# GAP-LAB-CUHK-SZ/GaussReg

Measured on AMD Instinct MI355X. Metric: GS views/sec @1M pts 640x480 (+ radius_neighbors Mpts/sec, see radius_neighbors), higher is better.
Workload: dtype f32; 1 GPU; diff_gaussian_rasterization forward: 1000000 synthetic Gaussians (SH deg 3), 640x480, 32 views per step per GPU (configs[1]); gaussians=1000000, width=640, height=480, parallelism=per-view sharding x1

## Files before the change

### gaussreg_amd/_lib.py

```python
import ctypes
import os
import re

_HERE = os.path.dirname(os.path.abspath(__file__))
LIB_PATH = os.path.join(_HERE, "lib", "libgaussreg_hip.so")
HEADER_PATH = os.path.join(_HERE, "..", "include", "gaussreg_hip.h")
TRAIN_HEADER_PATH = os.path.join(_HERE, "..", "include", "gaussreg_hip_train.h")
MATCH_TRAIN_HEADER_PATH = os.path.join(_HERE, "..", "include", "gaussreg_hip_train_matching.h")
BACKBONE_TRAIN_HEADER_PATH = os.path.join(_HERE, "..", "include", "gaussreg_hip_train_backbone.h")

_lib = None

c_void = ctypes.c_void_p
c_f32 = ctypes.c_float


class RasterView(ctypes.Structure):
    _fields_ = [("image_height", ctypes.c_int32), ("image_width", ctypes.c_int32),
                ("tanfovx", c_f32), ("tanfovy", c_f32), ("bg", c_f32 * 3), ("scale_modifier", c_f32),
                ("viewmatrix", c_f32 * 16), ("projmatrix", c_f32 * 16), ("campos", c_f32 * 3),
                ("sh_degree", ctypes.c_int32), ("prefiltered", ctypes.c_int32), ("debug", ctypes.c_int32)]


class GsAdamGroup(ctypes.Structure):
    _fields_ = [("param", c_void), ("grad", c_void), ("exp_avg", c_void), ("exp_avg_sq", c_void),
                ("lr", ctypes.c_double), ("K", ctypes.c_int32)]


class GsDensifyGroup(ctypes.Structure):
    _fields_ = [("src_param", c_void), ("dst_param", c_void), ("src_exp_avg", c_void), ("dst_exp_avg", c_void),
                ("src_exp_avg_sq", c_void), ("dst_exp_avg_sq", c_void), ("K", ctypes.c_int32), ("role", ctypes.c_int32)]


_SCALARS = {"int": ctypes.c_int, "int32_t": ctypes.c_int32, "uint32_t": ctypes.c_uint32, "int64_t": ctypes.c_int64,
            "size_t": ctypes.c_size_t, "float": ctypes.c_float, "double": ctypes.c_double}
_POINTEES = set(_SCALARS) | {"void", "uint8_t", "uint64_t"}
_STRUCTS = {"gr_raster_view": RasterView, "gr_gs_adam_group": GsAdamGroup, "gr_gs_densify_group": GsDensifyGroup}
_TYPE = r"(?:const\s+)?(\w+)"


def _ctype(base, star, where):
    if star:
        if base == "char":
            return ctypes.c_char_p
        if base in _STRUCTS:
            return ctypes.POINTER(_STRUCTS[base])
        if base in _POINTEES:
            return ctypes.c_void_p
    elif base in _SCALARS:
        return _SCALARS[base]
    raise ValueError(f"gaussreg_hip.h: type '{base}{star}' in {where} is outside the binding's vocabulary")


def parse_header(text):
    text = re.sub(r"/\*.*?\*/", " ", text, flags=re.S)
    defines = {m.group(1): int(m.group(2)) for m in re.finditer(r"^[ \t]*#[ \t]*define[ \t]+(GR_\w+)[ \t]+(-?\d+)[ \t]*$",
                                                                  text, flags=re.M)}
    text = re.sub(r"^[ \t]*#.*$", "", text, flags=re.M)
    text = re.sub(r"\b(?:typedef\s+struct|enum)\b[^{};]*\{[^{}]*\}[^;]*;", "", text)
    text = re.sub(r'extern\s+"C"\s*\{(.*)\}', r"\1", text, flags=re.S)
    signatures = {}
    for decl in filter(None, (" ".join(d.split()) for d in text.split(";"))):
        m = re.fullmatch(r"(.+?)\b(gr_\w+) ?\((.*)\)", decl)
        if m is None:
            raise ValueError(f"gaussreg_hip.h: cannot parse the declaration '{decl}'")
        ret, name, args = m.group(1).strip(), m.group(2), m.group(3).strip()
        r = re.fullmatch(_TYPE + r"\s*(\*?)", ret)
        if r is None:
            raise ValueError(f"gaussreg_hip.h: cannot parse the return type '{ret}' of {name}")
        restype = None if r.groups() == ("void", "") else _ctype(r.group(1), r.group(2), f"the return type of {name}")
        argtypes = []
        for arg in ([] if args in ("", "void") else args.split(",")):
            a = re.fullmatch(_TYPE + r"(?:\s*(\*)\s*|\s+)\w+", arg.strip())
            if a is None:
                raise ValueError(f"gaussreg_hip.h: cannot parse the argument '{arg.strip()}' of {name}")
            argtypes.append(_ctype(a.group(1), a.group(2) or "", f"argument '{arg.strip()}' of {name}"))
        if name in signatures:
            raise ValueError(f"gaussreg_hip.h: {name} is declared twice")
        signatures[name] = (restype, argtypes)
    return signatures, defines


with open(HEADER_PATH) as _f:
    SIGNATURES, DEFINES = parse_header(_f.read())
with open(TRAIN_HEADER_PATH) as _f:
    TRAIN_SIGNATURES, TRAIN_DEFINES = parse_header(_f.read())
with open(MATCH_TRAIN_HEADER_PATH) as _f:
    MATCH_TRAIN_SIGNATURES, MATCH_TRAIN_DEFINES = parse_header(_f.read())
with open(BACKBONE_TRAIN_HEADER_PATH) as _f:
    BACKBONE_TRAIN_SIGNATURES, BACKBONE_TRAIN_DEFINES = parse_header(_f.read())

GR_PENDING = DEFINES["GR_PENDING"]
GR_RETRY_FULL = DEFINES["GR_RETRY_FULL"]
GR_RETRY_BIN = DEFINES["GR_RETRY_BIN"]
GS_ADAM_MAX_GROUPS = DEFINES["GR_GS_ADAM_MAX_GROUPS"]
GS_KNN_MAX_K = DEFINES["GR_GS_KNN_MAX_K"]
GS_DENSIFY_CARRIED, GS_DENSIFY_XYZ, GS_DENSIFY_SCALING = (DEFINES["GR_GS_DENSIFY_" + r] for r in ("CARRIED", "XYZ", "SCALING"))


class HipLibraryError(RuntimeError):
    pass


def lib():
    global _lib
    if _lib is None:
        import torch
        if not os.path.exists(LIB_PATH):
            raise HipLibraryError(
                f"{LIB_PATH} is missing: build it with `python -m gaussreg_amd.build` "
                "(there is no CPU fallback for the gaussreg_amd ops)")
        L = ctypes.CDLL(LIB_PATH)
        for name, (res, args) in (list(SIGNATURES.items()) + list(TRAIN_SIGNATURES.items())
                                   + list(MATCH_TRAIN_SIGNATURES.items()) + list(BACKBONE_TRAIN_SIGNATURES.items())):
            fn = getattr(L, name)
            fn.restype = res
            fn.argtypes = args
        _lib = L
    return _lib


def check(rc, allow=()):
    if rc != 0 and rc not in allow:
        msg = lib().gr_last_error()
        raise RuntimeError("gaussreg_hip: " + (msg.decode() if msg else f"error {rc}"))
    return rc


def tensor_stamp(tensors):
    out = []
    for t in tensors:
        if t.is_inference():
            return None
        out.append((t.data_ptr(), t._version))
    return tuple(out)


def require_gpu():
    import torch
    if not torch.cuda.is_available():
        raise HipLibraryError("gaussreg_amd ops need an MI355X (torch.cuda.is_available() is False); "
                              "there is no CPU fallback")
    return torch.device("cuda", torch.cuda.current_device())


_ws_cache = {}


def workspace(device, nbytes):
    import threading

    import torch
    key = (device.type, device.index, torch.cuda.current_stream(device).cuda_stream, threading.get_ident())
    buf = _ws_cache.get(key)
    if buf is None or buf.numel() < nbytes:
        buf = torch.empty(int(nbytes * 1.25) + 4096, dtype=torch.uint8, device=device)
        _ws_cache[key] = buf
    return buf


def stream_ptr(device):
    import torch
    return ctypes.c_void_p(torch.cuda.current_stream(device).cuda_stream)


def ptr(t):
    return ctypes.c_void_p(t.data_ptr()) if t is not None else ctypes.c_void_p(0)


def device_ptr(t, dev, what, pos=None):
    if t is None:
        return None
    if t.is_cuda and t.device == dev and t.is_contiguous():
        return t.data_ptr()
    where = what if pos is None else f"{what}: argument {pos}"
    if not t.is_contiguous():
        raise HipLibraryError(f"{where}: the tensor is not contiguous")
    raise HipLibraryError(f"{where}: the tensor is on {t.device}, the call runs on {dev}")


def call(dev, name, *args, ws=None, allow=()):
    import torch
    Tensor = torch.Tensor
    argv = [device_ptr(a, dev, name, i) if isinstance(a, Tensor) else a for i, a in enumerate(args)]
    if ws is not None:
        if not isinstance(ws, Tensor):
            ws = workspace(dev, ws)
        argv += (device_ptr(ws, dev, name + ": workspace"), ws.numel())
    fn = getattr(lib(), name)
    with torch.cuda.device(dev):
        return check(fn(*argv, torch.cuda.current_stream(dev).cuda_stream), allow)


def to_device(t, dev, dtype=None, name=None, cast=True):
    if dtype is not None and not cast and t.dtype != dtype:
        raise RuntimeError(f"{name} must be a float tensor" if name else "expected a float tensor")
    if dev is None:
        dev = require_gpu()
    t = t if t.is_cuda else t.to(dev)
    return (t if dtype is None else t.to(dtype)).contiguous()


def to_device_bool(t, dev):
    import torch
    return to_device(t if t.dtype == torch.bool else t != 0, dev)


def like_input(outs, out_device):
    if out_device.type == "cuda":
        return outs
    return tuple(o.to(out_device) for o in outs) if isinstance(outs, (tuple, list)) else outs.to(out_device)


def offsets(lengths):
    off = [0]
    for n in lengths:
        off.append(off[-1] + int(n))
    return off


def host_i64(values):
    arr = (ctypes.c_int64 * max(len(values), 1))(*[int(v) for v in values])
    return arr
```

### gaussreg_amd/build.py

```python
import concurrent.futures
import os
import subprocess
import sys

HERE = os.path.dirname(os.path.abspath(__file__))
CSRC = os.path.join(HERE, "csrc")
LIBDIR = os.path.join(HERE, "lib")
OBJDIR = os.path.join(LIBDIR, "obj")
LIB = os.path.join(LIBDIR, "libgaussreg_hip.so")

HIPCC = os.environ.get("HIPCC", "/opt/rocm/bin/hipcc")
FLAGS = ["--offload-arch=gfx950", "-O3", "-std=c++17", "-fPIC", "-ffp-contract=off", "-Wall",
         "-Wno-unused-function", "-Wno-unused-result"]


def sources():
    return sorted(f for f in os.listdir(CSRC) if f.endswith(".hip"))


def _stale(out, deps):
    if not os.path.exists(out):
        return True
    t = os.path.getmtime(out)
    return any(os.path.getmtime(d) > t for d in deps)


def build(force=False, verbose=False):
    os.makedirs(OBJDIR, exist_ok=True)
    headers = [os.path.join(CSRC, f) for f in os.listdir(CSRC) if f.endswith((".hpp", ".h"))]
    headers += [os.path.join(HERE, "..", "include", h) for h in ("gaussreg_hip.h", "gaussreg_hip_train.h",
                                                                 "gaussreg_hip_train_matching.h",
                                                                 "gaussreg_hip_train_backbone.h")]
    jobs = []
    objs = []
    for src in sources():
        s = os.path.join(CSRC, src)
        o = os.path.join(OBJDIR, src[:-4] + ".o")
        objs.append(o)
        if force or _stale(o, [s] + headers):
            jobs.append([HIPCC] + FLAGS + ["-c", s, "-o", o])

    def run(cmd):
        if verbose:
            print(" ".join(cmd), flush=True)
        r = subprocess.run(cmd, stdout=subprocess.PIPE, stderr=subprocess.STDOUT, text=True)
        return cmd, r.returncode, r.stdout

    if jobs:
        with concurrent.futures.ThreadPoolExecutor(max_workers=min(8, len(jobs))) as ex:
            for cmd, rc, out in ex.map(run, jobs):
                if rc != 0:
                    raise RuntimeError("hipcc failed: %s\n%s" % (" ".join(cmd), out))
                if verbose and out.strip():
                    print(out)
    if force or jobs or _stale(LIB, objs):
        cmd = [HIPCC, "--offload-arch=gfx950", "-shared", "-fPIC", "-o", LIB] + objs
        _, rc, out = run(cmd)
        if rc != 0:
            raise RuntimeError("link failed:\n" + out)
    return LIB


if __name__ == "__main__":
    print(build(force="--force" in sys.argv, verbose=True))
```

### gaussreg_amd/csrc/common.hpp

```cpp
#pragma once
#include <hip/hip_runtime.h>

#include <cstdarg>
#include <cstdint>
#include <cstdio>
#include <cstring>

#include "../../include/gaussreg_hip.h"

namespace gr {

constexpr int WAVE = 64;
#if defined(__HIP_DEVICE_COMPILE__) && !defined(__gfx950__)
#error "libgaussreg_hip is written for gfx950 (MI355X, 160 KB of LDS per CU): build with --offload-arch=gfx950"
#endif

void set_error(const char* fmt, ...);

#define GR_HIP(call)                                                                       \
  do {                                                                                     \
    hipError_t _e = (call);                                                                \
    if (_e != hipSuccess) {                                                                \
      gr::set_error("%s failed: %s (%s:%d)", #call, hipGetErrorString(_e), __FILE__, __LINE__); \
      return GR_ERR_HIP;                                                                   \
    }                                                                                      \
  } while (0)

#define GR_REQUIRE(cond, ...)       \
  do {                              \
    if (!(cond)) {                  \
      gr::set_error(__VA_ARGS__);   \
      return GR_ERR_INVALID;        \
    }                               \
  } while (0)

#define GR_LAUNCH_CHECK() GR_HIP(hipGetLastError())

inline size_t align_up(size_t x, size_t a) { return (x + a - 1) / a * a; }

struct Carver {
  char* base;
  size_t off = 0;
  explicit Carver(void* p) : base(static_cast<char*>(p)) {}
  template <typename T>
  T* take(size_t count) {
    off = align_up(off, 256);
    T* r = reinterpret_cast<T*>(base ? base + off : nullptr);
    off += sizeof(T) * count;
    return r;
  }
  size_t used() const { return align_up(off, 256); }
};

__host__ __device__ inline uint32_t f2ord(float f) {
  uint32_t u;
#ifdef __HIP_DEVICE_COMPILE__
  u = __float_as_uint(f);
#else
  memcpy(&u, &f, 4);
#endif
  return (u & 0x80000000u) ? ~u : (u | 0x80000000u);
}
__host__ __device__ inline float ord2f(uint32_t o) {
  uint32_t u = (o & 0x80000000u) ? (o & 0x7fffffffu) : ~o;
  float f;
#ifdef __HIP_DEVICE_COMPILE__
  f = __uint_as_float(u);
#else
  memcpy(&f, &u, 4);
#endif
  return f;
}

size_t scan_ws_ints(int64_t n);
constexpr int SCAN_SINGLE_ROW = 2048;
int exclusive_scan_i32(const int32_t* in, int32_t* out, int64_t n, int rows, int64_t row_stride,
                       int32_t* scan_ws, int32_t* total, hipStream_t stream, const int32_t* last_dev = nullptr,
                       int32_t* row_max = nullptr);

void* pinned_scratch(int slot, size_t bytes);

constexpr int MAIL_WORDS = 1024;
constexpr int MAIL_GRID_BOXES = 0;
constexpr int MAIL_GRID_COUNTS = 512;
constexpr int MAIL_RADIUS = 1008;
volatile int32_t* mailbox();
inline void mailbox_arm(volatile int32_t* stamp_word) { __atomic_store_n(stamp_word, 0, __ATOMIC_RELEASE); }
int mailbox_next_stamp();
int mailbox_wait(const volatile int32_t* stamp_word, int stamp, hipStream_t stream, const char* what);
__device__ __forceinline__ void mail_post(int32_t* stamp_word, int stamp) {
  __hip_atomic_store(stamp_word, stamp, __ATOMIC_RELEASE, __HIP_MEMORY_SCOPE_SYSTEM);
}

void bbox_block_offsets(const int32_t* h_off, int32_t* h_blk, int nb);
int compute_bbox(const float* pts, const int32_t* h_off, int32_t* h_blk, const int32_t* off_dev, int nb,
                 uint32_t* bbox_dev, int32_t* blk_off_dev, hipStream_t stream, bool blk_off_on_device = false,
                 bool init_bbox = true,
                 int32_t* zeroed_ticket = nullptr, int32_t* mail = nullptr, int stamp = 0);

size_t sort_pairs_temp_bytes(int64_t n);
int sort_pairs_u64_i32(void* temp, size_t temp_bytes, const uint64_t* keys_in, uint64_t* keys_out,
                       const int32_t* vals_in, int32_t* vals_out, int64_t n, int begin_bit,
                       int end_bit, hipStream_t stream);
int sort_pairs_u64_iota(void* temp, size_t temp_bytes, const uint64_t* keys_in, uint64_t* keys_out, int64_t period,
                        int32_t* vals_out, int64_t n, int begin_bit, int end_bit, hipStream_t stream);

int lds_atomics_lane_ordered(hipStream_t stream, bool* ordered);
int lds_atomics_lane_ordered_state();
int lds_ballot_ranking_force(int on);
void lds_order_demote();

constexpr int RASTER_TILE = 16;
constexpr uint32_t RECT_MARKER26 = 127u | (127u << 7);
#ifdef __HIPCC__
__device__ __forceinline__ void get_rect(float px, float py, int radius, int gx, int gy, int* rmin, int* rmax) {
  const float r = (float)radius;
  rmin[0] = min(gx, max(0, (int)((px - r) / (float)RASTER_TILE)));
  rmin[1] = min(gy, max(0, (int)((py - r) / (float)RASTER_TILE)));
  rmax[0] = min(gx, max(0, (int)((px + r + (float)(RASTER_TILE - 1)) / (float)RASTER_TILE)));
  rmax[1] = min(gy, max(0, (int)((py + r + (float)(RASTER_TILE - 1)) / (float)RASTER_TILE)));
}
__device__ __forceinline__ bool rect_decode(uint32_t r, int id, int64_t vbase, const float4* __restrict__ rec, int gx,
                                            int gy, int& x0, int& y0, int& w, int& h) {
  x0 = (int)(r & 127u);
  y0 = (int)((r >> 7) & 127u);
  w = (int)((r >> 14) & 63u);
  h = (int)((r >> 20) & 63u);
  if (r == RECT_MARKER26) {
    const float4 r0 = rec[4 * (vbase + id)];
    int rmin[2], rmax[2];
    get_rect(r0.x, r0.y, __float_as_int(rec[4 * (vbase + id) + 3].x), gx, gy, rmin, rmax);
    x0 = rmin[0];
    y0 = rmin[1];
    w = rmax[0] - rmin[0];
    h = rmax[1] - rmin[1];
  }
  return w * h != 0;
}
#endif

struct DepthSortTotals {
  int32_t* chunk_total;
  int chunk, nchunk;
  const float4* rec;
  int gx, gy;
};
struct DepthSortSegments {
  const int32_t* seg_off;
  const uint32_t* range_in;
  uint64_t* key64_out;
  int key64_shift;
  int32_t* big_cnt;
  int32_t* big_list;
  const uint64_t* gather64;
  int bins_used = 0;
  int xcd_segments = 0;
};
size_t depth_sort_table_bytes(int64_t P, int V);
int depth_sort_views(const uint32_t* field, const uint32_t* rect_raw, uint64_t* keys_a, uint64_t* keys_b, int32_t* ids_out,
                     uint32_t* rect_out, int32_t* nvalid_out, int64_t P, int V, int key_bits, void* table, size_t table_bytes,
                     hipStream_t stream, const int2* key_mm = nullptr, int nb_mm = 0, int32_t* overflow_flag = nullptr,
                     int overflow_value = 0, const DepthSortTotals* chunk_totals = nullptr,
                     const DepthSortSegments* segments = nullptr);
bool depth_sort_msd_possible(int64_t P, int V, int key_bits);

void kpconv_rowflag_launch(const float* s_feats, int64_t n, int64_t cin, uint8_t* flag, hipStream_t stream);
void kpconv_gather_launch(int plan, const float* s_feats, const float* q_points, const float* s_points,
                          const int64_t* neighbor_indices, int64_t n, int64_t m, int64_t h, int64_t cin, int64_t k,
                          const float* kernel_points, float sigma, float inf, const uint8_t* flag, float* WF, float* num,
                          hipStream_t stream);

struct KernelTimer {
  KernelTimer(const char* name, hipStream_t stream);
  ~KernelTimer();
  KernelTimer(const KernelTimer&) = delete;
  int slot_;
  hipStream_t stream_;
};

void unordered_map_order(const uint64_t* keys, int64_t n, int32_t base, int32_t* perm_out);
size_t hash_order_device_bytes(int64_t n, int64_t batch);
int hash_order_device(const uint64_t* keys, const int64_t* h_begins, int64_t batch, int32_t* perm_out, void* ws,
                      size_t ws_bytes, hipStream_t stream, const float* rows_in = nullptr, const int32_t* row_of = nullptr,
                      float* rows_out = nullptr);

__device__ __forceinline__ int wave_incl_scan_add_dpp(int v) {
  v += __builtin_amdgcn_update_dpp(0, v, 0x111, 0xf, 0xf, false);
  v += __builtin_amdgcn_update_dpp(0, v, 0x112, 0xf, 0xf, false);
  v += __builtin_amdgcn_update_dpp(0, v, 0x114, 0xf, 0xf, false);
  v += __builtin_amdgcn_update_dpp(0, v, 0x118, 0xf, 0xf, false);
  v += __builtin_amdgcn_update_dpp(0, v, 0x142, 0xa, 0xf, false);
  v += __builtin_amdgcn_update_dpp(0, v, 0x143, 0xc, 0xf, false);
  return v;
}

__device__ __forceinline__ double wave_sum_f64_dpp(double x) {
#define GR_F64_STEP(CTRL, ROWMASK)                                                                         \
  {                                                                                                        \
    const int lo = __builtin_amdgcn_update_dpp(0, __double2loint(x), CTRL, ROWMASK, 0xf, false);           \
    const int hi = __builtin_amdgcn_update_dpp(0, __double2hiint(x), CTRL, ROWMASK, 0xf, false);           \
    x += __hiloint2double(hi, lo);                                                                         \
  }
  GR_F64_STEP(0x111, 0xf) GR_F64_STEP(0x112, 0xf) GR_F64_STEP(0x114, 0xf) GR_F64_STEP(0x118, 0xf)
  GR_F64_STEP(0x142, 0xa) GR_F64_STEP(0x143, 0xc)
#undef GR_F64_STEP
  return __hiloint2double(__builtin_amdgcn_readlane(__double2hiint(x), 63), __builtin_amdgcn_readlane(__double2loint(x), 63));
}

#define GR_DPP_REDUCE(NAME, OP, IDENT)                                                         \
  __device__ __forceinline__ int NAME(int v) {                                                 \
    v = OP(v, __builtin_amdgcn_update_dpp(IDENT, v, 0x111, 0xf, 0xf, false));                  \
    v = OP(v, __builtin_amdgcn_update_dpp(IDENT, v, 0x112, 0xf, 0xf, false));                  \
    v = OP(v, __builtin_amdgcn_update_dpp(IDENT, v, 0x114, 0xf, 0xf, false));                  \
    v = OP(v, __builtin_amdgcn_update_dpp(IDENT, v, 0x118, 0xf, 0xf, false));                  \
    v = OP(v, __builtin_amdgcn_update_dpp(IDENT, v, 0x142, 0xa, 0xf, false));                  \
    v = OP(v, __builtin_amdgcn_update_dpp(IDENT, v, 0x143, 0xc, 0xf, false));                  \
    return __builtin_amdgcn_readlane(v, 63);                                                   \
  }
#define GR_OP_MIN(a, b) min(a, b)
#define GR_OP_MAX(a, b) max(a, b)
#define GR_OP_ADD(a, b) ((a) + (b))
GR_DPP_REDUCE(wave_min_i32_dpp, GR_OP_MIN, 0x7fffffff)
GR_DPP_REDUCE(wave_max_i32_dpp, GR_OP_MAX, (int)0x80000000)
GR_DPP_REDUCE(wave_sum_i32_dpp, GR_OP_ADD, 0)
#undef GR_DPP_REDUCE

__device__ inline int find_batch(const int32_t* __restrict__ off, int nb, int32_t i) {
  int lo = 0, hi = nb;
  while (hi - lo > 1) {
    int mid = (lo + hi) >> 1;
    if (off[mid] <= i) lo = mid; else hi = mid;
  }
  return lo;
}

}
```

### gaussreg_amd/csrc/preprocess_body.hpp

```cpp
#ifndef GR_PREPROCESS_BODY_OK
#error "preprocess_body.hpp is the body of the two preprocess kernels of rasterizer.hip"
#endif
static_assert(std::is_same<decltype(WAVE_MM), const bool>::value, "the including kernel defines `constexpr bool WAVE_MM`");
  if (LATE && blockIdx.x == 0 && threadIdx.x < (int)(sizeof(DevView) / 4))
    reinterpret_cast<float*>(const_cast<DevView*>(views))[threadIdx.x] = reinterpret_cast<const float*>(&cam1)[threadIdx.x];
  __shared__ float4 s_sh[(SH16 && !LATE) ? WAVE * SH_ROW : 1];
  __shared__ float4 s_rec[256 / WAVE][4 * REC_PLANE];
  __shared__ int s_mm[WAVE_MM ? 1 : 2][2][256 / WAVE];
  int i = blockIdx.x * blockDim.x + threadIdx.x;
  float shr[SH16 ? 48 : 1];
  if (SH16 && !LATE) {
    const int g0 = blockIdx.x * 256;
    const int n_here = min(256, P - g0);
    const float4* src = reinterpret_cast<const float4*>(shs + (int64_t)g0 * 48);
#pragma unroll 1
    for (int w = 0; w < 256 / WAVE; ++w) {
      const int lim = min(WAVE, n_here - w * WAVE) * 12;
#pragma unroll
      for (int u = 0; u < 3; ++u) {
        const int f = threadIdx.x + u * 256;
        if (f < lim) {
          const int g = f / 12, j = f - g * 12;
          s_sh[g * SH_ROW + j] = src[w * WAVE * 12 + f];
        }
      }
      __syncthreads();
      if ((int)threadIdx.x / WAVE == w && i < P) {
#pragma unroll
        for (int j = 0; j < 12; ++j) {
          const float4 t = s_sh[(threadIdx.x & (WAVE - 1)) * SH_ROW + j];
          shr[4 * j] = t.x;
          shr[4 * j + 1] = t.y;
          shr[4 * j + 2] = t.z;
          shr[4 * j + 3] = t.w;
        }
      }
      __syncthreads();
    }
  }
  const bool valid = i < P;
  const int lane = threadIdx.x & (WAVE - 1);
  const int wave_first = i - lane;
  i = min(i, P - 1);
  const float p[3] = {means3D[3 * (int64_t)i], means3D[3 * (int64_t)i + 1], means3D[3 * (int64_t)i + 2]};
  const float opacity = opacities[i];
  float c6[6];
  if (HAS_COV) {
#pragma unroll
    for (int k = 0; k < 6; ++k) c6[k] = cov3D_precomp[6 * (int64_t)i + k];
  }
  const int gx = (W + TILE - 1) / TILE, gy = (H + TILE - 1) / TILE;
  const float* sh = HAS_SH ? shs + (int64_t)i * M * 3 : nullptr;
  float cpre[3] = {0.f, 0.f, 0.f};
  if (!HAS_SH) {
#pragma unroll
    for (int k = 0; k < 3; ++k) cpre[k] = colors_precomp[3 * (int64_t)i + k];
  }
  float4* wrec = s_rec[threadIdx.x / WAVE];
  float mod_prev = 0.f;
  bool have_cov = HAS_COV;
  for (int v = 0; v < V; ++v) {
    const DevView& cam = LATE ? cam1 : views[v];
    const int64_t o = (int64_t)v * P + i;
    int out_radius = 0;
    uint32_t out_field = 0u, out_rect = 0u;
    float out_depth = 0.f, out_sxx = INFINITY, out_syy = INFINITY, out_kc = 0.f;
    float2 out_xy = make_float2(0.f, 0.f);
    float4 out_co = make_float4(0.f, 0.f, 0.f, 0.f);
    bool shade = false;
    float rgb[3] = {0.f, 0.f, 0.f};
    float pv[3];
    xform4x3(cam.view, p, pv);
    if (pv[2] > 0.2f) {
      float ph[4];
      xform4x4(cam.proj, p, ph);
      const float pw = 1.0f / (ph[3] + 0.0000001f);
      const float pprojx = ph[0] * pw, pprojy = ph[1] * pw;
      if (!HAS_COV && (!have_cov || cam.scale_mod != mod_prev)) {
        float sc[3], rot[4];
#pragma unroll
        for (int k = 0; k < 3; ++k) sc[k] = scales[3 * (int64_t)i + k];
#pragma unroll
        for (int k = 0; k < 4; ++k) rot[k] = rotations[4 * (int64_t)i + k];
        cov3d_from_scale_rot(sc, cam.scale_mod, rot, c6);
        have_cov = true;
        mod_prev = cam.scale_mod;
      }
      float cv[3];
      cov2d(pv, cam.fx, cam.fy, cam.tanx, cam.tany, c6, cam.view, cv);
      const float det = cv[0] * cv[2] - cv[1] * cv[1];
      if (det != 0.0f) {
        const float det_inv = 1.f / det;
        const float mid = 0.5f * (cv[0] + cv[2]);
        const float sq = sqrtf(fmaxf(0.1f, mid * mid - det));
        const float l1 = mid + sq, l2 = mid - sq;
        const float my_radius = ceilf(3.f * sqrtf(fmaxf(l1, l2)));
        const float px = ((pprojx + 1.0f) * (float)W - 1.0f) * 0.5f;
        const float py = ((pprojy + 1.0f) * (float)H - 1.0f) * 0.5f;
        int rmin[2], rmax[2];
        get_rect(px, py, (int)my_radius, gx, gy, rmin, rmax);
        const int ntile = (rmax[0] - rmin[0]) * (rmax[1] - rmin[1]);
        if (ntile != 0) {
          shade = true;
          if (HAS_SH && SH16 && LATE) {
            const float4* s4 = reinterpret_cast<const float4*>(shs + (int64_t)i * 48);
#pragma unroll
            for (int jj = 0; jj < 12; ++jj) {
              const float4 t4 = s4[jj];
              shr[4 * jj] = t4.x;
              shr[4 * jj + 1] = t4.y;
              shr[4 * jj + 2] = t4.z;
              shr[4 * jj + 3] = t4.w;
            }
            sh_to_rgb(D, p, cam.campos, [&](int k, int c) { return shr[k * 3 + c]; }, rgb);
          }
          out_depth = pv[2];
          out_radius = (int)my_radius;
          out_xy = make_float2(px, py);
          out_co = make_float4(cv[2] * det_inv, -cv[1] * det_inv, cv[0] * det_inv, opacity);
          const bool cullable = det > 0.0f && l2 >= 0.29f && l1 < 1.0e4f;
          const float kc = cullable ? 1.001f / (0.5f / l1 - 2.0e-6f) : INFINITY;
          out_kc = kc;
          if (cullable) {
            out_sxx = 2.0f * cv[0] * 1.004f;
            out_syy = 2.0f * cv[2] * 1.004f;
            const float pcm = __logf(255.0f * opacity) + 2.0e-3f;
            if (pcm > 0.0f) {
              const float cp = pcm + 2.0e-6f * (pcm * kc);
              const float hx = sqrtf(2.0f * cp * cv[0]) * 1.001f + 1.0e-2f;
              const float hy = sqrtf(2.0f * cp * cv[2]) * 1.001f + 1.0e-2f;
              const float xlo = ceilf(px - hx), xhi = floorf(px + hx), ylo = ceilf(py - hy), yhi = floorf(py + hy);
              if (xlo > -1.0e6f && xhi < 1.0e6f && ylo > -1.0e6f && yhi < 1.0e6f) {
                rmin[0] = max(rmin[0], (int)floorf(xlo / (float)TILE));
                rmin[1] = max(rmin[1], (int)floorf(ylo / (float)TILE));
                rmax[0] = min(rmax[0], (int)floorf(xhi / (float)TILE) + 1);
                rmax[1] = min(rmax[1], (int)floorf(yhi / (float)TILE) + 1);
                if (rmax[0] < rmin[0]) rmax[0] = rmin[0];
                if (rmax[1] < rmin[1]) rmax[1] = rmin[1];
              }
            }
          }
          uint32_t dk = __float_as_uint(out_depth) - KEY_DEPTH_BASE;
          if (dk >= (1u << KEY_DEPTH_BITS)) {
            dk = (1u << KEY_DEPTH_BITS) - 1;
            if (LATE) *far_flag = far_seq; else atomicOr(far_flag, 1);
          }
          out_field = dk;
          out_rect = pack_rect(rmin, rmax);
        }
      }
    }
    if (valid) {
      __builtin_nontemporal_store(out_radius, radii + o);
      dfield[o] = out_field;
      rect_raw[o] = out_rect;
    }
    wrec[0 * REC_PLANE + lane] = make_float4(out_xy.x, out_xy.y, out_sxx, out_syy);
    wrec[1 * REC_PLANE + lane] = out_co;
    wrec[3 * REC_PLANE + lane] = make_float4(__int_as_float(out_radius), out_depth, 0.f, 0.f);
    if (WAVE_MM) {
      const uint32_t fld = valid ? out_field : 0u;
      const int mn = wave_min_i32_dpp(fld != 0u ? (int)fld : 0x7fffffff), mx = wave_max_i32_dpp((int)fld);
      const int wave_id = __builtin_amdgcn_readfirstlane((int)(blockIdx.x * (256 / WAVE) + threadIdx.x / WAVE));
      if (lane == 0) key_mm[(int64_t)v * (gridDim.x * (256 / WAVE)) + wave_id] = make_int2(mn, mx);
      __builtin_amdgcn_fence(__ATOMIC_RELEASE, "wavefront");
      __builtin_amdgcn_wave_barrier();
      __builtin_amdgcn_fence(__ATOMIC_ACQUIRE, "wavefront");
    } else if (key_mm != nullptr) {
      const uint32_t fld = valid ? out_field : 0u;
      const int mn = wave_min_i32_dpp(fld != 0u ? (int)fld : 0x7fffffff), mx = wave_max_i32_dpp((int)fld);
      if (lane == 0) s_mm[v & 1][0][threadIdx.x / WAVE] = mn, s_mm[v & 1][1][threadIdx.x / WAVE] = mx;
      __syncthreads();
      if (threadIdx.x == 0) {
        int bmn = 0x7fffffff, bmx = 0;
#pragma unroll
        for (int w = 0; w < 256 / WAVE; ++w) bmn = min(bmn, s_mm[v & 1][0][w]), bmx = max(bmx, s_mm[v & 1][1][w]);
        key_mm[(int64_t)v * gridDim.x + blockIdx.x] = make_int2(bmn, bmx);
      }
    }
    if (shade && !(HAS_SH && SH16 && LATE)) {
      if (HAS_SH) {
        if (SH16) sh_to_rgb(D, p, cam.campos, [&](int k, int c) { return shr[k * 3 + c]; }, rgb);
        else sh_to_rgb(D, p, cam.campos, [&](int k, int c) { return sh[k * 3 + c]; }, rgb);
      } else {
        rgb[0] = cpre[0]; rgb[1] = cpre[1]; rgb[2] = cpre[2];
      }
    }
    wrec[2 * REC_PLANE + lane] = make_float4(rgb[0], rgb[1], rgb[2], out_kc);
    const unsigned long long vis = __ballot(valid && out_radius > 0);
    __builtin_amdgcn_fence(__ATOMIC_RELEASE, "wavefront");
    __builtin_amdgcn_wave_barrier();
    __builtin_amdgcn_fence(__ATOMIC_ACQUIRE, "wavefront");
    float4* wout = rec + 4 * ((int64_t)v * P + wave_first);
#pragma unroll
    for (int k = 0; k < 4; ++k) {
      const int rl = 16 * k + lane / 4;
      const float4 piece = wrec[(lane & 3) * REC_PLANE + rl];
      if ((vis >> rl) & 1ull) {
        typedef float pre_f4 __attribute__((ext_vector_type(4)));
        __builtin_nontemporal_store(pre_f4{piece.x, piece.y, piece.z, piece.w}, reinterpret_cast<pre_f4*>(wout + 4 * rl + (lane & 3)));
      }
    }
    __builtin_amdgcn_fence(__ATOMIC_RELEASE, "wavefront");
    __builtin_amdgcn_wave_barrier();
    __builtin_amdgcn_fence(__ATOMIC_ACQUIRE, "wavefront");
  }
```

### gaussreg_amd/csrc/raster_shared.hpp

```cpp
#pragma once

#include "common.hpp"

namespace gr {
namespace {

constexpr int TILE = 16;
constexpr int BLOCK = TILE * TILE;
constexpr int MAX_VIEWS = 64;

struct DevView {
  float view[16];
  float proj[16];
  float campos[3];
  float tanx, tany;
  float fx, fy;
  float scale_mod;
  float bg[3];
};

__device__ __constant__ float SH_C0 = 0.28209479177387814f;
__device__ __constant__ float SH_C1 = 0.4886025119029199f;
__device__ __constant__ float SH_C2[5] = {1.0925484305920792f, -1.0925484305920792f,
                                          0.31539156525252005f, -1.0925484305920792f,
                                          0.5462742152960396f};
__device__ __constant__ float SH_C3[7] = {-0.5900435899266435f, 2.890611442640554f,
                                          -0.4570457994644658f, 0.3731763325901154f,
                                          -0.4570457994644658f, 1.445305721320277f,
                                          -0.5900435899266435f};

__device__ __forceinline__ float exp_det(float x) {
  x = fmaxf(x, -86.0f);
  const float L2E = 1.44269504088896341f, MAGIC = 12582912.0f;
  const float t = x * L2E;
  const float tm = t + MAGIC;
  const float nf = tm - MAGIC;
  const float f = fmaf(x, L2E, -nf);
  float p = 1.3264815788716078e-3f;
  p = fmaf(p, f, 9.671512059867382e-3f);
  p = fmaf(p, f, 5.550733581185341e-2f);
  p = fmaf(p, f, 2.4022242426872253e-1f);
  p = fmaf(p, f, 6.931470036506653e-1f);
  p = fmaf(p, f, 1.0f);
  return __uint_as_float(__float_as_uint(p) + (__float_as_uint(tm) << 23));
}

__device__ __forceinline__ void xform4x3(const float* M, const float* p, float* o) {
  o[0] = fmaf(M[0], p[0], fmaf(M[4], p[1], fmaf(M[8], p[2], M[12])));
  o[1] = fmaf(M[1], p[0], fmaf(M[5], p[1], fmaf(M[9], p[2], M[13])));
  o[2] = fmaf(M[2], p[0], fmaf(M[6], p[1], fmaf(M[10], p[2], M[14])));
}
__device__ __forceinline__ void xform4x4(const float* M, const float* p, float* o) {
  o[0] = fmaf(M[0], p[0], fmaf(M[4], p[1], fmaf(M[8], p[2], M[12])));
  o[1] = fmaf(M[1], p[0], fmaf(M[5], p[1], fmaf(M[9], p[2], M[13])));
  o[2] = fmaf(M[2], p[0], fmaf(M[6], p[1], fmaf(M[10], p[2], M[14])));
  o[3] = fmaf(M[3], p[0], fmaf(M[7], p[1], fmaf(M[11], p[2], M[15])));
}

__device__ __forceinline__ void cov3d_from_scale_rot(const float* sc, float mod, const float* q,
                                                     float* c6) {
  const float s0 = mod * sc[0], s1 = mod * sc[1], s2 = mod * sc[2];
  const float r = q[0], x = q[1], y = q[2], z = q[3];
  float R[3][3];
  R[0][0] = 1.f - 2.f * (y * y + z * z);
  R[0][1] = 2.f * (x * y - r * z);
  R[0][2] = 2.f * (x * z + r * y);
  R[1][0] = 2.f * (x * y + r * z);
  R[1][1] = 1.f - 2.f * (x * x + z * z);
  R[1][2] = 2.f * (y * z - r * x);
  R[2][0] = 2.f * (x * z - r * y);
  R[2][1] = 2.f * (y * z + r * x);
  R[2][2] = 1.f - 2.f * (x * x + y * y);
  float M[3][3];
#pragma unroll
  for (int i = 0; i < 3; ++i) {
    M[0][i] = s0 * R[i][0];
    M[1][i] = s1 * R[i][1];
    M[2][i] = s2 * R[i][2];
  }
#define GR_SIG(i, j) fmaf(M[0][i], M[0][j], fmaf(M[1][i], M[1][j], M[2][i] * M[2][j]))
  c6[0] = GR_SIG(0, 0);
  c6[1] = GR_SIG(0, 1);
  c6[2] = GR_SIG(0, 2);
  c6[3] = GR_SIG(1, 1);
  c6[4] = GR_SIG(1, 2);
  c6[5] = GR_SIG(2, 2);
#undef GR_SIG
}

__device__ __forceinline__ void cov2d(const float* t_in, float fx, float fy, float tanx, float tany,
                                      const float* c6, const float* V, float* out3) {
  float t[3] = {t_in[0], t_in[1], t_in[2]};
  const float limx = 1.3f * tanx, limy = 1.3f * tany;
  const float txtz = t[0] / t[2], tytz = t[1] / t[2];
  t[0] = fminf(limx, fmaxf(-limx, txtz)) * t[2];
  t[1] = fminf(limy, fmaxf(-limy, tytz)) * t[2];
  const float J00 = fx / t[2];
  const float J02 = -(fx * t[0]) / (t[2] * t[2]);
  const float J11 = fy / t[2];
  const float J12 = -(fy * t[1]) / (t[2] * t[2]);
  float A0[3], A1[3];
#pragma unroll
  for (int j = 0; j < 3; ++j) {
    A0[j] = fmaf(J00, V[j * 4 + 0], J02 * V[j * 4 + 2]);
    A1[j] = fmaf(J11, V[j * 4 + 1], J12 * V[j * 4 + 2]);
  }
  const float S[3][3] = {{c6[0], c6[1], c6[2]}, {c6[1], c6[3], c6[4]}, {c6[2], c6[4], c6[5]}};
  float B0[3], B1[3];
#pragma unroll
  for (int k = 0; k < 3; ++k) {
    B0[k] = fmaf(S[k][0], A0[0], fmaf(S[k][1], A0[1], S[k][2] * A0[2]));
    B1[k] = fmaf(S[k][0], A1[0], fmaf(S[k][1], A1[1], S[k][2] * A1[2]));
  }
  out3[0] = fmaf(A0[0], B0[0], fmaf(A0[1], B0[1], A0[2] * B0[2])) + 0.3f;
  out3[1] = fmaf(A1[0], B0[0], fmaf(A1[1], B0[1], A1[2] * B0[2]));
  out3[2] = fmaf(A1[0], B1[0], fmaf(A1[1], B1[1], A1[2] * B1[2])) + 0.3f;
}

template <typename ShLoad>
__device__ __forceinline__ void sh_to_rgb(int deg, const float* pos, const float* campos,
                                          ShLoad S, float* rgb) {
  const float dx = pos[0] - campos[0], dy = pos[1] - campos[1], dz = pos[2] - campos[2];
  const float len = sqrtf(dx * dx + dy * dy + dz * dz);
  const float x = dx / len, y = dy / len, z = dz / len;
#pragma unroll
  for (int c = 0; c < 3; ++c) {
    float res = SH_C0 * S(0, c);
    if (deg > 0) {
      res = res - SH_C1 * y * S(1, c) + SH_C1 * z * S(2, c) - SH_C1 * x * S(3, c);
      if (deg > 1) {
        const float xx = x * x, yy = y * y, zz = z * z, xy = x * y, yz = y * z, xz = x * z;
        res = res + SH_C2[0] * xy * S(4, c) + SH_C2[1] * yz * S(5, c) +
              SH_C2[2] * (2.0f * zz - xx - yy) * S(6, c) + SH_C2[3] * xz * S(7, c) +
              SH_C2[4] * (xx - yy) * S(8, c);
        if (deg > 2) {
          res = res + SH_C3[0] * y * (3.0f * xx - yy) * S(9, c) + SH_C3[1] * xy * z * S(10, c) +
                SH_C3[2] * y * (4.0f * zz - xx - yy) * S(11, c) +
                SH_C3[3] * z * (2.0f * zz - 3.0f * xx - 3.0f * yy) * S(12, c) +
                SH_C3[4] * x * (4.0f * zz - xx - yy) * S(13, c) +
                SH_C3[5] * z * (xx - yy) * S(14, c) + SH_C3[6] * x * (xx - 3.0f * yy) * S(15, c);
        }
      }
    }
    res += 0.5f;
    rgb[c] = fmaxf(res, 0.0f);
  }
}

struct Geom {
  float4* rec;
  uint32_t* dfield;
  uint32_t* rect_raw;
  uint64_t* keys_a;
  uint64_t* keys_b;
  int32_t* order_a;
  int32_t* order_b;
  uint32_t* rects;
  uint16_t* chunk_cnt;
  uint32_t* seg_off;
  int32_t* chunk_total;
  int32_t* chunk_max;
  void* ds_table;
  size_t ds_table_bytes;
  int2* key_mm;
  int32_t* nvis;
  int32_t* totals;
  DevView* views;
  int32_t* scan_ws;
  size_t bytes;
};

constexpr int BIN_T = 256;
constexpr int BIN_CHUNK = 2048;

Geom carve_geom(void* p, int64_t P, int V, int64_t tiles) {
  Geom g;
  Carver c(p);
  const int64_t nchunk = (P + BIN_CHUNK - 1) / BIN_CHUNK;
  g.rec = c.take<float4>(P * V * 4);
  g.dfield = c.take<uint32_t>(P * V);
  g.rect_raw = c.take<uint32_t>(P * V);
  g.keys_a = c.take<uint64_t>(P * V);
  g.keys_b = c.take<uint64_t>(P * V);
  g.order_a = nullptr;
  g.order_b = c.take<int32_t>(P * V);
  g.rects = c.take<uint32_t>(P * V);
  g.chunk_cnt = c.take<uint16_t>(V * nchunk * tiles);
  g.seg_off = c.take<uint32_t>(V * nchunk * (tiles + 1));
  g.chunk_total = c.take<int32_t>(2 * V * nchunk);
  g.chunk_max = c.take<int32_t>(1);
  g.ds_table_bytes = depth_sort_table_bytes(P, V);
  g.ds_table = c.take<char>(g.ds_table_bytes);
  g.key_mm = c.take<int2>(V <= 4 ? V * ((P + 255) / 256) : P <= (1ll << 20) ? V * ((P + 255) / 256) * (256 / WAVE) : 0);
  g.nvis = c.take<int32_t>(V);
  g.totals = c.take<int32_t>(2 * V + 4 + MAX_VIEWS * (sizeof(DevView) / sizeof(int32_t)));
  g.views = reinterpret_cast<DevView*>(g.totals ? g.totals + 2 * V + 4 : nullptr);
  static_assert(sizeof(DevView) % sizeof(int32_t) == 0, "camera table follows an int array");
  g.scan_ws = c.take<int32_t>(V * scan_ws_ints(nchunk));
  g.bytes = c.used();
  return g;
}

struct Bin {
  int32_t* point_list;
  size_t bytes;
};

Bin carve_bin(void* p, int64_t R, int64_t vtiles) {
  Bin b;
  Carver c(p);
  (void)vtiles;
  b.point_list = c.take<int32_t>(R + 64);
  b.bytes = c.used();
  return b;
}

}
}
```

### gaussreg_amd/csrc/rasterizer.hip

```cpp
#include <algorithm>
#include <type_traits>
#include <vector>

#include <atomic>

#include "raster_shared.hpp"

namespace gr {
namespace {

static_assert(TILE == RASTER_TILE, "get_rect / rect_decode (common.hpp) are written for this tile size");


constexpr int KEY_DEPTH_BITS = 27;
constexpr uint32_t KEY_DEPTH_BASE = 0x3E000000u;

__device__ __forceinline__ uint32_t pack_rect(const int* rmin, const int* rmax) {
  const int w = rmax[0] - rmin[0], h = rmax[1] - rmin[1];
  if (w > 63 || h > 63 || rmin[0] > 126 || rmin[1] > 126) return RECT_MARKER26;
  return (uint32_t)rmin[0] | ((uint32_t)rmin[1] << 7) | ((uint32_t)w << 14) | ((uint32_t)h << 20);
}

constexpr int REC_PLANE = 66;
constexpr int SH_ROW = 13;

template <bool HAS_SH, bool HAS_COV, bool SH16, bool LATE>
__global__ __launch_bounds__(256) void preprocess_kernel(
    int P, int D, int M, int V, const DevView* __restrict__ views, const float* __restrict__ means3D,
    const float* __restrict__ shs, const float* __restrict__ colors_precomp,
    const float* __restrict__ opacities, const float* __restrict__ scales,
    const float* __restrict__ rotations, const float* __restrict__ cov3D_precomp, int W, int H,
    int32_t* __restrict__ radii, float4* __restrict__ rec, uint32_t* __restrict__ dfield,
    uint32_t* __restrict__ rect_raw, int32_t* __restrict__ far_flag, DevView cam1, int far_seq,
    int2* __restrict__ key_mm) {
  constexpr bool WAVE_MM = false;
#define GR_PREPROCESS_BODY_OK
#include "preprocess_body.hpp"
#undef GR_PREPROCESS_BODY_OK
}

template <bool HAS_SH, bool HAS_COV, bool SH16>
__global__ __launch_bounds__(256) void preprocess_many_kernel(
    int P, int D, int M, int V, const DevView* __restrict__ views, const float* __restrict__ means3D,
    const float* __restrict__ shs, const float* __restrict__ colors_precomp,
    const float* __restrict__ opacities, const float* __restrict__ scales,
    const float* __restrict__ rotations, const float* __restrict__ cov3D_precomp, int W, int H,
    int32_t* __restrict__ radii, float4* __restrict__ rec, uint32_t* __restrict__ dfield,
    uint32_t* __restrict__ rect_raw, int32_t* __restrict__ far_flag, DevView cam1, int far_seq,
    int2* __restrict__ key_mm) {
  constexpr bool WAVE_MM = true;
  constexpr bool LATE = false;
#define GR_PREPROCESS_BODY_OK
#include "preprocess_body.hpp"
#undef GR_PREPROCESS_BODY_OK
}

__global__ __launch_bounds__(256) void full_keys_kernel(int64_t n, const float4* __restrict__ rec,
                                                        const int32_t* __restrict__ radii, uint32_t* __restrict__ dfield) {
  const int64_t o = (int64_t)blockIdx.x * blockDim.x + threadIdx.x;
  if (o >= n) return;
  dfield[o] = radii[o] > 0 ? __float_as_uint(rec[4 * o + 3].y) : 0u;
}


__device__ __forceinline__ bool bin_block(int V, int nchunk, int& v, int& c) {
  const int b = blockIdx.x;
  if (V >= 8) {
    const int k = b >> 3;
    v = (b & 7) + 8 * (k / nchunk);
    c = k % nchunk;
    return v < V;
  }
  v = b / nchunk;
  c = b % nchunk;
  return true;
}
inline int bin_grid(int V, int nchunk) { return V >= 8 ? 8 * ((V + 7) / 8) * nchunk : V * nchunk; }
inline bool bin_scans_self(int nchunk, int V) { return !(nchunk <= SCAN_SINGLE_ROW && V <= 4); }
constexpr int SCATTER_WGS = 6;
constexpr int WIDE_T = 1024;

__device__ __forceinline__ constexpr int mod_small(int n, int d) {
  const unsigned long long tab = d <= 4 ? 0x2001'2aab'4001'8001ull : 0x1001'124a'1556'199aull;
  const unsigned int m = (unsigned int)(tab >> (((d - 1) & 3) * 16)) & 0xffffu;
  return n - (int)(((unsigned int)n * m) >> 15) * d;
}
static_assert(mod_small(255, 7) == 255 % 7 && mod_small(254, 3) == 254 % 3 && mod_small(250, 5) == 0 &&
              mod_small(251, 6) == 251 % 6 && mod_small(255, 8) == 7 && mod_small(200, 1) == 0, "mod_small multipliers");
template <typename F>
__device__ __forceinline__ void by_modulus(int mx, F&& f) {
  switch (mx) {
    case 1: f(std::integral_constant<int, 1>{}); break;
    case 2: f(std::integral_constant<int, 2>{}); break;
    case 3: f(std::integral_constant<int, 3>{}); break;
    case 4: f(std::integral_constant<int, 4>{}); break;
    case 5: f(std::integral_constant<int, 5>{}); break;
    case 6: f(std::integral_constant<int, 6>{}); break;
    case 7: f(std::integral_constant<int, 7>{}); break;
    default: f(std::integral_constant<int, 8>{}); break;
  }
}

__global__ __launch_bounds__(BIN_T) void tile_count_kernel(int P, int V, int gx, int gy, int nchunk,
                                                           const int32_t* __restrict__ nvis,
                                                           const uint32_t* __restrict__ rects,
                                                           const int32_t* __restrict__ ids,
                                                           const float4* __restrict__ rec,
                                                           uint16_t* __restrict__ chunk_cnt,
                                                           int32_t* __restrict__ chunk_total) {
  extern __shared__ unsigned int s_hist[];
  __shared__ int s_wsum[BIN_T / WAVE];
  int v, c;
  if (!bin_block(V, nchunk, v, c)) return;
  const int tiles = gx * gy;
  for (int T = threadIdx.x; T < tiles; T += BIN_T) s_hist[T] = 0u;
  __syncthreads();
  const int64_t vbase = (int64_t)v * P;
  const int nv = nvis[v];
  int mine = 0;
  uint32_t rr[BIN_CHUNK / BIN_T];
#pragma unroll
  for (int it = 0; it < BIN_CHUNK / BIN_T; ++it) {
    const int t = c * BIN_CHUNK + it * BIN_T + threadIdx.x;
    rr[it] = t < nv ? rects[vbase + t] : 0u;
  }
#pragma unroll
  for (int it = 0; it < BIN_CHUNK / BIN_T; ++it) {
    const int t = c * BIN_CHUNK + it * BIN_T + threadIdx.x;
    const uint32_t r = rr[it];
    if (r == 0u) continue;
    int x0, y0, w, h;
    if (!rect_decode(r, r == RECT_MARKER26 ? ids[vbase + t] : 0, vbase, rec, gx, gy, x0, y0, w, h)) continue;
    mine += w * h;
    for (int y = y0; y < y0 + h; ++y)
      for (int x = x0; x < x0 + w; ++x) atomicAdd(&s_hist[y * gx + x], 1u);
  }
  const int wsum = wave_sum_i32_dpp(mine);
  if ((threadIdx.x & (WAVE - 1)) == 0) s_wsum[threadIdx.x / WAVE] = wsum;
  __syncthreads();
  uint16_t* dst = chunk_cnt + ((int64_t)v * nchunk + c) * tiles;
  for (int T = threadIdx.x; T < tiles; T += BIN_T) dst[T] = (uint16_t)s_hist[T];
  if (threadIdx.x == 0) {
    int tot = 0;
    for (int i = 0; i < BIN_T / WAVE; ++i) tot += s_wsum[i];
    chunk_total[v * nchunk + c] = tot;
  }
}

__global__ __launch_bounds__(BIN_T) void chunk_total_kernel(int P, int V, int gx, int gy, int nchunk,
                                                            const int32_t* __restrict__ nvis,
                                                            const uint32_t* __restrict__ rects,
                                                            const int32_t* __restrict__ ids,
                                                            const float4* __restrict__ rec,
                                                            int32_t* __restrict__ chunk_total) {
  __shared__ int s_wsum[BIN_T / WAVE];
  int v, c;
  if (!bin_block(V, nchunk, v, c)) return;
  const int64_t vbase = (int64_t)v * P;
  const int nv = nvis[v];
  int mine = 0;
  uint32_t rr[BIN_CHUNK / BIN_T];
#pragma unroll
  for (int it = 0; it < BIN_CHUNK / BIN_T; ++it) {
    const int t = c * BIN_CHUNK + it * BIN_T + threadIdx.x;
    rr[it] = t < nv ? rects[vbase + t] : 0u;
  }
#pragma unroll
  for (int it = 0; it < BIN_CHUNK / BIN_T; ++it) {
    const int t = c * BIN_CHUNK + it * BIN_T + threadIdx.x;
    const uint32_t r = rr[it];
    int x0, y0, w, h;
    if (r != 0u && rect_decode(r, r == RECT_MARKER26 ? ids[vbase + t] : 0, vbase, rec, gx, gy, x0, y0, w, h)) mine += w * h;
  }
  const int wsum = wave_sum_i32_dpp(mine);
  if ((threadIdx.x & (WAVE - 1)) == 0) s_wsum[threadIdx.x / WAVE] = wsum;
  __syncthreads();
  if (threadIdx.x == 0) {
    int tot = 0;
    for (int i = 0; i < BIN_T / WAVE; ++i) tot += s_wsum[i];
    chunk_total[v * nchunk + c] = tot;
  }
}

__global__ __launch_bounds__(1024) void chunk_max_kernel(int n, const int32_t* __restrict__ chunk_total,
                                                         int32_t* __restrict__ chunk_max) {
  __shared__ int s_m[1024 / WAVE];
  int m = 0;
  for (int i = threadIdx.x; i < n; i += 1024) m = max(m, chunk_total[i]);
  m = wave_max_i32_dpp(m);
  if ((threadIdx.x & (WAVE - 1)) == 0) s_m[threadIdx.x / WAVE] = m;
  __syncthreads();
  if (threadIdx.x == 0) {
    for (int i = 0; i < 1024 / WAVE; ++i) m = max(m, s_m[i]);
    *chunk_max = m;
  }
}

template <bool SELF>
__global__ __launch_bounds__(256) void seg_scan_kernel(int V, int tiles, int nchunk, const uint16_t* __restrict__ chunk_cnt,
                                                       const int32_t* __restrict__ chunk_base ,
                                                       int32_t* __restrict__ totals, uint32_t* __restrict__ seg_off,
                                                       int32_t* __restrict__ mail, int mail_seq) {
  __shared__ int s_w[256 / WAVE];
  __shared__ int s_carry;
  const int v = blockIdx.x / nchunk, c = blockIdx.x % nchunk;
  const int lane = threadIdx.x & (WAVE - 1), wv = threadIdx.x / WAVE;
  int vb = 0;
  if (SELF) {
    const int me = (int)blockIdx.x;
    int part = 0;
    for (int i = threadIdx.x; i < me; i += 256) part += chunk_base[i];
    part = wave_sum_i32_dpp(part);
    if (lane == 0) s_w[wv] = part;
    __syncthreads();
    vb = s_w[0] + s_w[1] + s_w[2] + s_w[3];
    __syncthreads();
    if (c == 0) {
      int sum = 0, mx = 0;
      for (int i = threadIdx.x; i < nchunk; i += 256) {
        const int t = chunk_base[v * nchunk + i];
        sum += t;
        mx = max(mx, t);
      }
      sum = wave_sum_i32_dpp(sum);
      mx = wave_max_i32_dpp(mx);
      if (lane == 0) {
        s_w[wv] = sum;
      }
      __shared__ int s_m[256 / WAVE];
      if (lane == 0) s_m[wv] = mx;
      __syncthreads();
      if (threadIdx.x == 0) {
        const int tv = s_w[0] + s_w[1] + s_w[2] + s_w[3], mv = max(max(s_m[0], s_m[1]), max(s_m[2], s_m[3]));
        totals[v] = tv;
        totals[V + v] = mv;
        if (mail != nullptr) {
          __hip_atomic_store(&mail[v], tv, __ATOMIC_RELAXED, __HIP_MEMORY_SCOPE_SYSTEM);
          __hip_atomic_store(&mail[V + v], mv, __ATOMIC_RELAXED, __HIP_MEMORY_SCOPE_SYSTEM);
          if (v == 0) __hip_atomic_store(&mail[2 * V], totals[2 * V], __ATOMIC_RELAXED, __HIP_MEMORY_SCOPE_SYSTEM);
          __hip_atomic_store(&mail[2 * V + 1 + v], mail_seq, __ATOMIC_RELEASE, __HIP_MEMORY_SCOPE_SYSTEM);
        }
      }
      __syncthreads();
    }
  } else {
    for (int u = 0; u < v; ++u) vb += totals[u];
  }
  const uint16_t* src = chunk_cnt + ((int64_t)v * nchunk + c) * tiles;
  uint32_t* dst = seg_off + ((int64_t)v * nchunk + c) * (tiles + 1);
  if (threadIdx.x == 0) s_carry = SELF ? vb : vb + chunk_base[v * nchunk + c];
  __syncthreads();
  for (int T0 = 0; T0 < tiles; T0 += 256) {
    const int T = T0 + threadIdx.x;
    const int n = T < tiles ? (int)src[T] : 0;
    const int incl = wave_incl_scan_add_dpp(n);
    if (lane == WAVE - 1) s_w[wv] = incl;
    __syncthreads();
    int base = s_carry;
    for (int i = 0; i < wv; ++i) base += s_w[i];
    if (T < tiles) dst[T] = (uint32_t)(base + incl - n);
    __syncthreads();
    if (threadIdx.x == 255) s_carry = base + incl;
    __syncthreads();
  }
  if (threadIdx.x == 0) dst[tiles] = (uint32_t)s_carry;
}

constexpr int SEG_READ = 0, SEG_SELF_RAW = 1, SEG_SELF_SCAN = 2;
struct SelfSeg {
  const int32_t* chunk_total;
  int32_t* totals;
  int32_t* mail;
  int mail_seq;
};
template <bool LANE_ORDERED, int TT, int SEG = SEG_READ>
__global__ __launch_bounds__(TT) void tile_scatter_kernel(int P, int V, int gx, int gy, int nchunk, int tile_bits,
                                                             int stage_cap, const int32_t* __restrict__ nvis,
                                                             const uint32_t* __restrict__ rects,
                                                             const int32_t* __restrict__ ids,
                                                             const float4* __restrict__ rec,
                                                             uint32_t* __restrict__ seg_off,
                                                             int32_t* __restrict__ point_list, unsigned int list_cap, int elist_cap,
                                                             SelfSeg self) {
  extern __shared__ unsigned int s_cur[];
  constexpr int NW = TT / WAVE, CW = BIN_CHUNK / NW;
  constexpr bool SELF = SEG != SEG_READ;
  int v, c;
  if (!bin_block(V, nchunk, v, c)) return;
  const int tiles = gx * gy;
  const int row = (tiles + 1) & ~1;
  uint32_t* seg = seg_off + ((int64_t)v * nchunk + c) * (tiles + 1);
  const int lane = threadIdx.x & (WAVE - 1), wv = threadIdx.x / WAVE;
  const int64_t vbase = (int64_t)v * P;
  const int w_begin = c * BIN_CHUNK + wv * (BIN_CHUNK / (TT / WAVE));
  uint32_t rr[BIN_CHUNK / TT];
  int32_t ii[BIN_CHUNK / TT];
#pragma unroll
  for (int j = 0; j < BIN_CHUNK / TT; ++j) {
    const int64_t o = vbase + min(w_begin + j * WAVE + lane, P - 1);
    rr[j] = rects[o];
    ii[j] = ids[o];
  }
  const int nv = nvis[v];
  __shared__ int s_red[2][TT / WAVE];
  __shared__ unsigned int s_carry;
  unsigned int chunk_begin;
  int total;
  if (SEG == SEG_SELF_RAW) {
    const int me = v * nchunk + c;
    int part = 0;
    for (int i = threadIdx.x; i < me; i += TT) part += self.chunk_total[i];
    part = wave_sum_i32_dpp(part);
    if (lane == 0) s_red[0][wv] = part;
    __syncthreads();
    int front = 0;
#pragma unroll
    for (int w2 = 0; w2 < TT / WAVE; ++w2) front += s_red[0][w2];
    chunk_begin = (unsigned int)front;
    total = self.chunk_total[me];
    if (c == 0) {
      __syncthreads();
      int sum = 0, mx = 0;
      for (int i = threadIdx.x; i < nchunk; i += TT) {
        const int t = self.chunk_total[v * nchunk + i];
        sum += t;
        mx = max(mx, t);
      }
      sum = wave_sum_i32_dpp(sum);
      mx = wave_max_i32_dpp(mx);
      if (lane == 0) s_red[0][wv] = sum, s_red[1][wv] = mx;
      __syncthreads();
      if (threadIdx.x == 0) {
        int tv = 0, mv = 0;
        for (int w2 = 0; w2 < TT / WAVE; ++w2) tv += s_red[0][w2], mv = max(mv, s_red[1][w2]);
        self.totals[v] = tv;
        self.totals[V + v] = mv;
        if (self.mail != nullptr) {
          __hip_atomic_store(&self.mail[v], tv, __ATOMIC_RELAXED, __HIP_MEMORY_SCOPE_SYSTEM);
          __hip_atomic_store(&self.mail[V + v], mv, __ATOMIC_RELAXED, __HIP_MEMORY_SCOPE_SYSTEM);
          if (v == 0) __hip_atomic_store(&self.mail[2 * V], self.totals[2 * V], __ATOMIC_RELAXED, __HIP_MEMORY_SCOPE_SYSTEM);
          __hip_atomic_store(&self.mail[2 * V + 1 + v], self.mail_seq, __ATOMIC_RELEASE, __HIP_MEMORY_SCOPE_SYSTEM);
        }
      }
    }
  } else if (SEG == SEG_SELF_SCAN) {
    unsigned int front = (unsigned int)self.chunk_total[(int64_t)V * nchunk + v * nchunk + c];
    for (int u = 0; u < v; ++u) front += (unsigned int)self.totals[u];
    chunk_begin = front;
    total = self.chunk_total[v * nchunk + c];
  } else {
    chunk_begin = seg[0];
    total = (int)(seg[tiles] - chunk_begin);
    if (total == 0 || seg[tiles] > list_cap) return;
  }
  if (SELF && total == 0) {
    for (int T = threadIdx.x; T <= tiles; T += TT) seg[T] = chunk_begin;
    return;
  }
  const bool big = total > 0xffff;
  const bool staged = !big && total <= stage_cap;
  unsigned int* myw = s_cur + wv * (row / 2);
  unsigned short* const cur16 = reinterpret_cast<unsigned short*>(s_cur);
  unsigned short* my16 = cur16 + wv * row;
  unsigned short* stage = reinterpret_cast<unsigned short*>(s_cur + NW * (row / 2));
  unsigned int* elist = s_cur + NW * (row / 2) + (stage_cap + 1) / 2 + wv * elist_cap;
  for (int T = threadIdx.x; T < NW * (row / 2); T += TT) s_cur[T] = 0u;
  __syncthreads();
  const int w_end = min(nv, w_begin + CW);
#pragma unroll
  for (int j = 0; j < CW / WAVE; ++j) {
    const int t = w_begin + j * WAVE + lane;
    rr[j] = t < w_end ? rr[j] : 0u;
    ii[j] = t < w_end ? ii[j] : 0;
  }
  auto count = [&](int tile) { atomicAdd(&myw[tile >> 1], 1u << ((tile & 1) * 16)); };
#pragma unroll
  for (int j = 0; j < CW / WAVE; ++j) {
    const uint32_t r = rr[j];
    int x0 = 0, y0 = 0, w = 0, h = 0;
    if (r != 0u && !rect_decode(r, ii[j], vbase, rec, gx, gy, x0, y0, w, h)) w = h = 0;
    const int Mx = wave_max_i32_dpp(w), My = wave_max_i32_dpp(h);
    auto cwalk = [&](auto mtag) {
      constexpr int MX = decltype(mtag)::value;
      const int x0m = mod_small(x0, MX), y0m = mod_small(y0, My);
#pragma unroll 1
      for (int ry = 0; ry < My; ++ry) {
        int dy = ry - y0m;
        dy += dy < 0 ? My : 0;
        const int rowbase = (y0 + dy) * gx + x0;
#pragma unroll
        for (int rx = 0; rx < MX; ++rx) {
          int dx = rx - x0m;
          dx += dx < 0 ? MX : 0;
          if (dy < h && dx < w) count(rowbase + dx);
        }
      }
    };
    if (Mx == 0) continue;
    if (TT == WIDE_T || max(Mx, My) > 8) {
      for (int y = y0; y < y0 + h; ++y)
        for (int x = x0; x < x0 + w; ++x) count(y * gx + x);
    } else
      by_modulus(Mx, cwalk);
  }
  __syncthreads();
  if (SELF) {
    if (threadIdx.x == 0) s_carry = 0u;
    __syncthreads();
    for (int T0 = 0; T0 < tiles; T0 += TT) {
      const int T = T0 + (int)threadIdx.x;
      unsigned int cw[NW];
      int n_all = 0;
#pragma unroll
      for (int w2 = 0; w2 < NW; ++w2) {
        cw[w2] = T < tiles ? cur16[w2 * row + T] : 0u;
        n_all += (int)cw[w2];
      }
      const int incl = wave_incl_scan_add_dpp(n_all);
      if (lane == WAVE - 1) s_red[0][wv] = incl;
      __syncthreads();
      unsigned int before = s_carry + (unsigned int)(incl - n_all);
      for (int w2 = 0; w2 < wv; ++w2) before += (unsigned int)s_red[0][w2];
      if (T < tiles) {
        seg[T] = chunk_begin + before;
        unsigned int run = big ? 0u : before;
#pragma unroll
        for (int w2 = 0; w2 < NW; ++w2) {
          cur16[w2 * row + T] = (unsigned short)run;
          run += cw[w2];
        }
      }
      __syncthreads();
      if (threadIdx.x == TT - 1) s_carry = before + (unsigned int)n_all;
      __syncthreads();
    }
    if (threadIdx.x == 0) seg[tiles] = chunk_begin + (unsigned int)total;
    if (chunk_begin + (unsigned int)total > list_cap) return;
  } else {
    for (int T = threadIdx.x; T < tiles; T += TT) {
      unsigned int run = big ? 0u : seg[T] - chunk_begin;
#pragma unroll
      for (int w2 = 0; w2 < NW; ++w2) {
        const unsigned int n = cur16[w2 * row + T];
        cur16[w2 * row + T] = (unsigned short)run;
        run += n;
      }
    }
  }
  __syncthreads();
  auto put = [&](unsigned int tile, unsigned int pos, int local, int val) {
    if (staged) stage[pos] = (unsigned short)local;
    else if (!big) point_list[chunk_begin + pos] = val;
    else point_list[seg[tile] + pos] = val;
  };
  auto bump_raw = [&](unsigned int tile) -> unsigned int {
    return atomicAdd(&myw[tile >> 1], 1u << ((tile & 1u) * 16u));
  };
  auto bump = [&](unsigned int tile) -> unsigned int { return (bump_raw(tile) >> ((tile & 1u) * 16u)) & 0xffffu; };
  const unsigned long long lt = (1ull << lane) - 1ull;
#pragma unroll 1
  for (int t0 = w_begin; t0 < w_end; t0 += WAVE) {
    const int t = t0 + lane;
    int x0 = 0, y0 = 0, w = 0, h = 0;
    const int id = ii[0];
    const uint32_t r_now = rr[0];
#pragma unroll
    for (int k = 0; k + 1 < CW / WAVE; ++k) {
      rr[k] = rr[k + 1];
      ii[k] = ii[k + 1];
    }
    if (r_now != 0u && !rect_decode(r_now, id, vbase, rec, gx, gy, x0, y0, w, h)) w = h = 0;
    unsigned long long live = __ballot(w * h != 0);
    if (live == 0ull) continue;
    const int Mx = wave_max_i32_dpp(w), My = wave_max_i32_dpp(h);
    const int maxd = max(Mx, My);
    if (maxd <= 8) {
      auto walk = [&](auto mtag) {
        constexpr int MX = decltype(mtag)::value;
        const int x0m = mod_small(x0, MX), y0m = mod_small(y0, My);
        auto dx_of = [&](int rx) {
          const int d = rx - x0m;
          return d + (d < 0 ? MX : 0);
        };
#pragma unroll 1
        for (int ry = 0; ry < My; ++ry) {
          int dy = ry - y0m;
          dy += dy < 0 ? My : 0;
          const int rowbase = (y0 + dy) * gx + x0;
          const bool vy = dy < h;
          if (LANE_ORDERED) {
            unsigned int raw[MX];
            bool act[MX];
            const int wrow = vy ? w : 0;
#pragma unroll
            for (int rx = 0; rx < MX; ++rx) {
              const int dx = dx_of(rx);
              act[rx] = dx < wrow;
              raw[rx] = 0u;
              if (act[rx]) raw[rx] = bump_raw((unsigned int)(rowbase + dx));
            }
#pragma unroll
            for (int rx = 0; rx < MX; ++rx)
              if (act[rx]) {
                const unsigned int tile = (unsigned int)(rowbase + dx_of(rx));
                put(tile, (raw[rx] >> ((tile & 1u) * 16u)) & 0xffffu, t - c * BIN_CHUNK, id);
              }
          } else {
            for (int rx = 0; rx < MX; ++rx) {
              const int dx = dx_of(rx);
              const bool act = vy && dx < w;
              const unsigned int tile = (unsigned int)(rowbase + dx);
              unsigned long long peers = __ballot(act);
              if (peers == 0ull) continue;
              for (int bit = 0; bit < tile_bits; ++bit) {
                const bool one = (tile >> bit) & 1u;
                const unsigned long long bal = __ballot(one);
                peers &= one ? bal : ~bal;
              }
              if (act) {
                const unsigned int base = my16[tile];
                put(tile, base + (unsigned int)__popcll(peers & lt), t - c * BIN_CHUNK, id);
                if ((peers >> lane) == 1ull) my16[tile] = (unsigned short)(base + (unsigned int)__popcll(peers));
              }
              __builtin_amdgcn_fence(__ATOMIC_RELEASE, "wavefront");
              __builtin_amdgcn_wave_barrier();
              __builtin_amdgcn_fence(__ATOMIC_ACQUIRE, "wavefront");
            }
          }
        }
      };
      int n_inst = 0, inc_inst = 0, t_inst = 0x7fffffff;
      if (maxd > 4 && elist_cap > 0) {
        n_inst = w * h;
        inc_inst = wave_incl_scan_add_dpp(n_inst);
        t_inst = __builtin_amdgcn_readlane(inc_inst, WAVE - 1);
      }
      if (t_inst > elist_cap) by_modulus(Mx, walk);
      else {
        {
          unsigned int* dst = elist + (inc_inst - n_inst);
          const unsigned int tag = (unsigned int)lane << 16;
          for (int dy = 0; dy < h; ++dy)
            for (int dx = 0; dx < w; ++dx) *dst++ = tag | (unsigned int)((y0 + dy) * gx + x0 + dx);
        }
        __builtin_amdgcn_fence(__ATOMIC_RELEASE, "wavefront");
        __builtin_amdgcn_wave_barrier();
        __builtin_amdgcn_fence(__ATOMIC_ACQUIRE, "wavefront");
        for (int i0 = 0; i0 < t_inst; i0 += WAVE) {
          const int i = i0 + lane;
          const bool act = i < t_inst;
          const unsigned int e = act ? elist[i] : 0u;
          const int owner = (int)(e >> 16);
          const unsigned int tile = e & 0xffffu;
          const int oid = __shfl(id, owner, WAVE);
          const int olocal = t0 + owner - c * BIN_CHUNK;
          if (LANE_ORDERED) {
            if (act) put(tile, bump(tile), olocal, oid);
          } else {
            unsigned long long peers = __ballot(act);
            for (int bit = 0; bit < tile_bits; ++bit) {
              const bool one = (tile >> bit) & 1u;
              const unsigned long long bal = __ballot(one);
              peers &= one ? bal : ~bal;
            }
            if (act) {
              const unsigned int base = my16[tile];
              put(tile, base + (unsigned int)__popcll(peers & lt), olocal, oid);
              if ((peers >> lane) == 1ull) my16[tile] = (unsigned short)(base + (unsigned int)__popcll(peers));
            }
          }
          __builtin_amdgcn_fence(__ATOMIC_RELEASE, "wavefront");
          __builtin_amdgcn_wave_barrier();
          __builtin_amdgcn_fence(__ATOMIC_ACQUIRE, "wavefront");
        }
      }
    } else {
      const uint32_t pr = (uint32_t)x0 | ((uint32_t)y0 << 8) | ((uint32_t)w << 16) | ((uint32_t)h << 24);
      while (live) {
        const int j = __ffsll((long long)live) - 1;
        live &= live - 1ull;
        const uint32_t sr = (uint32_t)__builtin_amdgcn_readlane((int)pr, j);
        const int sid = __builtin_amdgcn_readlane(id, j);
        const int sx = (int)(sr & 255u), sy = (int)((sr >> 8) & 255u), sw = (int)((sr >> 16) & 255u), sh = (int)(sr >> 24);
        for (int y = 0; y < sh; ++y)
          for (int xb = 0; xb < sw; xb += WAVE)
            if (xb + lane < sw) {
              const unsigned int tile = (unsigned int)((sy + y) * gx + sx + xb + lane);
              if (LANE_ORDERED) {
                put(tile, bump(tile), t0 + j - c * BIN_CHUNK, sid);
              } else {
                const unsigned int pos = my16[tile];
                my16[tile] = (unsigned short)(pos + 1u);
                put(tile, pos, t0 + j - c * BIN_CHUNK, sid);
              }
            }
        __builtin_amdgcn_fence(__ATOMIC_RELEASE, "wavefront");
        __builtin_amdgcn_wave_barrier();
        __builtin_amdgcn_fence(__ATOMIC_ACQUIRE, "wavefront");
      }
    }
  }
  if (!staged) return;
  __syncthreads();
  const int32_t* cid = ids + vbase + (int64_t)c * BIN_CHUNK;
  int i = threadIdx.x;
  for (; i + 3 * TT < total; i += 4 * TT) {
    const int a0 = cid[stage[i]], a1 = cid[stage[i + TT]], a2 = cid[stage[i + 2 * TT]], a3 = cid[stage[i + 3 * TT]];
    point_list[chunk_begin + i] = a0;
    point_list[chunk_begin + i + TT] = a1;
    point_list[chunk_begin + i + 2 * TT] = a2;
    point_list[chunk_begin + i + 3 * TT] = a3;
  }
  for (; i < total; i += TT) point_list[chunk_begin + i] = cid[stage[i]];
}

typedef float f32x2 __attribute__((ext_vector_type(2)));
constexpr int CELL = 4;
constexpr int NCELL = (TILE / CELL) * (TILE / CELL);

template <typename T>
__device__ __forceinline__ T lds_at(const T* base, unsigned int byte_off) {
  return *reinterpret_cast<const T*>(reinterpret_cast<const char*>(base) + byte_off);
}
__device__ __forceinline__ float max_f32_raw(float a, float b) {
  float r;
  asm("v_max_f32 %0, %1, %2" : "=v"(r) : "v"(a), "v"(b));
  return r;
}

__device__ __forceinline__ float min_f32_raw(float a, float b) {
  float r;
  asm("v_min_f32 %0, %1, %2" : "=v"(r) : "v"(a), "v"(b));
  return r;
}

template <bool FAST_EXP>
__device__ __forceinline__ float entry_alpha(float4 a, float cy, float op, f32x2 pf, float& power) {
  const f32x2 d = f32x2{a.x, a.y} - pf;
  const f32x2 m = f32x2{a.z, a.w} * d;
  float q, t;
  asm("v_mul_f32 %0, %1, %2" : "=v"(q) : "v"(m.y), "v"(d.y));
  asm("v_fma_f32 %0, %1, %2, %0" : "+v"(q) : "v"(m.x), "v"(d.x));
  asm("v_mul_f32 %0, %1, %2" : "=v"(t) : "v"(cy), "v"(d.x));
  asm("v_mul_f32 %0, %0, %1" : "+v"(t) : "v"(d.y));
  asm("v_fma_f32 %0, -0.5, %1, -%2" : "=v"(power) : "v"(q), "v"(t));
  float e;
  if (FAST_EXP) {
    e = __builtin_amdgcn_exp2f(power * 1.44269504088896341f);
  } else {
    const float x = max_f32_raw(power, -86.0f);
    const float tm = x * 1.44269504088896341f + 12582912.0f;
    const float f = fmaf(x, 1.44269504088896341f, -(tm - 12582912.0f));
    float pl = fmaf(1.3264815788716078e-3f, f, 9.671512059867382e-3f);
    pl = fmaf(pl, f, 5.550733581185341e-2f);
    pl = fmaf(pl, f, 2.4022242426872253e-1f);
    pl = fmaf(pl, f, 6.931470036506653e-1f);
    pl = fmaf(pl, f, 1.0f);
    e = __uint_as_float(__float_as_uint(pl) + (__float_as_uint(tm) << 23));
  }
  return min_f32_raw(op * e, 0.99f);
}

template <bool AUX>
struct BlendAux {};
template <>
struct BlendAux<true> {
  float* depth;
  float* alpha;
  float* state;
};

template <bool FAST_EXP, bool KEEP = false, bool AUX = false>
__global__ __launch_bounds__(BLOCK) __attribute__((amdgpu_waves_per_eu(8, 8))) void blend_kernel(
    int P, int W, int H, int nchunk, const DevView* __restrict__ views, const uint32_t* __restrict__ seg_off,
    const int32_t* __restrict__ point_list, const float4* __restrict__ rec, float* __restrict__ out_color,
    unsigned int list_cap, BlendAux<AUX> aux) {
  __shared__ float4 s_ga[BLOCK + 1], s_gb[BLOCK + 1];
  __shared__ f32x2 s_gc[BLOCK + 1];
  __shared__ float s_z[AUX ? BLOCK + 1 : 1];
  __shared__ unsigned short s_list[NCELL][BLOCK + 2];
  __shared__ int s_cnt[NCELL][BLOCK / WAVE];
  __shared__ int s_alldone[BLOCK / WAVE];
  __shared__ int s_wpre[WAVE];
  __shared__ unsigned int s_woff[WAVE];
  const int gx = (W + TILE - 1) / TILE, gy = (H + TILE - 1) / TILE;
  if (list_cap != 0xffffffffu && nchunk > 0 &&
      seg_off[(int64_t)gridDim.z * nchunk * (gx * gy + 1) - 1] > list_cap) return;
  const int v = blockIdx.z;
  const int tile = blockIdx.y * gx + blockIdx.x;
  const int tid = threadIdx.x;
  const int lane = tid & (WAVE - 1), lw = tid / WAVE;
  const int cell = tid / (CELL * CELL), pin = tid % (CELL * CELL);
  const int lx = (cell % (TILE / CELL)) * CELL + pin % CELL;
  const int ly = (cell / (TILE / CELL)) * CELL + pin / CELL;
  const int pxi = blockIdx.x * TILE + lx, pyi = blockIdx.y * TILE + ly;
  const bool inside = pxi < W && pyi < H;
  const f32x2 pf = {(float)pxi, (float)pyi};
  const float tx0 = (float)(blockIdx.x * TILE), ty0 = (float)(blockIdx.y * TILE);
  const int tiles = gx * gy;
  const int64_t goff = (int64_t)v * P;
  bool done = !inside;
  if (tid == 0) {
    s_ga[BLOCK] = make_float4(0.0f, 0.0f, 0.0f, 0.0f);
    s_gb[BLOCK] = make_float4(0.0f, 0.0f, INFINITY, 0.0f);
    s_gc[BLOCK] = f32x2{0.0f, 0.0f};
    if (AUX) s_z[BLOCK] = 0.0f;
  }
  float T = 1.0f, C0 = 0.f, Dz = 0.f;
  f32x2 C12 = {0.f, 0.f};
  int c_next = 0, w_pos = 0, w_total = 0;
  int list_base = 0, batch_base = 0, last = 0;
  const uint32_t* seg_col = seg_off + (int64_t)v * nchunk * (tiles + 1) + tile;
  while (true) {
    const unsigned long long live = __ballot(!done);
    if (lane == 0) s_alldone[lw] = live == 0ull ? 1 : 0;
    __syncthreads();
    if (s_alldone[0] & s_alldone[1] & s_alldone[2] & s_alldone[3]) break;
    bool exhausted = false;
    while (w_pos >= w_total) {
      if (c_next >= nchunk) {
        exhausted = true;
        break;
      }
      if (tid < WAVE) {
        const int c = c_next + tid;
        unsigned int a = 0u, b = 0u;
        if (c < nchunk) {
          a = seg_col[(int64_t)c * (tiles + 1)];
          b = seg_col[(int64_t)c * (tiles + 1) + 1];
        }
        s_woff[tid] = a;
        s_wpre[tid] = wave_incl_scan_add_dpp((int)(b - a));
      }
      __syncthreads();
      if (KEEP) list_base += w_total;
      w_total = s_wpre[WAVE - 1];
      w_pos = 0;
      c_next += WAVE;
      __syncthreads();
    }
    if (exhausted) break;
    const int e = w_pos + tid;
    if (KEEP) batch_base = list_base + w_pos;
    w_pos += BLOCK;
    float ctr_x = 0.0f, ctr_y = 0.0f, rc2 = -1.0f, hx2 = 0.0f, hy2 = 0.0f;
    if (e < w_total) {
      int lo = 0;
#pragma unroll
      for (int st = WAVE / 2; st > 0; st >>= 1)
        if (s_wpre[lo + st - 1] <= e) lo += st;
      const int before = lo ? s_wpre[lo - 1] : 0;
      const float4* r = rec + 4 * (goff + point_list[s_woff[lo] + (unsigned int)(e - before)]);
      const float4 r0 = r[0];
      const float4 co = r[1];
      const float4 col = r[2];
      const float pc = -__logf(255.0f * co.w) - 1.0e-3f;
      rc2 = -pc * col.w;
      const float cpr = -pc + 1.0e-3f + 2.0e-6f * rc2;
      hx2 = cpr * r0.z;
      hy2 = cpr * r0.w;
      ctr_x = r0.x;
      ctr_y = r0.y;
      s_ga[tid] = make_float4(r0.x, r0.y, co.x, co.z);
      s_gb[tid] = make_float4(co.y, co.w, pc, col.x);
      s_gc[tid] = f32x2{col.y, col.z};
      if (AUX) s_z[tid] = r[3].y;
    }
    float ex2[TILE / CELL], ey2[TILE / CELL];
    bool xin[TILE / CELL], yin[TILE / CELL];
#pragma unroll
    for (int c = 0; c < TILE / CELL; ++c) {
      const float xlo = tx0 + (float)(c * CELL), ylo = ty0 + (float)(c * CELL);
      const float ex = fmaxf(fmaxf(xlo - ctr_x, ctr_x - (xlo + (float)(CELL - 1))), 0.0f);
      const float ey = fmaxf(fmaxf(ylo - ctr_y, ctr_y - (ylo + (float)(CELL - 1))), 0.0f);
      ex2[c] = ex * ex;
      ey2[c] = ey * ey;
      xin[c] = !(ex2[c] > hx2);
      yin[c] = !(ey2[c] > hy2);
    }
    unsigned long long reach[NCELL];
    int cnt_lane = 0;
#pragma unroll
    for (int c = 0; c < NCELL; ++c) {
      reach[c] = __ballot(!(ex2[c % (TILE / CELL)] + ey2[c / (TILE / CELL)] > rc2) && xin[c % (TILE / CELL)] &&
                          yin[c / (TILE / CELL)]);
      asm("v_writelane_b32 %0, %1, %2" : "+v"(cnt_lane) : "s"((int)__popcll(reach[c])), "n"(c));
    }
    if (lane < NCELL) s_cnt[lane][lw] = cnt_lane;
    __syncthreads();
    int base_lane = 0, tot_lane = 0;
    if (lane < NCELL) {
#pragma unroll
      for (int w = 0; w < BLOCK / WAVE; ++w) {
        const int n = s_cnt[lane][w];
        base_lane += w < lw ? n : 0;
        tot_lane += n;
      }
      if (lw == 0 && (tot_lane & 1)) s_list[lane][tot_lane] = (unsigned short)(16 * BLOCK);
    }
#pragma unroll
    for (int c = 0; c < NCELL; ++c) {
      const int base = __builtin_amdgcn_readlane(base_lane, c);
      const unsigned int rank = __builtin_amdgcn_mbcnt_hi((unsigned int)(reach[c] >> 32),
                                                          __builtin_amdgcn_mbcnt_lo((unsigned int)reach[c], 0u));
      if (__builtin_amdgcn_inverse_ballot_w64(reach[c])) s_list[c][base + rank] = (unsigned short)(16 * tid);
    }
    __syncthreads();
    const int len_cell = __shfl(tot_lane, (BLOCK / WAVE) * lw + lane / (CELL * CELL));
    const int n_cell = done ? 0 : len_cell;
    const unsigned int* lp = reinterpret_cast<const unsigned int*>(&s_list[cell][0]);
    unsigned int pair = lp[0];
    for (int i = 0; i < n_cell && !done; i += 2) {
      const unsigned int o0 = pair & 0xffffu, o1 = pair >> 16;
      pair = lp[i / 2 + 1];
      const float4 a0 = lds_at(s_ga, o0), b0 = lds_at(s_gb, o0);
      const float4 a1 = lds_at(s_ga, o1), b1 = lds_at(s_gb, o1);
      const f32x2 c0 = lds_at(s_gc, o0 / 2), c1 = lds_at(s_gc, o1 / 2);
      asm volatile("" ::"v"(b0.w), "v"(b1.w), "v"(b0.z), "v"(b1.z));
      float power0, power1;
      const float alpha0 = entry_alpha<FAST_EXP>(a0, b0.x, b0.y, pf, power0);
      const float alpha1 = entry_alpha<FAST_EXP>(a1, b1.x, b1.y, pf, power1);
      asm volatile("" ::"v"(c0.x), "v"(c0.y), "v"(c1.x), "v"(c1.y), "v"(alpha0), "v"(alpha1));
      const bool ok0 = !(power0 > 0.0f) && !(alpha0 < 1.0f / 255.0f);
      const bool ok1 = !(power1 > 0.0f) && !(alpha1 < 1.0f / 255.0f);
      if (ok0) {
        const float test_T = T * (1.0f - alpha0);
        if (test_T < 0.0001f) {
          done = true;
        } else {
          const float w = alpha0 * T;
          C0 = fmaf(b0.w, w, C0);
          C12 = __builtin_elementwise_fma(c0, f32x2{w, w}, C12);
          if (AUX) Dz = fmaf(lds_at(s_z, o0 / 4), w, Dz);
          T = test_T;
          if (KEEP) last = batch_base + (int)(o0 / 16) + 1;
        }
      }
      if (ok1 && !done) {
        const float test_T = T * (1.0f - alpha1);
        if (test_T < 0.0001f) {
          done = true;
        } else {
          const float w = alpha1 * T;
          C0 = fmaf(b1.w, w, C0);
          C12 = __builtin_elementwise_fma(c1, f32x2{w, w}, C12);
          if (AUX) Dz = fmaf(lds_at(s_z, o1 / 4), w, Dz);
          T = test_T;
          if (KEEP) last = batch_base + (int)(o1 / 16) + 1;
        }
      }
    }
  }
  if (inside) {
    const DevView& cam = views[v];
    float* o = out_color + (int64_t)v * 3 * H * W + (int64_t)pyi * W + pxi;
    o[0] = fmaf(T, cam.bg[0], C0);
    o[(int64_t)H * W] = fmaf(T, cam.bg[1], C12.x);
    o[2 * (int64_t)H * W] = fmaf(T, cam.bg[2], C12.y);
    if constexpr (AUX) {
      const int64_t q = ((int64_t)v * H + pyi) * W + pxi;
      aux.depth[q] = Dz;
      aux.alpha[q] = 1.0f - T;
    }
    if (KEEP) {
      const int64_t q = ((int64_t)v * H + pyi) * W + pxi, hw = (int64_t)gridDim.z * H * W;
      if constexpr (AUX) {
        aux.state[q] = T;
        reinterpret_cast<int32_t*>(aux.state)[hw + q] = last;
      } else {
        out_color[3 * hw + q] = T;
        reinterpret_cast<int32_t*>(out_color)[4 * hw + q] = last;
      }
    }
  }
}

__global__ __launch_bounds__(256) void mark_visible_kernel(int P, const float* __restrict__ means3D,
                                                           float v2, float v6, float v10, float v14,
                                                           uint8_t* __restrict__ present) {
  const int i = blockIdx.x * blockDim.x + threadIdx.x;
  if (i >= P) return;
  const float z = fmaf(v2, means3D[3 * (int64_t)i],
                       fmaf(v6, means3D[3 * (int64_t)i + 1], fmaf(v10, means3D[3 * (int64_t)i + 2], v14)));
  present[i] = z > 0.2f ? 1 : 0;
}

int check_views(const gr_raster_view* h_views, int num_views) {
  GR_REQUIRE(h_views != nullptr && num_views >= 1, "need at least one view");
  GR_REQUIRE(num_views <= MAX_VIEWS, "at most %d views per call (got %d)", MAX_VIEWS, num_views);
  for (int v = 0; v < num_views; ++v) {
    GR_REQUIRE(h_views[v].image_width == h_views[0].image_width &&
                   h_views[v].image_height == h_views[0].image_height &&
                   h_views[v].sh_degree == h_views[0].sh_degree,
               "all views of one call must share image size and sh_degree");
    GR_REQUIRE(h_views[v].image_width > 0 && h_views[v].image_height > 0, "bad image size");
    GR_REQUIRE(h_views[v].sh_degree >= 0 && h_views[v].sh_degree <= 3, "sh_degree must be 0..3");
  }
  return GR_OK;
}

__global__ __launch_bounds__(256) void verify_depth_order_kernel(int P, int V, const int32_t* __restrict__ nvis,
                                                                 const uint32_t* __restrict__ dfield,
                                                                 const int32_t* __restrict__ ids, int32_t* __restrict__ rank,
                                                                 int* __restrict__ bad) {
  const int v = blockIdx.y;
  const int n = nvis[v];
  const int64_t o = (int64_t)v * P;
  for (int i = blockIdx.x * 256 + threadIdx.x; i < n; i += gridDim.x * 256) {
    const int a = ids[o + i];
    rank[o + a] = i;
    if (i + 1 < n) {
      const int b = ids[o + i + 1];
      const uint32_t fa = dfield[o + a], fb = dfield[o + b];
      if (fa > fb || (fa == fb && a >= b)) atomicOr(bad, 1);
    }
  }
}

__global__ __launch_bounds__(256) void verify_tile_lists_kernel(int P, int V, int nchunk, int tiles,
                                                                const uint32_t* __restrict__ seg_off,
                                                                const int32_t* __restrict__ point_list,
                                                                const int32_t* __restrict__ rank, int* __restrict__ bad) {
  const int v = blockIdx.x / nchunk;
  const uint32_t* seg = seg_off + (int64_t)blockIdx.x * (tiles + 1);
  const int32_t* rk = rank + (int64_t)v * P;
  for (int t = threadIdx.x; t < tiles; t += 256) {
    int prev = -1;
    for (uint32_t e = seg[t]; e < seg[t + 1]; ++e) {
      const int r = rk[point_list[e]];
      if (r <= prev) atomicOr(bad, 2);
      prev = r;
    }
  }
}

}
}

namespace gr {
namespace {
std::atomic<int> g_frames[64];

bool verify_this_frame() {
  static const bool always = getenv("GR_RASTER_VERIFY") && getenv("GR_RASTER_VERIFY")[0] == '1';
  if (lds_atomics_lane_ordered_state() != 1) return always;
  int dev = 0;
  if (hipGetDevice(&dev) != hipSuccess || dev < 0 || dev >= 64) dev = 63;
  const int f = g_frames[dev].load();
  return always || f < 3 || (f & 255) == 0;
}

thread_local int g_bucket_cooldown = 0;
constexpr int BUCKET_COOLDOWN_FRAMES = 256;
bool bucket_sort_allowed(bool possible) {
  if (!possible) return false;
  if (g_bucket_cooldown == 0) return true;
  --g_bucket_cooldown;
  return false;
}
void bucket_sort_overflowed() { g_bucket_cooldown = BUCKET_COOLDOWN_FRAMES; }

void frame_done() {
  int dev = 0;
  if (hipGetDevice(&dev) != hipSuccess || dev < 0 || dev >= 64) dev = 63;
  g_frames[dev].fetch_add(1);
}

template <typename F>
int device_check(hipStream_t stream, F&& launch_check, int* h_flag) {
  int* d_bad = nullptr;
  GR_HIP(hipMallocAsync(reinterpret_cast<void**>(&d_bad), sizeof(int), stream));
  GR_HIP(hipMemsetAsync(d_bad, 0, sizeof(int), stream));
  launch_check(d_bad);
  GR_HIP(hipMemcpyAsync(h_flag, d_bad, sizeof(int), hipMemcpyDeviceToHost, stream));
  GR_HIP(hipStreamSynchronize(stream));
  GR_HIP(hipFreeAsync(d_bad, stream));
  return GR_OK;
}

constexpr int VIEW_PACK = 4;
struct ViewPack {
  DevView v[VIEW_PACK];
};
__global__ void upload_views_kernel(ViewPack pack, int num_views, int32_t* __restrict__ d_flag) {
  const int t = threadIdx.x;
  if (t < 4) d_flag[t] = 0;
  constexpr int WORDS = sizeof(DevView) / 4;
  float* dst = reinterpret_cast<float*>(d_flag + 4);
  const float* src = reinterpret_cast<const float*>(&pack);
  for (int i = t; i < num_views * WORDS; i += blockDim.x) dst[i] = src[i];
}

static void fill_view(DevView& d, const gr_raster_view& s) {
  memcpy(d.view, s.viewmatrix, sizeof(d.view));
  memcpy(d.proj, s.projmatrix, sizeof(d.proj));
  memcpy(d.campos, s.campos, sizeof(d.campos));
  memcpy(d.bg, s.bg, sizeof(d.bg));
  d.tanx = s.tanfovx;
  d.tany = s.tanfovy;
  d.fx = (float)s.image_width / (2.0f * s.tanfovx);
  d.fy = (float)s.image_height / (2.0f * s.tanfovy);
  d.scale_mod = s.scale_modifier;
}

int upload_views(const gr_raster_view* h_views, int num_views, int32_t* d_flag, hipStream_t stream) {
  static_assert(sizeof(DevView) % 4 == 0, "DevView is copied word by word");
  if (num_views <= VIEW_PACK) {
    ViewPack pack;
    memset(&pack, 0, sizeof(pack));
    for (int v = 0; v < num_views; ++v) fill_view(pack.v[v], h_views[v]);
    hipLaunchKernelGGL(upload_views_kernel, dim3(1), dim3(WAVE), 0, stream, pack, num_views, d_flag);
    GR_LAUNCH_CHECK();
    return GR_OK;
  }
  char* raw = static_cast<char*>(pinned_scratch(0, 16 + sizeof(DevView) * num_views));
  GR_REQUIRE(raw != nullptr, "pinned staging buffer for %d views could not be allocated", num_views);
  memset(raw, 0, 16);
  DevView* stage = reinterpret_cast<DevView*>(raw + 16);
  for (int v = 0; v < num_views; ++v) fill_view(stage[v], h_views[v]);
  GR_HIP(hipMemcpyAsync(d_flag, raw, 16 + sizeof(DevView) * num_views, hipMemcpyHostToDevice, stream));
  return GR_OK;
}

}
}

using namespace gr;

static int64_t tiles_of(int width, int height) {
  return (int64_t)((width + TILE - 1) / TILE) * ((height + TILE - 1) / TILE);
}

extern "C" int gr_raster_lds_atomics_lane_ordered(void) { return lds_atomics_lane_ordered_state(); }
extern "C" int gr_raster_ballot_ranking(int on) { return lds_ballot_ranking_force(on); }

extern "C" size_t gr_raster_geom_bytes(int64_t P, int num_views, int width, int height) {
  if (P < 0 || num_views < 1 || width <= 0 || height <= 0) return 0;
  return carve_geom(nullptr, P, num_views, tiles_of(width, height)).bytes;
}

extern "C" int gr_raster_debug_geom_layout(int64_t P, int num_views, int width, int height, int64_t* h_offsets) {
  GR_REQUIRE(P >= 0 && num_views >= 1 && width > 0 && height > 0 && h_offsets != nullptr, "bad argument");
  char* const origin = reinterpret_cast<char*>(uintptr_t(1) << 32);
  const Geom g = carve_geom(origin, P, num_views, tiles_of(width, height));
  h_offsets[0] = reinterpret_cast<char*>(g.dfield) - origin;
  h_offsets[1] = reinterpret_cast<char*>(g.order_b) - origin;
  h_offsets[2] = reinterpret_cast<char*>(g.rects) - origin;
  h_offsets[3] = reinterpret_cast<char*>(g.nvis) - origin;
  return 4;
}

extern "C" size_t gr_raster_bin_bytes(int64_t total_rendered, int width, int height, int num_views) {
  if (total_rendered < 0 || width <= 0 || height <= 0 || num_views < 1) return 0;
  return carve_bin(nullptr, total_rendered, tiles_of(width, height) * num_views).bytes;
}

struct Deferred {
  hipEvent_t ev;
  volatile int32_t* mail;
  int seq;
  int far_seq;
  bool by_mail;
  bool bucket_sort;
  bool self_seg;
};

static int preprocess_impl(int64_t P, int M, const float* means3D, const float* shs,
                           const float* colors_precomp, const float* opacities,
                           const float* scales, const float* rotations,
                           const float* cov3D_precomp, const gr_raster_view* h_views,
                           int num_views, int32_t* radii, void* geom, size_t geom_bytes,
                           int64_t* h_num_rendered, hipStream_t stream, Deferred* defer_ev) {
  int rc = check_views(h_views, num_views);
  if (rc != GR_OK) return rc;
  GR_REQUIRE(h_num_rendered != nullptr, "h_num_rendered is null");
  for (int v = 0; v <= num_views; ++v) h_num_rendered[v] = 0;
  GR_REQUIRE(P >= 0 && P < (1ll << 31) - 1, "P out of range");
  if (P == 0) {
    Geom g0 = carve_geom(geom, 0, num_views, tiles_of(h_views[0].image_width, h_views[0].image_height));
    if (!geom || geom_bytes < g0.bytes) {
      set_error("raster geometry buffer too small: need %zu bytes, got %zu", g0.bytes, geom_bytes);
      return GR_ERR_WORKSPACE;
    }
    rc = upload_views(h_views, num_views, g0.totals + 2 * num_views, stream);
    if (rc != GR_OK) return rc;
    GR_HIP(hipStreamSynchronize(stream));
    return GR_OK;
  }
  GR_REQUIRE(means3D && opacities && radii, "means3D / opacities / radii must be non-null");
  GR_REQUIRE((shs != nullptr) != (colors_precomp != nullptr),
             "Please provide excatly one of either SHs or precomputed colors!");
  GR_REQUIRE(((scales != nullptr && rotations != nullptr) != (cov3D_precomp != nullptr)) &&
                 ((scales != nullptr) == (rotations != nullptr)),
             "Please provide exactly one of either scale/rotation pair or precomputed 3D covariance!");
  const int D = h_views[0].sh_degree;
  if (shs) GR_REQUIRE(M >= (D + 1) * (D + 1), "shs has %d coefficients, sh_degree %d needs %d", M, D, (D + 1) * (D + 1));
  const int W = h_views[0].image_width, H = h_views[0].image_height;
  const int gx = (W + TILE - 1) / TILE, gy = (H + TILE - 1) / TILE;
  const int tiles = gx * gy;
  GR_REQUIRE(gx <= 255 && gy <= 255, "image too large: at most 255 x 255 tiles of 16 px (got %d x %d)", gx, gy);
  const size_t bin_lds = (size_t)(BIN_T / WAVE) * tiles * sizeof(unsigned int);
  GR_REQUIRE(bin_lds <= 156 * 1024, "image too large: the per-wave tile cursors (%zu bytes) do not fit in LDS", bin_lds);
  Geom g = carve_geom(geom, P, num_views, tiles);
  if (!geom || geom_bytes < g.bytes) {
    set_error("raster geometry buffer too small: need %zu bytes, got %zu", g.bytes, geom_bytes);
    return GR_ERR_WORKSPACE;
  }
  const dim3 blk(256), grd((unsigned)((P + 255) / 256));
  const bool sh16 = shs != nullptr && M == 16 && (reinterpret_cast<uintptr_t>(shs) % 16 == 0);
  const bool cam_in_args = sh16 && num_views == 1 && defer_ev != nullptr && defer_ev->mail != nullptr &&
                           (P + BIN_CHUNK - 1) / BIN_CHUNK <= SCAN_SINGLE_ROW;
  DevView cam1;
  memset(&cam1, 0, sizeof(cam1));
  int far_seq = 1;
  if (sh16 && num_views == 1) fill_view(cam1, h_views[0]);
  if (cam_in_args) {
    far_seq = defer_ev->seq;
  } else {
    rc = upload_views(h_views, num_views, g.totals + 2 * num_views, stream);
    if (rc != GR_OK) return rc;
  }
  if (defer_ev != nullptr) defer_ev->far_seq = far_seq;
  const bool msd_possible = depth_sort_msd_possible(P, num_views, KEY_DEPTH_BITS);
  const bool msd = msd_possible && (defer_ev != nullptr ? defer_ev->bucket_sort : bucket_sort_allowed(true));
  int2* const mm_out = msd ? g.key_mm : nullptr;
#define GR_PRE(SH, COV, S16)                                                                       \
  if (S16 && num_views == 1)                                                                       \
    hipLaunchKernelGGL((preprocess_kernel<SH, COV, S16, S16>), grd, blk, 0, stream, (int)P, D, M, num_views, \
                       g.views, means3D, shs, colors_precomp, opacities, scales, rotations,        \
                       cov3D_precomp, W, H, radii, g.rec, g.dfield, g.rect_raw, g.totals + 2 * num_views, cam1, far_seq, \
                       mm_out);                                                                    \
  else if (msd && num_views > 4)                                                                   \
    hipLaunchKernelGGL((preprocess_many_kernel<SH, COV, S16>), grd, blk, 0, stream, (int)P, D, M, num_views, \
                       g.views, means3D, shs, colors_precomp, opacities, scales, rotations,        \
                       cov3D_precomp, W, H, radii, g.rec, g.dfield, g.rect_raw, g.totals + 2 * num_views, cam1, far_seq, \
                       mm_out);                                                                    \
  else                                                                                             \
  hipLaunchKernelGGL((preprocess_kernel<SH, COV, S16, false>), grd, blk, 0, stream, (int)P, D, M, num_views, \
                     g.views, means3D, shs, colors_precomp, opacities, scales, rotations,          \
                     cov3D_precomp, W, H, radii, g.rec, g.dfield, g.rect_raw, g.totals + 2 * num_views, cam1, far_seq, \
                     mm_out)
  auto run_preprocess = [&]() {
    KernelTimer timer("raster_preprocess", stream);
    if (shs && cov3D_precomp) { if (sh16) GR_PRE(true, true, true); else GR_PRE(true, true, false); }
    else if (shs) { if (sh16) GR_PRE(true, false, true); else GR_PRE(true, false, false); }
    else if (cov3D_precomp) GR_PRE(false, true, false);
    else GR_PRE(false, false, false);
  };
  run_preprocess();
  GR_LAUNCH_CHECK();
  int32_t* tot = static_cast<int32_t*>(pinned_scratch(1, sizeof(int32_t) * (2 * num_views + 2)));
  GR_REQUIRE(tot != nullptr, "pinned read-back buffer could not be allocated");
  const int nchunk = (int)((P + BIN_CHUNK - 1) / BIN_CHUNK);
  int32_t h_chunk_max = 0;
  auto sort_and_count = [&](int key_bits, bool buckets = true) -> int {
    bool totals_sorted = false;
    {
      KernelTimer timer("raster_depth_sort", stream);
      const bool msd_now = msd && buckets && key_bits == KEY_DEPTH_BITS;
      const bool self_seg = msd_now && defer_ev != nullptr && defer_ev->mail != nullptr && nchunk <= SCAN_SINGLE_ROW &&
                            num_views <= 4;
      totals_sorted = msd_now && num_views > 4;
      const DepthSortTotals ct{g.chunk_total, BIN_CHUNK, nchunk, g.rec, gx, gy};
      int rcs = depth_sort_views(g.dfield, g.rect_raw, g.keys_a, g.keys_b, g.order_b, g.rects, g.nvis, P, num_views, key_bits,
                                 g.ds_table, g.ds_table_bytes, stream, msd_now ? g.key_mm : nullptr,
                                 num_views > 4 ? (int)((P + 255) / 256) * (256 / WAVE) : (int)((P + 255) / 256),
                                 g.totals + 2 * num_views, defer_ev != nullptr ? -far_seq : 2,
                                 self_seg || totals_sorted ? &ct : nullptr);
      if (rcs != GR_OK) return rcs;
      if (self_seg) {
        defer_ev->by_mail = true;
        defer_ev->self_seg = true;
        return GR_OK;
      }
    }
    {
      KernelTimer timer("raster_bin", stream);
      const bool short_rows = nchunk <= SCAN_SINGLE_ROW;
      if (!bin_scans_self(nchunk, num_views)) {
        if (tiles * sizeof(unsigned int) > 64 * 1024)
          GR_HIP(hipFuncSetAttribute(reinterpret_cast<const void*>(tile_count_kernel),
                                     hipFuncAttributeMaxDynamicSharedMemorySize, 160 * 1024));
        hipLaunchKernelGGL(tile_count_kernel, dim3((unsigned)bin_grid(num_views, nchunk)), dim3(BIN_T),
                           tiles * sizeof(unsigned int), stream, (int)P, num_views, gx, gy, nchunk, g.nvis, g.rects, g.order_b,
                           g.rec, g.chunk_cnt, g.chunk_total);
        const bool by_mail = defer_ev != nullptr && defer_ev->mail != nullptr;
        hipLaunchKernelGGL(seg_scan_kernel<true>, dim3((unsigned)(num_views * nchunk)), blk, 0, stream, num_views, tiles, nchunk,
                           g.chunk_cnt, g.chunk_total, g.totals, g.seg_off, by_mail ? const_cast<int32_t*>(defer_ev->mail) : nullptr,
                           by_mail ? defer_ev->seq : 0);
        if (by_mail) defer_ev->by_mail = true;
        GR_LAUNCH_CHECK();
      } else {
        if (!totals_sorted)
          hipLaunchKernelGGL(chunk_total_kernel, dim3((unsigned)bin_grid(num_views, nchunk)), dim3(BIN_T), 0, stream, (int)P,
                             num_views, gx, gy, nchunk, g.nvis, g.rects, g.order_b, g.rec, g.chunk_total);
        if (!short_rows)
          hipLaunchKernelGGL(chunk_max_kernel, dim3(1), dim3(1024), 0, stream, num_views * nchunk, g.chunk_total, g.chunk_max);
        GR_LAUNCH_CHECK();
        int rcs = exclusive_scan_i32(g.chunk_total, g.chunk_total + (int64_t)num_views * nchunk, nchunk, num_views, nchunk,
                                     g.scan_ws, g.totals, stream, nullptr, short_rows ? g.totals + num_views : nullptr);
        if (rcs != GR_OK) return rcs;
      }
    }
    const bool short_rows = nchunk <= SCAN_SINGLE_ROW;
    if (defer_ev != nullptr) {
      if (defer_ev->by_mail) return GR_OK;
      static thread_local hipStream_t side = nullptr;
      static thread_local hipEvent_t counted = nullptr;
      if (side == nullptr) GR_HIP(hipStreamCreateWithFlags(&side, hipStreamNonBlocking));
      if (counted == nullptr) GR_HIP(hipEventCreateWithFlags(&counted, hipEventDisableTiming));
      GR_HIP(hipEventRecord(counted, stream));
      GR_HIP(hipStreamWaitEvent(side, counted, 0));
      GR_HIP(hipMemcpyAsync(tot, g.totals, sizeof(int32_t) * (2 * num_views + 1), hipMemcpyDeviceToHost, side));
      if (!short_rows)
        GR_HIP(hipMemcpyAsync(tot + 2 * num_views + 1, g.chunk_max, sizeof(int32_t), hipMemcpyDeviceToHost, side));
      GR_HIP(hipEventRecord(defer_ev->ev, side));
      return GR_OK;
    }
    GR_HIP(hipMemcpyAsync(tot, g.totals, sizeof(int32_t) * (2 * num_views + 1), hipMemcpyDeviceToHost, stream));
    if (!short_rows)
      GR_HIP(hipMemcpyAsync(tot + 2 * num_views + 1, g.chunk_max, sizeof(int32_t), hipMemcpyDeviceToHost, stream));
    GR_HIP(hipStreamSynchronize(stream));
    h_chunk_max = short_rows ? tot[num_views] : tot[2 * num_views + 1];
    if (short_rows)
      for (int v = 1; v < num_views; ++v) h_chunk_max = std::max(h_chunk_max, tot[num_views + v]);
    return GR_OK;
  };
  rc = sort_and_count(KEY_DEPTH_BITS);
  if (rc != GR_OK) return rc;
  if (defer_ev != nullptr) return GR_OK;
  auto check_depth_order = [&]() -> int {
    if (!verify_this_frame()) return GR_OK;
    int h_bad = 0;
    int rcv = device_check(stream, [&](int* d_bad) {
      hipLaunchKernelGGL(verify_depth_order_kernel, dim3((unsigned)std::min<int64_t>((P + 255) / 256, 4096), num_views), blk, 0,
                         stream, (int)P, num_views, g.nvis, g.dfield, g.order_b, reinterpret_cast<int32_t*>(g.keys_a), d_bad);
    }, &h_bad);
    if (rcv != GR_OK) return rcv;
    if (h_bad != 0 && lds_atomics_lane_ordered_state() == 1) {
      lds_order_demote();
      return 1;
    }
    GR_REQUIRE(h_bad == 0, "depth sort produced an unsorted order (internal error)");
    return GR_OK;
  };
  if (tot[2 * num_views] & 2) {
    bucket_sort_overflowed();
    GR_HIP(hipMemsetD32Async(reinterpret_cast<hipDeviceptr_t>(g.totals + 2 * num_views), tot[2 * num_views] & 1, 1, stream));
    rc = sort_and_count(KEY_DEPTH_BITS, false);
    if (rc != GR_OK) return rc;
  }
  if (tot[2 * num_views] != 0) {
    hipLaunchKernelGGL(full_keys_kernel, dim3((unsigned)((P * num_views + 255) / 256)), blk, 0, stream, P * num_views,
                       g.rec, radii, g.dfield);
    GR_LAUNCH_CHECK();
    rc = sort_and_count(32);
    if (rc != GR_OK) return rc;
  }
  rc = check_depth_order();
  if (rc == 1) {
    rc = sort_and_count(tot[2 * num_views] != 0 ? 32 : KEY_DEPTH_BITS, false);
    if (rc != GR_OK) return rc;
    rc = check_depth_order();
    if (rc == 1) rc = GR_OK;
  }
  if (rc != GR_OK) return rc;
#undef GR_PRE
  for (int v = 0; v < num_views; ++v) h_num_rendered[v] = tot[v];
  h_num_rendered[num_views] = h_chunk_max;
  return GR_OK;
}

extern "C" int gr_raster_render(int64_t P, const gr_raster_view* h_views, int num_views,
                                const int64_t* h_num_rendered, const void* geom, size_t geom_bytes,
                                void* bin, size_t bin_bytes, float* out_color, void* stream_) {
  static const int env_flags = (getenv("GR_RASTER_FAST_EXP") && getenv("GR_RASTER_FAST_EXP")[0] == '1') ? GR_RASTER_FAST_EXP : 0;
  return gr_raster_render_ex(P, h_views, num_views, h_num_rendered, geom, geom_bytes, bin, bin_bytes, out_color, env_flags,
                             stream_);
}

extern "C" int gr_raster_preprocess(int64_t P, int M, const float* means3D, const float* shs,
                                    const float* colors_precomp, const float* opacities,
                                    const float* scales, const float* rotations,
                                    const float* cov3D_precomp, const gr_raster_view* h_views,
                                    int num_views, int32_t* radii, void* geom, size_t geom_bytes,
                                    int64_t* h_num_rendered, void* stream_) {
  return preprocess_impl(P, M, means3D, shs, colors_precomp, opacities, scales, rotations, cov3D_precomp, h_views, num_views,
                         radii, geom, geom_bytes, h_num_rendered, static_cast<hipStream_t>(stream_), nullptr);
}

static int preprocess_collect(int64_t P, int num_views, int64_t* h_num_rendered, bool* far_depth, Deferred& d, hipStream_t stream,
                              bool* bucket_overflow = nullptr) {
  const int nchunk = (int)((P + BIN_CHUNK - 1) / BIN_CHUNK);
  if (d.by_mail) {
    const volatile int32_t* m = d.mail;
    bool ready = false;
    for (unsigned long spin = 1; !ready; ++spin) {
      ready = true;
      for (int v = 0; v < num_views; ++v) ready = ready && __atomic_load_n(&m[2 * num_views + 1 + v], __ATOMIC_ACQUIRE) == d.seq;
      if (!ready && (spin & 0xffff) == 0 && hipStreamQuery(stream) != hipErrorNotReady) {
        ready = true;
        for (int v = 0; v < num_views; ++v) ready = ready && __atomic_load_n(&m[2 * num_views + 1 + v], __ATOMIC_ACQUIRE) == d.seq;
        GR_HIP(hipStreamSynchronize(stream));
        GR_REQUIRE(ready, "rasterizer: the counting kernel did not report its totals");
      }
    }
    int32_t cm = m[num_views];
    for (int v = 1; v < num_views; ++v) {
      const int32_t mv = m[num_views + v];
      cm = std::max(cm, mv);
    }
    for (int v = 0; v < num_views; ++v) h_num_rendered[v] = m[v];
    h_num_rendered[num_views] = cm;
    *far_depth = m[2 * num_views] == d.far_seq || m[2 * num_views] == -d.far_seq;
    if (bucket_overflow) *bucket_overflow = m[2 * num_views] == -d.far_seq;
    return GR_OK;
  }
  GR_HIP(hipEventSynchronize(d.ev));
  const int32_t* tot = static_cast<const int32_t*>(pinned_scratch(1, sizeof(int32_t) * (2 * num_views + 2)));
  GR_REQUIRE(tot != nullptr, "pinned read-back buffer missing");
  const bool short_rows = nchunk <= SCAN_SINGLE_ROW;
  int32_t cm = short_rows ? tot[num_views] : tot[2 * num_views + 1];
  if (short_rows)
    for (int v = 1; v < num_views; ++v) cm = std::max(cm, tot[num_views + v]);
  for (int v = 0; v < num_views; ++v) h_num_rendered[v] = tot[v];
  h_num_rendered[num_views] = cm;
  *far_depth = tot[2 * num_views] != 0;
  if (bucket_overflow) *bucket_overflow = tot[2 * num_views] < 0;
  return GR_OK;
}

static int render_impl(int64_t P, const gr_raster_view* h_views, int num_views, const int64_t* h_num_rendered,
                       const void* geom, size_t geom_bytes, void* bin, size_t bin_bytes, float* out_color, int flags,
                       int64_t spec_entries, hipStream_t stream, const Deferred* defer = nullptr, bool keep = false,
                       float* out_depth = nullptr, float* out_alpha = nullptr, float* aux_state = nullptr) {
  int rc = check_views(h_views, num_views);
  if (rc != GR_OK) return rc;
  GR_REQUIRE(out_color != nullptr && h_num_rendered != nullptr, "null argument");
  const bool spec = spec_entries >= 0;
  const int W = h_views[0].image_width, H = h_views[0].image_height;
  const int gx = (W + TILE - 1) / TILE, gy = (H + TILE - 1) / TILE;
  const int64_t vtiles = (int64_t)gx * gy * num_views;
  GR_REQUIRE(vtiles < (1ll << 31), "too many tiles");
  int64_t R = 0;
  if (spec) R = spec_entries;
  else
    for (int v = 0; v < num_views; ++v) R += h_num_rendered[v];
  GR_REQUIRE(R < (1ll << 31) - 1, "too many rendered instances (%lld)", (long long)R);
  const int tiles = gx * gy;
  Geom g = carve_geom(const_cast<void*>(geom), P, num_views, tiles);
  GR_REQUIRE(P == 0 || (geom && geom_bytes >= g.bytes), "geometry buffer missing or too small");
  Bin b = carve_bin(bin, R, vtiles);
  if (!bin || bin_bytes < b.bytes) {
    set_error("raster binning buffer too small: need %zu bytes, got %zu", b.bytes, bin_bytes);
    return GR_ERR_WORKSPACE;
  }
  const int32_t* point_list = b.point_list;
  const int nchunk = (int)((P + BIN_CHUNK - 1) / BIN_CHUNK);
  const unsigned int list_cap = spec ? (unsigned int)R : 0xffffffffu;
  if (R > 0 || (spec && P > 0)) {
    const bool wide = num_views <= 4 && (size_t)(WIDE_T / WAVE) * tiles * sizeof(unsigned int) <= 100 * 1024;
    const int scatter_threads = wide ? WIDE_T : BIN_T;
    const size_t cur_bytes = (size_t)(scatter_threads / WAVE) * ((tiles + 1) & ~1) * sizeof(unsigned short);
    int64_t lds_budget = wide ? 156 * 1024 : 160 * 1024 / SCATTER_WGS - 512;
    if (lds_budget < (int64_t)cur_bytes + 8 * 1024) lds_budget = 78 * 1024;
    const int64_t cap_max = (lds_budget - (int64_t)cur_bytes) / 2;
    int64_t want = std::max<int64_t>(h_num_rendered[num_views], 0);
    if (spec) want = want > 0 ? want + 64 : cap_max;
    int stage_cap = (int)std::min<int64_t>(std::max<int64_t>(cap_max, 0), (want + 63) / 64 * 64);
    constexpr int ELIST = 1024;
    const size_t base_lds = cur_bytes + ((size_t)stage_cap * sizeof(unsigned short) + 3) / 4 * 4;
    const int elist_cap = tiles >= 4096 && base_lds + (size_t)(scatter_threads / WAVE) * ELIST * 4 <= 156 * 1024 ? ELIST : 0;
    const size_t lds = base_lds + (size_t)(scatter_threads / WAVE) * elist_cap * 4;
    bool ordered = false;
    rc = lds_atomics_lane_ordered(stream, &ordered);
    if (rc != GR_OK) return rc;
    const bool self_seg = spec && defer != nullptr && defer->self_seg;
    const int seg_mode = self_seg ? SEG_SELF_RAW : bin_scans_self(nchunk, num_views) ? SEG_SELF_SCAN : SEG_READ;
    const SelfSeg self{g.chunk_total, g.totals, self_seg ? const_cast<int32_t*>(defer->mail) : nullptr, self_seg ? defer->seq : 0};
    auto pick = [&](bool lane_ordered) {
#define GR_SCATTER(LO, S) (wide ? tile_scatter_kernel<LO, WIDE_T, S> : tile_scatter_kernel<LO, BIN_T, S>)
      if (lane_ordered)
        return seg_mode == SEG_SELF_RAW ? GR_SCATTER(true, SEG_SELF_RAW)
               : seg_mode == SEG_SELF_SCAN ? GR_SCATTER(true, SEG_SELF_SCAN) : GR_SCATTER(true, SEG_READ);
      return seg_mode == SEG_SELF_RAW ? GR_SCATTER(false, SEG_SELF_RAW)
             : seg_mode == SEG_SELF_SCAN ? GR_SCATTER(false, SEG_SELF_SCAN) : GR_SCATTER(false, SEG_READ);
#undef GR_SCATTER
    };
    auto kern = pick(ordered);
    int tile_bits = 0;
    while ((1 << tile_bits) < tiles) ++tile_bits;
    if (lds > 64 * 1024)
      GR_HIP(hipFuncSetAttribute(reinterpret_cast<const void*>(kern), hipFuncAttributeMaxDynamicSharedMemorySize,
                                 160 * 1024 - 512));
    {
      KernelTimer timer("raster_bin", stream);
      hipLaunchKernelGGL(kern, dim3((unsigned)bin_grid(num_views, nchunk)), dim3(scatter_threads), lds, stream, (int)P, num_views, gx, gy,
                         nchunk, tile_bits, stage_cap, g.nvis, g.rects, g.order_b, g.rec, g.seg_off, b.point_list, list_cap, elist_cap,
                         self);
      GR_LAUNCH_CHECK();
    }
    if (!spec && verify_this_frame()) {
      int h_bad = 0;
      rc = device_check(stream, [&](int* d_bad) {
        hipLaunchKernelGGL(verify_tile_lists_kernel, dim3((unsigned)(num_views * nchunk)), dim3(256), 0, stream, (int)P, num_views,
                           nchunk, tiles, g.seg_off, b.point_list, reinterpret_cast<const int32_t*>(g.keys_a), d_bad);
      }, &h_bad);
      if (rc != GR_OK) return rc;
      if (h_bad != 0 && ordered) {
        lds_order_demote();
        auto kern_b = pick(false);
        if (lds > 64 * 1024)
          GR_HIP(hipFuncSetAttribute(reinterpret_cast<const void*>(kern_b), hipFuncAttributeMaxDynamicSharedMemorySize,
                                     160 * 1024 - 512));
        hipLaunchKernelGGL(kern_b, dim3((unsigned)bin_grid(num_views, nchunk)), dim3(scatter_threads), lds, stream, (int)P,
                           num_views, gx, gy, nchunk, tile_bits, stage_cap, g.nvis, g.rects, g.order_b, g.rec, g.seg_off,
                           b.point_list, list_cap, elist_cap, self);
        GR_LAUNCH_CHECK();
      } else {
        GR_REQUIRE(h_bad == 0, "tile binning produced an unsorted list (internal error)");
      }
    }
  }
  KernelTimer timer("raster_blend", stream);
  const bool fast = (flags & GR_RASTER_FAST_EXP) != 0;
  const int blend_chunks = (R > 0 || (spec && P > 0)) ? nchunk : 0;
  const size_t blend_pad = (spec && (flags & GR_RASTER_SHARE)) ? 14000 : 0;
#define GR_BLEND(FE, KEEP)                                                                                            \
  hipLaunchKernelGGL((blend_kernel<FE, KEEP>), dim3(gx, gy, num_views), dim3(BLOCK), blend_pad, stream, (int)P, W, H,      \
                     blend_chunks, g.views, g.seg_off, point_list, g.rec, out_color, list_cap, BlendAux<false>{})
#define GR_BLEND_AUX(FE, KEEP)                                                                                        \
  hipLaunchKernelGGL((blend_kernel<FE, KEEP, true>), dim3(gx, gy, num_views), dim3(BLOCK), 0, stream, (int)P, W, H,        \
                     blend_chunks, g.views, g.seg_off, point_list, g.rec, out_color, list_cap,                           \
                     BlendAux<true>{out_depth, out_alpha, aux_state})
  if (out_depth != nullptr) {
    if (keep) { if (fast) GR_BLEND_AUX(true, true); else GR_BLEND_AUX(false, true); }
    else if (fast) GR_BLEND_AUX(true, false); else GR_BLEND_AUX(false, false);
  }
  else if (keep) { if (fast) GR_BLEND(true, true); else GR_BLEND(false, true); }
  else if (fast) GR_BLEND(true, false); else GR_BLEND(false, false);
#undef GR_BLEND
#undef GR_BLEND_AUX
  GR_LAUNCH_CHECK();
  frame_done();
  return GR_OK;
}

extern "C" int gr_raster_render_ex(int64_t P, const gr_raster_view* h_views, int num_views,
                                   const int64_t* h_num_rendered, const void* geom, size_t geom_bytes,
                                   void* bin, size_t bin_bytes, float* out_color, int flags, void* stream_) {
  return render_impl(P, h_views, num_views, h_num_rendered, geom, geom_bytes, bin, bin_bytes, out_color, flags, -1,
                     static_cast<hipStream_t>(stream_));
}

extern "C" int gr_raster_render_keep(int64_t P, const gr_raster_view* h_views, int num_views,
                                     const int64_t* h_num_rendered, const void* geom, size_t geom_bytes,
                                     void* bin, size_t bin_bytes, float* out_state, int flags, void* stream_) {
  return render_impl(P, h_views, num_views, h_num_rendered, geom, geom_bytes, bin, bin_bytes, out_state, flags, -1,
                     static_cast<hipStream_t>(stream_), nullptr, true);
}

extern "C" int gr_raster_render_aux(int64_t P, const gr_raster_view* h_views, int num_views,
                                    const int64_t* h_num_rendered, const void* geom, size_t geom_bytes,
                                    void* bin, size_t bin_bytes, float* out_color, float* out_depth, float* out_alpha,
                                    float* out_state, int flags, void* stream_) {
  GR_REQUIRE(out_depth != nullptr && out_alpha != nullptr, "out_depth / out_alpha is null");
  return render_impl(P, h_views, num_views, h_num_rendered, geom, geom_bytes, bin, bin_bytes, out_color, flags, -1,
                     static_cast<hipStream_t>(stream_), nullptr, out_state != nullptr, out_depth, out_alpha, out_state);
}

namespace gr {
namespace {
struct Pending {
  bool open;
  int64_t P;
  int num_views;
  int64_t entries;
  Deferred d;
  hipStream_t stream;
};
thread_local Pending g_pending{false, 0, 0, 0, Deferred{nullptr, nullptr, 0, 0, false, false, false}, nullptr};
}
}

extern "C" int gr_raster_debug_bucket_cooldown(int set) {
  const int left = gr::g_bucket_cooldown;
  if (set >= 0) gr::g_bucket_cooldown = set;
  return left;
}

extern "C" int gr_raster_forward_finish(int64_t* h_num_rendered) {
  using namespace gr;
  GR_REQUIRE(g_pending.open, "gr_raster_forward_finish: no split gr_raster_forward is open on this thread");
  GR_REQUIRE(h_num_rendered != nullptr, "h_num_rendered is null");
  Pending p = g_pending;
  g_pending.open = false;
  bool far_depth = false, bucket_overflow = false;
  int rc = preprocess_collect(p.P, p.num_views, h_num_rendered, &far_depth, p.d, p.stream, &bucket_overflow);
  if (rc != GR_OK) return rc;
  if (bucket_overflow) bucket_sort_overflowed();
  int64_t R = 0;
  for (int v = 0; v < p.num_views; ++v) R += h_num_rendered[v];
  if (far_depth) return GR_RETRY_FULL;
  return R <= p.entries ? GR_OK : GR_RETRY_BIN;
}

extern "C" int gr_raster_forward(int64_t P, int M, const float* means3D, const float* shs, const float* colors_precomp,
                                 const float* opacities, const float* scales, const float* rotations,
                                 const float* cov3D_precomp, const gr_raster_view* h_views, int num_views, int32_t* radii,
                                 void* geom, size_t geom_bytes, void* bin, size_t bin_bytes, float* out_color, int flags,
                                 int64_t* h_num_rendered, void* stream_) {
  hipStream_t stream = static_cast<hipStream_t>(stream_);
  GR_REQUIRE(h_num_rendered != nullptr, "h_num_rendered is null");
  GR_REQUIRE(!g_pending.open, "gr_raster_forward: the previous split call of this thread was not finished");
  const int64_t stage_hint = h_num_rendered[num_views > 0 ? num_views : 0];
  const int64_t entries = bin && bin_bytes > 512 ? (int64_t)((bin_bytes - 512) / sizeof(int32_t)) - 64 : -1;
  if (P > 0 && num_views <= 4 && entries > 0 && entries < (1ll << 31) - 1 && !verify_this_frame()) {
    static thread_local hipEvent_t ev = nullptr;
    if (ev == nullptr) GR_HIP(hipEventCreateWithFlags(&ev, hipEventDisableTiming));
    static thread_local int32_t* mail = nullptr;
    if (mail == nullptr) {
      static const bool no_mail = getenv("GR_NO_MAILBOX") && getenv("GR_NO_MAILBOX")[0] == '1';
      void* mp = nullptr;
      if (!no_mail && hipHostMalloc(&mp, 4096, hipHostMallocMapped | hipHostMallocCoherent) == hipSuccess) {
        memset(mp, 0, 4096);
        mail = static_cast<int32_t*>(mp);
      } else {
        (void)hipGetLastError();
      }
    }
    static std::atomic<int> frame_seq{0};
    int seq = frame_seq.fetch_add(1) + 1;
    if (seq > 0x7ffffff0) {
      frame_seq.store(1);
      seq = 1;
    }
    Deferred d{ev, mail, seq, 1, false, bucket_sort_allowed(depth_sort_msd_possible(P, num_views, KEY_DEPTH_BITS)), false};
    int rc = preprocess_impl(P, M, means3D, shs, colors_precomp, opacities, scales, rotations, cov3D_precomp, h_views,
                             num_views, radii, geom, geom_bytes, h_num_rendered, stream, &d);
    if (rc != GR_OK) return rc;
    h_num_rendered[num_views] = stage_hint;
    rc = render_impl(P, h_views, num_views, h_num_rendered, geom, geom_bytes, bin, bin_bytes, out_color, flags, entries, stream,
                     &d);
    if (rc != GR_OK) return rc;
    if (flags & GR_RASTER_SPLIT) {
      g_pending = Pending{true, P, num_views, entries, d, stream};
      return GR_PENDING;
    }
    bool far_depth = false, bucket_overflow = false;
    rc = preprocess_collect(P, num_views, h_num_rendered, &far_depth, d, stream, &bucket_overflow);
    if (rc != GR_OK) return rc;
    if (bucket_overflow) bucket_sort_overflowed();
    int64_t R = 0;
    for (int v = 0; v < num_views; ++v) R += h_num_rendered[v];
    if (!far_depth) return R <= entries ? GR_OK : GR_RETRY_BIN;
  }
  int rc = gr_raster_preprocess(P, M, means3D, shs, colors_precomp, opacities, scales, rotations, cov3D_precomp, h_views,
                                num_views, radii, geom, geom_bytes, h_num_rendered, stream);
  if (rc != GR_OK) return rc;
  int64_t R = 0;
  for (int v = 0; v < num_views; ++v) R += h_num_rendered[v];
  if (bin == nullptr || bin_bytes < gr_raster_bin_bytes(R, h_views[0].image_width, h_views[0].image_height, num_views))
    return GR_RETRY_BIN;
  return gr_raster_render_ex(P, h_views, num_views, h_num_rendered, geom, geom_bytes, bin, bin_bytes, out_color, flags, stream);
}

extern "C" int gr_raster_mark_visible(int64_t P, const float* means3D, const float* h_viewmatrix,
                                      uint8_t* present, void* stream_) {
  hipStream_t stream = static_cast<hipStream_t>(stream_);
  GR_REQUIRE(P >= 0 && h_viewmatrix != nullptr, "bad argument");
  if (P == 0) return GR_OK;
  GR_REQUIRE(means3D && present, "null argument");
  hipLaunchKernelGGL(mark_visible_kernel, dim3((unsigned)((P + 255) / 256)), dim3(256), 0, stream, (int)P, means3D,
                     h_viewmatrix[2], h_viewmatrix[6], h_viewmatrix[10], h_viewmatrix[14], present);
  GR_LAUNCH_CHECK();
  return GR_OK;
}
```

### gaussreg_amd/csrc/rasterizer_backward.hip

```cpp
#include <algorithm>
#include <type_traits>

#include "raster_shared.hpp"

namespace gr {
namespace {

constexpr int NF = 9;
constexpr int NF_AUX = 10;
constexpr int NWAVE = BLOCK / WAVE;

__device__ __forceinline__ float wave_sum_f32_dpp(float x) {
#define GR_F32_STEP(CTRL, ROWMASK) x += __int_as_float(__builtin_amdgcn_update_dpp(0, __float_as_int(x), CTRL, ROWMASK, 0xf, false));
  GR_F32_STEP(0x111, 0xf) GR_F32_STEP(0x112, 0xf) GR_F32_STEP(0x114, 0xf) GR_F32_STEP(0x118, 0xf)
  GR_F32_STEP(0x142, 0xa) GR_F32_STEP(0x143, 0xc)
#undef GR_F32_STEP
  return __int_as_float(__builtin_amdgcn_readlane(__float_as_int(x), 63));
}

__global__ __launch_bounds__(256) void slot_count_kernel(int64_t n, int P, int gx, int gy, const uint32_t* __restrict__ rect_raw,
                                                         const float4* __restrict__ rec, int32_t* __restrict__ slot_local,
                                                         int32_t* __restrict__ block_sum) {
  __shared__ int s_w[256 / WAVE];
  const int64_t o = (int64_t)blockIdx.x * 256 + threadIdx.x;
  int area = 0;
  if (o < n) {
    const uint32_t r = rect_raw[o];
    int x0, y0, w, h;
    const int64_t vbase = o / P * P;
    if (r != 0u && rect_decode(r, (int)(o - vbase), vbase, rec, gx, gy, x0, y0, w, h)) area = w * h;
  }
  const int lane = threadIdx.x & (WAVE - 1), wv = threadIdx.x / WAVE;
  const int incl = wave_incl_scan_add_dpp(area);
  if (lane == WAVE - 1) s_w[wv] = incl;
  __syncthreads();
  int before = 0;
  for (int w = 0; w < wv; ++w) before += s_w[w];
  if (o < n) slot_local[o] = before + incl - area;
  if (threadIdx.x == 0) block_sum[blockIdx.x] = s_w[0] + s_w[1] + s_w[2] + s_w[3];
}

__global__ __launch_bounds__(1024) void slot_block_scan_kernel(int nb, int32_t* __restrict__ block_pre) {
  __shared__ int s_w[1024 / WAVE];
  __shared__ int s_carry;
  const int lane = threadIdx.x & (WAVE - 1), wv = threadIdx.x / WAVE;
  if (threadIdx.x == 0) s_carry = 0;
  __syncthreads();
  for (int b0 = 0; b0 < nb; b0 += 1024) {
    const int b = b0 + threadIdx.x;
    const int x = b < nb ? block_pre[b] : 0;
    const int incl = wave_incl_scan_add_dpp(x);
    if (lane == WAVE - 1) s_w[wv] = incl;
    __syncthreads();
    int base = s_carry;
    for (int w = 0; w < wv; ++w) base += s_w[w];
    if (b < nb) block_pre[b] = base + incl - x;
    __syncthreads();
    if (threadIdx.x == 1023) s_carry = base + incl;
    __syncthreads();
  }
  if (threadIdx.x == 0) block_pre[nb] = s_carry;
}

template <bool AUX>
struct RenderBwdAux {};
template <>
struct RenderBwdAux<true> {
  const float* dL_ddepth;
  const float* dL_dalpha;
};

template <bool FAST_EXP, bool AUX = false>
__global__ __launch_bounds__(BLOCK) void render_backward_kernel(
    int P, int W, int H, int nchunk, const DevView* __restrict__ views, const uint32_t* __restrict__ seg_off,
    const int32_t* __restrict__ point_list, const float4* __restrict__ rec, const uint32_t* __restrict__ rect_raw,
    const int32_t* __restrict__ slot_local, const int32_t* __restrict__ block_pre, int64_t slot_cap,
    const float* __restrict__ final_T, const int32_t* __restrict__ n_contrib, const float* __restrict__ dL_dpix,
    float* __restrict__ slots, RenderBwdAux<AUX> aux) {
  constexpr int NF = AUX ? NF_AUX : gr::NF;
  using mask_t = typename std::conditional<AUX, unsigned char, unsigned int>::type;
  __shared__ float s_e[AUX ? 11 : 10][BLOCK];
  __shared__ int64_t s_slot[AUX ? 1 : BLOCK];
  int64_t my_slot = -1;
  __shared__ mask_t s_wmask[BLOCK];
  __shared__ float s_part[NWAVE][BLOCK][NF];
  __shared__ int s_wpre[WAVE];
  __shared__ unsigned int s_woff[WAVE];
  __shared__ int s_max[NWAVE];
  const int gx = (W + TILE - 1) / TILE, gy = (H + TILE - 1) / TILE;
  const int v = blockIdx.z;
  const int tile = blockIdx.y * gx + blockIdx.x;
  const int tid = threadIdx.x;
  const int lane = tid & (WAVE - 1), lw = tid / WAVE;
  constexpr int CELL = 4;
  const int cell = tid / (CELL * CELL), pin = tid % (CELL * CELL);
  const int lx = (cell % (TILE / CELL)) * CELL + pin % CELL;
  const int ly = (cell / (TILE / CELL)) * CELL + pin / CELL;
  const int pxi = blockIdx.x * TILE + lx, pyi = blockIdx.y * TILE + ly;
  const bool inside = pxi < W && pyi < H;
  const float pfx = (float)pxi, pfy = (float)pyi;
  const float tx0 = (float)(blockIdx.x * TILE), ty0 = (float)(blockIdx.y * TILE);
  const int tiles = gx * gy;
  const int64_t vbase = (int64_t)v * P;
  const int64_t q = ((int64_t)v * H + (inside ? pyi : 0)) * W + (inside ? pxi : 0);
  const int64_t hw = (int64_t)H * W;
  const float T_final = inside ? final_T[q] : 0.0f;
  const int last = inside ? n_contrib[q] : 0;
  float g[3] = {0.f, 0.f, 0.f};
  if (inside && (!AUX || dL_dpix != nullptr)) {
    const float* gp = dL_dpix + (int64_t)v * 3 * hw + (int64_t)pyi * W + pxi;
    g[0] = gp[0];
    g[1] = gp[hw];
    g[2] = gp[2 * hw];
  }
  float g_d = 0.f, g_a = 0.f, accum_d = 0.f, last_z = 0.f;
  if constexpr (AUX) {
    if (inside && aux.dL_ddepth != nullptr) g_d = aux.dL_ddepth[q];
    if (inside && aux.dL_dalpha != nullptr) g_a = aux.dL_dalpha[q];
  }
  const DevView& cam = views[v];
  const float bg_dot = cam.bg[0] * g[0] + cam.bg[1] * g[1] + cam.bg[2] * g[2];
  float T = T_final, accum[3] = {0.f, 0.f, 0.f}, last_col[3] = {0.f, 0.f, 0.f}, last_alpha = 0.f;
  const int wmax = wave_max_i32_dpp(last);
  if (lane == 0) s_max[lw] = wmax;
  __syncthreads();
  const int max_n = max(max(s_max[0], s_max[1]), max(s_max[2], s_max[3]));
  if (max_n == 0 || nchunk == 0) return;
  const uint32_t* seg_col = seg_off + (int64_t)v * nchunk * (tiles + 1) + tile;
  auto load_window = [&](int c0) -> int {
    if (tid < WAVE) {
      const int c = c0 + tid;
      unsigned int a = 0u, b = 0u;
      if (c < nchunk) {
        a = seg_col[(int64_t)c * (tiles + 1)];
        b = seg_col[(int64_t)c * (tiles + 1) + 1];
      }
      s_woff[tid] = a;
      s_wpre[tid] = wave_incl_scan_add_dpp((int)(b - a));
    }
    __syncthreads();
    return s_wpre[WAVE - 1];
  };
  int c0 = 0, base = 0, w_total = 0;
  while (true) {
    w_total = load_window(c0);
    __syncthreads();
    if (base + w_total >= max_n || c0 + WAVE >= nchunk) break;
    base += w_total;
    c0 += WAVE;
  }
  int hi = min(max_n - base, w_total);
  while (true) {
    while (hi > 0) {
      const int lo = max(0, hi - BLOCK), n = hi - lo;
      if (tid < n) {
        const int e = lo + tid;
        int l = 0;
#pragma unroll
        for (int st = WAVE / 2; st > 0; st >>= 1)
          if (s_wpre[l + st - 1] <= e) l += st;
        const int before = l ? s_wpre[l - 1] : 0;
        const int id = point_list[s_woff[l] + (unsigned int)(e - before)];
        const float4* r = rec + 4 * (vbase + id);
        const float4 r0 = r[0], co = r[1], col = r[2];
        const float pc = -__logf(255.0f * co.w) - 1.0e-3f;
        const float rc2 = -pc * col.w;
        const float cpr = -pc + 1.0e-3f + 2.0e-6f * rc2;
        const float hx2 = cpr * r0.z, hy2 = cpr * r0.w;
        s_e[0][tid] = r0.x;
        s_e[1][tid] = r0.y;
        s_e[2][tid] = pc;
        s_e[3][tid] = co.x;
        s_e[4][tid] = co.y;
        s_e[5][tid] = co.z;
        s_e[6][tid] = co.w;
        s_e[7][tid] = col.x;
        s_e[8][tid] = col.y;
        s_e[9][tid] = col.z;
        if constexpr (AUX) s_e[10][tid] = r[3].y;
        const float ex = fmaxf(fmaxf(tx0 - r0.x, r0.x - (tx0 + (float)(TILE - 1))), 0.0f);
        unsigned int m = 0u;
#pragma unroll
        for (int s = 0; s < NWAVE; ++s) {
          const float ylo = ty0 + (float)(s * CELL);
          const float ey = fmaxf(fmaxf(ylo - r0.y, r0.y - (ylo + (float)(CELL - 1))), 0.0f);
          if (!(ex * ex + ey * ey > rc2) && !(ex * ex > hx2) && !(ey * ey > hy2)) m |= 1u << s;
        }
        s_wmask[tid] = (mask_t)m;
        int x0, y0, w, h;
        int64_t slot = -1;
        if (rect_decode(rect_raw[vbase + id], id, vbase, rec, gx, gy, x0, y0, w, h)) {
          const int64_t o = vbase + id;
          slot = (int64_t)slot_local[o] + block_pre[o >> 8] + (int64_t)((int)blockIdx.y - y0) * w + ((int)blockIdx.x - x0);
        }
        if (AUX) my_slot = slot; else s_slot[tid] = slot;
      }
      __syncthreads();
      for (int j = n - 1; j >= 0; --j) {
        float* part = s_part[lw][j];
        if (!((s_wmask[j] >> lw) & 1u)) {
          if (lane < NF) part[lane] = 0.0f;
          continue;
        }
        const int gidx = base + lo + j;
        const float dx = s_e[0][j] - pfx, dy = s_e[1][j] - pfy;
        const float cx = s_e[3][j], cy = s_e[4][j], cz = s_e[5][j], op = s_e[6][j];
        const float qf = fmaf(cx * dx, dx, (cz * dy) * dy);
        const float power = fmaf(-0.5f, qf, -((cy * dx) * dy));
        const float G = FAST_EXP ? __builtin_amdgcn_exp2f(power * 1.44269504088896341f) : exp_det(power);
        const float alpha = fminf(op * G, 0.99f);
        const bool hit = inside && gidx < last && !(power > 0.0f) && !(power < s_e[2][j]) && !(alpha < 1.0f / 255.0f);
        float val[NF];
#pragma unroll
        for (int f = 0; f < NF; ++f) val[f] = 0.0f;
        if (hit) {
          T = T / (1.0f - alpha);
          const float dchannel_dcolor = alpha * T;
          float dL_dalpha = 0.0f;
#pragma unroll
          for (int ch = 0; ch < 3; ++ch) {
            const float c = s_e[7 + ch][j];
            accum[ch] = last_alpha * last_col[ch] + (1.0f - last_alpha) * accum[ch];
            last_col[ch] = c;
            dL_dalpha += (c - accum[ch]) * g[ch];
            val[6 + ch] = dchannel_dcolor * g[ch];
          }
          if constexpr (AUX) {
            const float z = s_e[10][j];
            accum_d = last_alpha * last_z + (1.0f - last_alpha) * accum_d;
            last_z = z;
            dL_dalpha += (z - accum_d) * g_d;
            val[9] = dchannel_dcolor * g_d;
          }
          dL_dalpha *= T;
          last_alpha = alpha;
          dL_dalpha += (-T_final / (1.0f - alpha)) * bg_dot;
          if constexpr (AUX) dL_dalpha += (T_final / (1.0f - alpha)) * g_a;
          const float dL_dG = op * dL_dalpha;
          const float gdx = G * dx, gdy = G * dy;
          val[0] = dL_dG * (-gdx * cx - gdy * cy);
          val[1] = dL_dG * (-gdy * cz - gdx * cy);
          val[2] = -0.5f * gdx * dx * dL_dG;
          val[3] = -gdx * dy * dL_dG;
          val[4] = -0.5f * gdy * dy * dL_dG;
          val[5] = G * dL_dalpha;
        }
        if (__ballot(hit) == 0ull) {
          if (lane < NF) part[lane] = 0.0f;
          continue;
        }
#pragma unroll
        for (int f = 0; f < NF; ++f) {
          const float s = wave_sum_f32_dpp(val[f]);
          if (lane == 0) part[f] = s;
        }
      }
      __syncthreads();
      if (tid < n) {
        const int64_t slot = AUX ? my_slot : s_slot[tid];
        if (slot >= 0 && slot < slot_cap) {
          float* dst = slots + NF * slot;
#pragma unroll
          for (int f = 0; f < NF; ++f)
            dst[f] = ((s_part[0][tid][f] + s_part[1][tid][f]) + s_part[2][tid][f]) + s_part[3][tid][f];
        }
      }
      __syncthreads();
      hi = lo;
    }
    if (c0 == 0) break;
    c0 -= WAVE;
    w_total = load_window(c0);
    base -= w_total;
    hi = w_total;
    __syncthreads();
  }
}

__device__ __forceinline__ void sh_basis_grad(int deg, float x, float y, float z, float* B, float* Bx, float* By, float* Bz) {
#pragma unroll
  for (int k = 0; k < 16; ++k) B[k] = Bx[k] = By[k] = Bz[k] = 0.0f;
  B[0] = SH_C0;
  if (deg > 0) {
    B[1] = -SH_C1 * y; By[1] = -SH_C1;
    B[2] = SH_C1 * z;  Bz[2] = SH_C1;
    B[3] = -SH_C1 * x; Bx[3] = -SH_C1;
    if (deg > 1) {
      const float xx = x * x, yy = y * y, zz = z * z, xy = x * y, yz = y * z, xz = x * z;
      B[4] = SH_C2[0] * xy;                 Bx[4] = SH_C2[0] * y;          By[4] = SH_C2[0] * x;
      B[5] = SH_C2[1] * yz;                 By[5] = SH_C2[1] * z;          Bz[5] = SH_C2[1] * y;
      B[6] = SH_C2[2] * (2.f * zz - xx - yy); Bx[6] = -2.f * SH_C2[2] * x; By[6] = -2.f * SH_C2[2] * y; Bz[6] = 4.f * SH_C2[2] * z;
      B[7] = SH_C2[3] * xz;                 Bx[7] = SH_C2[3] * z;          Bz[7] = SH_C2[3] * x;
      B[8] = SH_C2[4] * (xx - yy);          Bx[8] = 2.f * SH_C2[4] * x;    By[8] = -2.f * SH_C2[4] * y;
      if (deg > 2) {
        B[9] = SH_C3[0] * y * (3.f * xx - yy);
        Bx[9] = SH_C3[0] * 6.f * xy;            By[9] = SH_C3[0] * 3.f * (xx - yy);
        B[10] = SH_C3[1] * xy * z;
        Bx[10] = SH_C3[1] * yz;                 By[10] = SH_C3[1] * xz;            Bz[10] = SH_C3[1] * xy;
        B[11] = SH_C3[2] * y * (4.f * zz - xx - yy);
        Bx[11] = SH_C3[2] * -2.f * xy;          By[11] = SH_C3[2] * (4.f * zz - xx - 3.f * yy); Bz[11] = SH_C3[2] * 8.f * yz;
        B[12] = SH_C3[3] * z * (2.f * zz - 3.f * xx - 3.f * yy);
        Bx[12] = SH_C3[3] * -6.f * xz;          By[12] = SH_C3[3] * -6.f * yz;     Bz[12] = SH_C3[3] * (6.f * zz - 3.f * xx - 3.f * yy);
        B[13] = SH_C3[4] * x * (4.f * zz - xx - yy);
        Bx[13] = SH_C3[4] * (4.f * zz - 3.f * xx - yy); By[13] = SH_C3[4] * -2.f * xy; Bz[13] = SH_C3[4] * 8.f * xz;
        B[14] = SH_C3[5] * z * (xx - yy);
        Bx[14] = SH_C3[5] * 2.f * xz;           By[14] = SH_C3[5] * -2.f * yz;     Bz[14] = SH_C3[5] * (xx - yy);
        B[15] = SH_C3[6] * x * (xx - 3.f * yy);
        Bx[15] = SH_C3[6] * 3.f * (xx - yy);    By[15] = SH_C3[6] * -6.f * xy;
      }
    }
  }
}

struct BwdOut {
  float* means3D;
  float* means2D;
  float* shs;
  float* colors;
  float* opacity;
  float* scales;
  float* rotations;
  float* cov3D;
};

constexpr int NCAM = 27;
constexpr int NCAMF = 18;

struct PreBwdCam {
  float* partial;
};

template <bool HAS_SH, bool HAS_COV, bool AUX = false>
__global__ __launch_bounds__(256) void preprocess_backward_kernel(
    int P, int D, int M, int V, int W, int H, const DevView* __restrict__ views, const float* __restrict__ means3D,
    const float* __restrict__ shs, const float* __restrict__ scales, const float* __restrict__ rotations,
    const float* __restrict__ cov3D_precomp, const uint32_t* __restrict__ rect_raw, const float4* __restrict__ rec,
    const int32_t* __restrict__ slot_local, const int32_t* __restrict__ block_pre, int64_t slot_cap,
    const float* __restrict__ slots, BwdOut out) {
  constexpr bool CAM = false;
  const PreBwdCam cam_out{nullptr};
#define GR_PREPROCESS_BACKWARD_BODY_OK
#include "preprocess_backward_body.hpp"
#undef GR_PREPROCESS_BACKWARD_BODY_OK
}

template <bool HAS_SH, bool HAS_COV, bool AUX>
__global__ __launch_bounds__(256) void preprocess_backward_cam_kernel(
    int P, int D, int M, int V, int W, int H, const DevView* __restrict__ views, const float* __restrict__ means3D,
    const float* __restrict__ shs, const float* __restrict__ scales, const float* __restrict__ rotations,
    const float* __restrict__ cov3D_precomp, const uint32_t* __restrict__ rect_raw, const float4* __restrict__ rec,
    const int32_t* __restrict__ slot_local, const int32_t* __restrict__ block_pre, int64_t slot_cap,
    const float* __restrict__ slots, BwdOut out, PreBwdCam cam_out) {
  constexpr bool CAM = true;
#define GR_PREPROCESS_BACKWARD_BODY_OK
#include "preprocess_backward_body.hpp"
#undef GR_PREPROCESS_BACKWARD_BODY_OK
}

__global__ __launch_bounds__(1024) void camera_sum_kernel(int nb, const float* __restrict__ partial, float* __restrict__ dview,
                                                          float* __restrict__ dproj, float* __restrict__ dcampos) {
  __shared__ float s_row[32][32];
  __shared__ float s_tot[NCAM];
  const int v = blockIdx.x, f = threadIdx.x & 31, r = threadIdx.x >> 5;
  float acc = 0.0f;
  if (f < NCAM) {
    const float* src = partial + (int64_t)v * nb * NCAM + f;
    for (int b = r; b < nb; b += 32) acc += src[(int64_t)b * NCAM];
  }
  s_row[r][f] = acc;
  __syncthreads();
  if (threadIdx.x < NCAM) {
    float t = 0.0f;
    for (int k = 0; k < 32; ++k) t += s_row[k][threadIdx.x];
    s_tot[threadIdx.x] = t;
  }
  __syncthreads();
  const int t = threadIdx.x;
  if (t < 16) {
    const int j = t >> 2, c = t & 3;
    if (dview) dview[v * 16 + t] = c < 3 ? s_tot[3 * j + c] : 0.0f;
    if (dproj) dproj[v * 16 + t] = c == 2 ? 0.0f : s_tot[12 + 3 * j + (c == 3 ? 2 : c)];
  } else if (t < 19 && dcampos) {
    dcampos[v * 3 + (t - 16)] = s_tot[24 + (t - 16)];
  }
}

struct BwdScratch {
  int32_t* slot_local;
  int32_t* block_pre;
  float* slots;
  float* cam_partial;
  size_t bytes;
};

BwdScratch carve_bwd(void* p, int64_t P, int V, int64_t R, int nf = NF, bool cam = false) {
  BwdScratch s;
  Carver c(p);
  s.slot_local = c.take<int32_t>(P * V);
  s.block_pre = c.take<int32_t>((P * V + 255) / 256 + 1);
  s.slots = c.take<float>(R * nf);
  s.cam_partial = cam ? c.take<float>((P + 255) / 256 * V * NCAM) : nullptr;
  s.bytes = c.used();
  return s;
}

int64_t total_rendered(const int64_t* h_num_rendered, int V) {
  int64_t R = 0;
  for (int v = 0; v < V; ++v) R += std::max<int64_t>(h_num_rendered[v], 0);
  return R;
}

}
}

using namespace gr;

extern "C" size_t gr_raster_backward_bytes(int64_t P, int num_views, int width, int height, const int64_t* h_num_rendered) {
  if (P < 0 || num_views < 1 || width <= 0 || height <= 0 || h_num_rendered == nullptr) return 0;
  return carve_bwd(nullptr, P, num_views, total_rendered(h_num_rendered, num_views)).bytes;
}

extern "C" size_t gr_raster_backward_aux_bytes(int64_t P, int num_views, int width, int height,
                                               const int64_t* h_num_rendered) {
  if (P < 0 || num_views < 1 || width <= 0 || height <= 0 || h_num_rendered == nullptr) return 0;
  return carve_bwd(nullptr, P, num_views, total_rendered(h_num_rendered, num_views), NF_AUX).bytes;
}

extern "C" size_t gr_raster_backward_cam_bytes(int64_t P, int num_views, int width, int height,
                                               const int64_t* h_num_rendered, int flags) {
  if (P < 0 || num_views < 1 || width <= 0 || height <= 0 || h_num_rendered == nullptr) return 0;
  const int nf = (flags & GR_RASTER_BWD_COLOR_ONLY) ? NF : NF_AUX;
  return carve_bwd(nullptr, P, num_views, total_rendered(h_num_rendered, num_views), nf, true).bytes;
}

struct CamGrads {
  float* view = nullptr;
  float* proj = nullptr;
  float* campos = nullptr;
  bool any() const { return view != nullptr || proj != nullptr || campos != nullptr; }
};

static int backward_impl(bool aux, const CamGrads& cam, const float* dL_ddepth, const float* dL_dalpha, int64_t P, int M,
                         const float* means3D,
                         const float* shs, const float* colors_precomp, const float* opacities, const float* scales,
                         const float* rotations, const float* cov3D_precomp, const gr_raster_view* h_views, int num_views,
                         const void* geom, size_t geom_bytes, const void* bin, size_t bin_bytes,
                         const int64_t* h_num_rendered, const float* final_T, const int32_t* n_contrib,
                         const float* dL_dcolor, int flags, float* dL_dmeans3D, float* dL_dmeans2D, float* dL_dshs,
                         float* dL_dcolors, float* dL_dopacity, float* dL_dscales, float* dL_drotations, float* dL_dcov3D,
                         void* scratch, size_t scratch_bytes, void* stream_) {
  hipStream_t stream = static_cast<hipStream_t>(stream_);
  GR_REQUIRE(h_views != nullptr && num_views >= 1 && num_views <= MAX_VIEWS, "need 1 .. %d views", MAX_VIEWS);
  GR_REQUIRE(h_num_rendered != nullptr, "h_num_rendered is null");
  GR_REQUIRE(P >= 0 && P < (1ll << 31) - 1, "P out of range");
  const int W = h_views[0].image_width, H = h_views[0].image_height, D = h_views[0].sh_degree;
  for (int v = 0; v < num_views; ++v)
    GR_REQUIRE(h_views[v].image_width == W && h_views[v].image_height == H && h_views[v].sh_degree == D,
               "all views of one call must share image size and sh_degree");
  GR_REQUIRE(W > 0 && H > 0 && D >= 0 && D <= 3, "bad image size or sh_degree");
  if (P == 0) {
    if (cam.view) GR_HIP(hipMemsetAsync(cam.view, 0, sizeof(float) * 16 * num_views, stream));
    if (cam.proj) GR_HIP(hipMemsetAsync(cam.proj, 0, sizeof(float) * 16 * num_views, stream));
    if (cam.campos) GR_HIP(hipMemsetAsync(cam.campos, 0, sizeof(float) * 3 * num_views, stream));
    return GR_OK;
  }
  GR_REQUIRE(means3D != nullptr, "means3D is null");
  GR_REQUIRE((shs != nullptr) != (colors_precomp != nullptr), "exactly one of shs / colors_precomp");
  GR_REQUIRE((scales != nullptr && rotations != nullptr) != (cov3D_precomp != nullptr),
             "exactly one of (scales, rotations) / cov3D_precomp");
  if (shs) GR_REQUIRE(M >= (D + 1) * (D + 1), "shs has %d coefficients, sh_degree %d needs %d", M, D, (D + 1) * (D + 1));
  const int gx = (W + TILE - 1) / TILE, gy = (H + TILE - 1) / TILE;
  const int tiles = gx * gy;
  const int64_t R = total_rendered(h_num_rendered, num_views);
  GR_REQUIRE(R < (1ll << 31) - 1, "too many rendered instances");
  const Geom g = carve_geom(const_cast<void*>(geom), P, num_views, tiles);
  GR_REQUIRE(geom != nullptr && geom_bytes >= g.bytes, "geometry buffer missing or too small");
  const Bin bn = carve_bin(const_cast<void*>(bin), R, (int64_t)tiles * num_views);
  GR_REQUIRE(R == 0 || (bin != nullptr && bin_bytes >= bn.bytes), "binning buffer missing or too small");
  GR_REQUIRE(R == 0 || (final_T != nullptr && n_contrib != nullptr && (aux || dL_dcolor != nullptr)), "null per-pixel state");
  const int nf = aux ? NF_AUX : NF;
  const BwdScratch s = carve_bwd(scratch, P, num_views, R, nf, cam.any());
  if (!scratch || scratch_bytes < s.bytes) {
    set_error("raster backward scratch too small: need %zu bytes, got %zu", s.bytes, scratch_bytes);
    return GR_ERR_WORKSPACE;
  }
  const int64_t n = P * num_views;
  const int nb = (int)((n + 255) / 256);
  {
    KernelTimer timer("raster_bwd_slots", stream);
    hipLaunchKernelGGL(slot_count_kernel, dim3((unsigned)nb), dim3(256), 0, stream, n, (int)P, gx, gy, g.rect_raw, g.rec,
                       s.slot_local, s.block_pre);
    GR_LAUNCH_CHECK();
    hipLaunchKernelGGL(slot_block_scan_kernel, dim3(1), dim3(1024), 0, stream, nb, s.block_pre);
    GR_LAUNCH_CHECK();
    int32_t* h_tot = static_cast<int32_t*>(pinned_scratch(9, sizeof(int32_t)));
    GR_REQUIRE(h_tot != nullptr, "pinned read-back buffer could not be allocated");
    *h_tot = -1;
    GR_HIP(hipMemcpyAsync(h_tot, s.block_pre + nb, sizeof(int32_t), hipMemcpyDeviceToHost, stream));
    GR_HIP(hipStreamSynchronize(stream));
    const int32_t h_total = *h_tot;
    GR_REQUIRE(h_total == R, "raster backward: the tile rectangles hold %d instances, the forward binned %lld (geom / "
               "h_num_rendered not from the same forward call?)", h_total, (long long)R);
    if (R > 0) GR_HIP(hipMemsetAsync(s.slots, 0, sizeof(float) * nf * R, stream));
  }
  const int nchunk = (int)((P + BIN_CHUNK - 1) / BIN_CHUNK);
  if (R > 0) {
    KernelTimer timer("raster_bwd_render", stream);
#define GR_RBWD(FE, AUX, ...)                                                                                              \
  hipLaunchKernelGGL((render_backward_kernel<FE, AUX>), dim3(gx, gy, num_views), dim3(BLOCK), 0, stream, (int)P, W, H, nchunk, \
                     g.views, g.seg_off, bn.point_list, g.rec, g.rect_raw, s.slot_local, s.block_pre, R, final_T, n_contrib,  \
                     dL_dcolor, s.slots, RenderBwdAux<AUX>{__VA_ARGS__})
    const bool fast = (flags & GR_RASTER_FAST_EXP) != 0;
    if (aux) { if (fast) GR_RBWD(true, true, dL_ddepth, dL_dalpha); else GR_RBWD(false, true, dL_ddepth, dL_dalpha); }
    else if (fast) GR_RBWD(true, false); else GR_RBWD(false, false);
#undef GR_RBWD
    GR_LAUNCH_CHECK();
  }
  const BwdOut out{dL_dmeans3D, dL_dmeans2D, dL_dshs, dL_dcolors, dL_dopacity, dL_dscales, dL_drotations, dL_dcov3D};
  {
    KernelTimer timer("raster_bwd_preprocess", stream);
    const dim3 grd((unsigned)((P + 255) / 256)), blk(256);
    const size_t cam_lds = sizeof(float) * NCAM * 4 * num_views;
#define GR_PBWD_(SH, COV, AUX)                                                                                            \
  do {                                                                                                                    \
    if (cam.any())                                                                                                        \
      hipLaunchKernelGGL((preprocess_backward_cam_kernel<SH, COV, AUX>), grd, blk, cam_lds, stream, (int)P, D, M,         \
                         num_views, W, H, g.views, means3D, shs, scales, rotations, cov3D_precomp, g.rect_raw, g.rec,     \
                         s.slot_local, s.block_pre, R, s.slots, out, PreBwdCam{s.cam_partial});                     \
    else                                                                                                                  \
      hipLaunchKernelGGL((preprocess_backward_kernel<SH, COV, AUX>), grd, blk, 0, stream, (int)P, D, M, num_views, W, H,  \
                         g.views, means3D, shs, scales, rotations, cov3D_precomp, g.rect_raw, g.rec, s.slot_local,        \
                         s.block_pre, R, s.slots, out);                                                                   \
  } while (0)
#define GR_PBWD(SH, COV) do { if (aux) GR_PBWD_(SH, COV, true); else GR_PBWD_(SH, COV, false); } while (0)
    if (shs && cov3D_precomp) GR_PBWD(true, true);
    else if (shs) GR_PBWD(true, false);
    else if (cov3D_precomp) GR_PBWD(false, true);
    else GR_PBWD(false, false);
#undef GR_PBWD
#undef GR_PBWD_
    GR_LAUNCH_CHECK();
    if (cam.any()) {
      hipLaunchKernelGGL(camera_sum_kernel, dim3((unsigned)num_views), dim3(1024), 0, stream, (int)grd.x, s.cam_partial,
                         cam.view, cam.proj, cam.campos);
      GR_LAUNCH_CHECK();
    }
  }
  (void)opacities;
  return GR_OK;
}

extern "C" int gr_raster_backward(int64_t P, int M, const float* means3D, const float* shs, const float* colors_precomp,
                                  const float* opacities, const float* scales, const float* rotations,
                                  const float* cov3D_precomp, const gr_raster_view* h_views, int num_views, const void* geom,
                                  size_t geom_bytes, const void* bin, size_t bin_bytes, const int64_t* h_num_rendered,
                                  const float* final_T, const int32_t* n_contrib, const float* dL_dcolor, int flags,
                                  float* dL_dmeans3D, float* dL_dmeans2D, float* dL_dshs, float* dL_dcolors,
                                  float* dL_dopacity, float* dL_dscales, float* dL_drotations, float* dL_dcov3D,
                                  void* scratch, size_t scratch_bytes, void* stream_) {
  return backward_impl(false, CamGrads{}, nullptr, nullptr, P, M, means3D, shs, colors_precomp, opacities, scales, rotations,
                       cov3D_precomp, h_views, num_views, geom, geom_bytes, bin, bin_bytes, h_num_rendered, final_T, n_contrib,
                       dL_dcolor, flags, dL_dmeans3D, dL_dmeans2D, dL_dshs, dL_dcolors, dL_dopacity, dL_dscales,
                       dL_drotations, dL_dcov3D, scratch, scratch_bytes, stream_);
}

extern "C" int gr_raster_backward_aux(int64_t P, int M, const float* means3D, const float* shs, const float* colors_precomp,
                                      const float* opacities, const float* scales, const float* rotations,
                                      const float* cov3D_precomp, const gr_raster_view* h_views, int num_views,
                                      const void* geom, size_t geom_bytes, const void* bin, size_t bin_bytes,
                                      const int64_t* h_num_rendered, const float* final_T, const int32_t* n_contrib,
                                      const float* dL_dcolor, const float* dL_ddepth, const float* dL_dalpha, int flags,
                                      float* dL_dmeans3D, float* dL_dmeans2D, float* dL_dshs, float* dL_dcolors,
                                      float* dL_dopacity, float* dL_dscales, float* dL_drotations, float* dL_dcov3D,
                                      void* scratch, size_t scratch_bytes, void* stream_) {
  return backward_impl(true, CamGrads{}, dL_ddepth, dL_dalpha, P, M, means3D, shs, colors_precomp, opacities, scales, rotations,
                       cov3D_precomp, h_views, num_views, geom, geom_bytes, bin, bin_bytes, h_num_rendered, final_T, n_contrib,
                       dL_dcolor, flags, dL_dmeans3D, dL_dmeans2D, dL_dshs, dL_dcolors, dL_dopacity, dL_dscales,
                       dL_drotations, dL_dcov3D, scratch, scratch_bytes, stream_);
}

extern "C" int gr_raster_backward_cam(int64_t P, int M, const float* means3D, const float* shs, const float* colors_precomp,
                                      const float* opacities, const float* scales, const float* rotations,
                                      const float* cov3D_precomp, const gr_raster_view* h_views, int num_views,
                                      const void* geom, size_t geom_bytes, const void* bin, size_t bin_bytes,
                                      const int64_t* h_num_rendered, const float* final_T, const int32_t* n_contrib,
                                      const float* dL_dcolor, const float* dL_ddepth, const float* dL_dalpha, int flags,
                                      float* dL_dmeans3D, float* dL_dmeans2D, float* dL_dshs, float* dL_dcolors,
                                      float* dL_dopacity, float* dL_dscales, float* dL_drotations, float* dL_dcov3D,
                                      float* dL_dviewmatrix, float* dL_dprojmatrix, float* dL_dcampos, void* scratch,
                                      size_t scratch_bytes, void* stream_) {
  const bool colour_only = (flags & GR_RASTER_BWD_COLOR_ONLY) != 0;
  if (colour_only && (dL_ddepth != nullptr || dL_dalpha != nullptr)) {
    set_error("gr_raster_backward_cam: GR_RASTER_BWD_COLOR_ONLY takes no dL_ddepth / dL_dalpha");
    return GR_ERR_INVALID;
  }
  CamGrads cam;
  cam.view = dL_dviewmatrix, cam.proj = dL_dprojmatrix, cam.campos = dL_dcampos;
  return backward_impl(!colour_only, cam, dL_ddepth, dL_dalpha, P, M, means3D, shs, colors_precomp, opacities, scales,
                       rotations, cov3D_precomp, h_views, num_views, geom, geom_bytes, bin, bin_bytes, h_num_rendered,
                       final_T, n_contrib, dL_dcolor, flags, dL_dmeans3D, dL_dmeans2D, dL_dshs, dL_dcolors, dL_dopacity,
                       dL_dscales, dL_drotations, dL_dcov3D, scratch, scratch_bytes, stream_);
}
```

### gaussreg_amd/rasterizer.py

```python
import ctypes
import os
import threading
from typing import NamedTuple, Optional, Sequence

import torch

from . import _lib


class GaussianRasterizationSettings(NamedTuple):
    image_height: int
    image_width: int
    tanfovx: float
    tanfovy: float
    bg: torch.Tensor
    scale_modifier: float
    viewmatrix: torch.Tensor
    projmatrix: torch.Tensor
    sh_degree: int
    campos: torch.Tensor
    prefiltered: bool
    debug: bool


FAST_EXP, SPLIT, SHARE, BWD_COLOR_ONLY = (_lib.DEFINES["GR_RASTER_" + f] for f in ("FAST_EXP", "SPLIT", "SHARE", "BWD_COLOR_ONLY"))
_ENV_FAST = None
_bin_hint = {}


def _flags(fast_exp):
    global _ENV_FAST
    if fast_exp is None:
        if _ENV_FAST is None:
            _ENV_FAST = os.environ.get("GR_RASTER_FAST_EXP", "0")[:1] == "1"
        fast_exp = _ENV_FAST
    return FAST_EXP if fast_exp else 0


def _view_struct(rs: GaussianRasterizationSettings) -> _lib.RasterView:
    v = _lib.RasterView()
    v.image_height, v.image_width = int(rs.image_height), int(rs.image_width)
    v.tanfovx, v.tanfovy = float(rs.tanfovx), float(rs.tanfovy)
    v.scale_modifier = float(rs.scale_modifier)
    v.sh_degree = int(rs.sh_degree)
    v.prefiltered, v.debug = int(bool(rs.prefiltered)), int(bool(rs.debug))
    bg = rs.bg.detach().to("cpu", torch.float32).reshape(-1).tolist()
    vm = rs.viewmatrix.detach().to("cpu", torch.float32).reshape(-1).tolist()
    pm = rs.projmatrix.detach().to("cpu", torch.float32).reshape(-1).tolist()
    cp = rs.campos.detach().to("cpu", torch.float32).reshape(-1).tolist()
    if len(bg) != 3 or len(vm) != 16 or len(pm) != 16 or len(cp) != 3:
        raise ValueError("bg/campos must have 3 elements, viewmatrix/projmatrix 16")
    v.bg[:] = bg
    v.viewmatrix[:] = vm
    v.projmatrix[:] = pm
    v.campos[:] = cp
    return v


class ViewBatch:

    def __init__(self, settings: Sequence[GaussianRasterizationSettings]):
        if len(settings) < 1:
            raise ValueError("need at least one view")
        self.count = len(settings)
        self.height, self.width = int(settings[0].image_height), int(settings[0].image_width)
        self.array = (_lib.RasterView * self.count)(*[_view_struct(s) for s in settings])
        self.cameras = tuple((s.viewmatrix, s.projmatrix, s.campos) for s in settings)

    def wants_grad(self):
        return torch.is_grad_enabled() and any(t.requires_grad for cam in self.cameras for t in cam)

    def camera_inputs(self, dev):
        out = []
        for k, shape in enumerate(((4, 4), (4, 4), (3,))):
            ts = [cam[k] for cam in self.cameras]
            if not any(t.requires_grad for t in ts):
                out.append(None)
                continue
            out.append(torch.stack([t.to(device=dev, dtype=torch.float32).reshape(shape) for t in ts]))
        return out


def _dev_f32(t: Optional[torch.Tensor], dev, name, grad=False):
    if t is None:
        return None
    if not isinstance(t, torch.Tensor):
        raise TypeError(f"{name} must be a tensor")
    if grad:
        return t.to(device=dev, dtype=torch.float32).contiguous()
    if t.device == dev and t.dtype == torch.float32 and t.is_contiguous():
        return t
    return t.detach().to(device=dev, dtype=torch.float32).contiguous()


class _FramePipe:

    def __init__(self, dev):
        self.streams = tuple(torch.cuda.Stream(dev) for _ in range(2))
        self.turn = 0
        self.stamp = None
        self.keep = None
        self.caller = None
        self.ready = None
        self.ptrs = None
        self.overlapping = False

    def begin(self, dev, inputs):
        cur = torch.cuda.current_stream(dev)
        side = self.streams[self.turn]
        stamp = _lib.tensor_stamp(inputs)
        self.overlapping = False
        if stamp is not None and stamp == self.stamp and self.caller == cur.cuda_stream and self.ready is not None:
            side.wait_event(self.ready)
            self.overlapping = True
        else:
            side.wait_stream(cur)
            self.ptrs = None
            self.ready = None
            if stamp is not None:
                self.ready = torch.cuda.Event()
                self.ready.record(cur)
        self.stamp, self.keep, self.caller = stamp, inputs, cur.cuda_stream
        return cur, side

    def abort(self, cur, side):
        self.stamp = self.keep = self.ready = self.ptrs = None
        cur.wait_stream(side)

    def end(self, cur, side, outputs):
        self.turn = (self.turn + 1) % len(self.streams)
        cur.wait_stream(side)
        for t in outputs:
            t.record_stream(cur)


_pipes = threading.local()


def _frame_pipe(dev, static_scene):
    env = os.environ.get("GR_RASTER_PIPELINE")
    if env == "0" or not (static_scene or env == "1"):
        return None
    table = getattr(_pipes, "table", None)
    if table is None:
        table = _pipes.table = {}
    p = table.get(dev.index)
    if p is None:
        p = table[dev.index] = _FramePipe(dev)
    return p


_geom_bytes = {}


def _geom_size(L, P, V, W, H):
    gkey = (P, V, W, H)
    gbytes = _geom_bytes.get(gkey)
    if gbytes is None:
        if len(_geom_bytes) > 64:
            _geom_bytes.clear()
        gbytes = _geom_bytes[gkey] = L.gr_raster_geom_bytes(P, V, W, H) + 256
    return gbytes


def reset_frame_pipe():
    table = getattr(_pipes, "table", None)
    if table:
        for p in table.values():
            p.stamp = p.keep = p.ready = p.ptrs = None


_SCENE = ("means3D", "shs", "colors_precomp", "opacities", "scales", "rotations", "cov3D_precomp")
_GRADS = ("means3D", "means2D") + _SCENE[1:]
_CAMERA = ("viewmatrix", "projmatrix", "campos")
_CAMERA_SHAPES = ((4, 4), (4, 4), (3,))
_ARGS = ("vb", "flags", "aux", "one", "box", "means2D") + _SCENE + _CAMERA
_BACKWARD = {(False, False): "gr_raster_backward", (True, False): "gr_raster_backward_aux",
             (False, True): "gr_raster_backward_cam", (True, True): "gr_raster_backward_cam"}


def _sh_coeffs(sh, P):
    return 0 if sh is None else (sh.shape[1] if sh.dim() == 3 else sh.reshape(max(P, 1), -1, 3).shape[1])


def _render_serial(vb, flags, one, inputs, aux, keep):
    m = inputs[0]
    dev = m.device
    L = _lib.lib()
    V, views, H, W = vb.count, vb.array, vb.height, vb.width
    P = m.shape[0]
    M = _sh_coeffs(inputs[1], P)
    st = _lib.stream_ptr(dev)
    nr = (ctypes.c_int64 * (V + 1))()
    hw = H * W
    if aux:
        color = torch.empty((3, H, W) if one else (V, 3, H, W), dtype=torch.float32, device=dev)
        depth = torch.empty((1, H, W) if one else (V, 1, H, W), dtype=torch.float32, device=dev)
        alpha = torch.empty_like(depth)
        state = torch.empty(2 * V * hw, dtype=torch.float32, device=dev) if keep else None
    else:
        block = torch.empty(5 * V * hw, dtype=torch.float32, device=dev)
    radii = torch.empty((P,) if one else (V, P), dtype=torch.int32, device=dev)
    gbytes = _geom_size(L, P, V, W, H)
    geom = torch.empty(gbytes, dtype=torch.uint8, device=dev)
    _lib.check(L.gr_raster_preprocess(P, M, *map(_lib.ptr, inputs), views, V, _lib.ptr(radii), _lib.ptr(geom), gbytes, nr,
                                      st))
    binb = torch.empty(L.gr_raster_bin_bytes(sum(nr[:V]), W, H, V) + 256, dtype=torch.uint8, device=dev)
    shared = (P, views, V, nr, _lib.ptr(geom), gbytes, _lib.ptr(binb), binb.numel())
    if aux:
        _lib.check(L.gr_raster_render_aux(*shared, _lib.ptr(color), _lib.ptr(depth), _lib.ptr(alpha), _lib.ptr(state), flags,
                                          st))
        return (color, radii, depth, alpha), nr, (M, geom, binb, state)
    _lib.check(L.gr_raster_render_keep(*shared, _lib.ptr(block), flags, st))
    color = block[:3 * V * hw].view((3, H, W) if one else (V, 3, H, W)).clone()
    return (color, radii), nr, (M, geom, binb, block[3 * V * hw:])


class _Rasterize(torch.autograd.Function):

    @staticmethod
    def forward(ctx, vb, flags, aux, one, box, means2D, *scene_and_cameras):
        inputs = scene_and_cameras[:len(_SCENE)]
        outs, nr, (ctx.M, ctx.geom, ctx.binb, ctx.state) = _render_serial(vb, flags, one, inputs, aux, True)
        ctx.vb, ctx.flags, ctx.aux, ctx.nr = vb, flags, aux, nr
        ctx.m2d = None if means2D is None else (means2D.shape, means2D.dtype, means2D.device)
        ctx.save_for_backward(*inputs)
        ctx.mark_non_differentiable(outs[1])
        box.extend(nr[:vb.count])
        return outs

    @staticmethod
    @torch.autograd.function.once_differentiable
    def backward(ctx, grad_color, grad_radii, grad_depth=None, grad_alpha=None):
        inputs = ctx.saved_tensors
        dev = inputs[0].device
        L = _lib.lib()
        vb, aux = ctx.vb, ctx.aux
        V, H, W = vb.count, vb.height, vb.width
        P = inputs[0].shape[0]
        need = dict(zip(_ARGS, ctx.needs_input_grad))
        if grad_color is None and not aux:
            grad_color = torch.zeros((V, 3, H, W), dtype=torch.float32, device=dev)
        gc, gd, ga = (None if g is None else g.to(device=dev, dtype=torch.float32).contiguous()
                      for g in (grad_color, grad_depth, grad_alpha))
        grads = dict.fromkeys(_ARGS)
        for name, t in zip(_SCENE, inputs):
            if t is not None and need[name]:
                grads[name] = torch.empty_like(t)
        if need["means2D"]:
            grads["means2D"] = torch.empty((V, P, 3), dtype=torch.float32, device=dev)
        cam = False
        for name, shape in zip(_CAMERA, _CAMERA_SHAPES):
            if need[name]:
                cam = True
                grads[name] = torch.empty((V,) + shape, dtype=torch.float32, device=dev)
        hw = H * W
        final_T, n_contrib = ctx.state[:V * hw], ctx.state[V * hw:]
        entry = _BACKWARD[aux, cam]
        color_only = BWD_COLOR_ONLY if cam and not aux else 0
        maps = (_lib.ptr(gd), _lib.ptr(ga)) if aux or cam else ()
        outs = [_lib.ptr(grads[name]) for name in (_GRADS + _CAMERA if cam else _GRADS)]
        with torch.cuda.device(dev):
            sbytes = getattr(L, entry + "_bytes")(P, V, W, H, ctx.nr, *((color_only,) if cam else ())) + 256
            scratch = torch.empty(sbytes, dtype=torch.uint8, device=dev)
            _lib.check(getattr(L, entry)(
                P, ctx.M, *map(_lib.ptr, inputs), vb.array, V, _lib.ptr(ctx.geom), ctx.geom.numel(), _lib.ptr(ctx.binb),
                ctx.binb.numel(), ctx.nr, _lib.ptr(final_T), _lib.ptr(n_contrib), _lib.ptr(gc), *maps,
                ctx.flags | color_only, *outs,
                _lib.ptr(scratch), scratch.numel(), _lib.stream_ptr(dev)))
        if grads["means2D"] is not None:
            shape, dtype, device = ctx.m2d
            grads["means2D"] = grads["means2D"].reshape(shape).to(device=device, dtype=dtype)
        return tuple([grads[name] for name in _ARGS])


def _wants_grad(*ts):
    return torch.is_grad_enabled() and any(isinstance(t, torch.Tensor) and t.requires_grad for t in ts)


def _render_pipelined(vb, flags, one, inputs, static_scene):
    m, sh, cp, op, sc, rot, cov = inputs
    dev = m.device
    L = _lib.lib()
    V, views, H, W = vb.count, vb.array, vb.height, vb.width
    P = m.shape[0]
    M = _sh_coeffs(sh, P)
    nr = (ctypes.c_int64 * (V + 1))()
    pipe = _frame_pipe(dev, static_scene)
    cur = side = None
    home = torch.cuda.current_device()
    if home != dev.index:
        torch.cuda.set_device(dev)
    try:
        if pipe is not None:
            cur, side = pipe.begin(dev, tuple(t for t in (m, op, sh, cp, sc, rot, cov) if t is not None))
            torch.cuda.set_stream(side)
            st = ctypes.c_void_p(side.cuda_stream)
        else:
            st = _lib.stream_ptr(dev)
        color = torch.empty((3, H, W) if one else (V, 3, H, W), dtype=torch.float32, device=dev)
        radii = torch.empty((P,) if one else (V, P), dtype=torch.int32, device=dev)
        gbytes = _geom_size(L, P, V, W, H)
        geom = torch.empty(gbytes, dtype=torch.uint8, device=dev)
        key = (dev.index, P, V, W, H)
        hint, chunk_hint = _bin_hint.get(key, (0, 0))
        binb = torch.empty(hint + 256, dtype=torch.uint8, device=dev) if hint else None
        nr[V] = chunk_hint

        if pipe is not None and pipe.ptrs is not None:
            ptrs = pipe.ptrs
        else:
            ptrs = (_lib.ptr(m), _lib.ptr(sh), _lib.ptr(cp), _lib.ptr(op), _lib.ptr(sc), _lib.ptr(rot), _lib.ptr(cov))
            if pipe is not None:
                pipe.ptrs = ptrs

        def forward(fl):
            return L.gr_raster_forward(P, M, *ptrs, views, V, _lib.ptr(radii), _lib.ptr(geom), gbytes, _lib.ptr(binb),
                                       hint + 256 if binb is not None else 0, _lib.ptr(color), fl, nr, st)
        rc = forward(flags | ((SPLIT | (SHARE if pipe.overlapping and V == 1 else 0)) if pipe is not None else 0))
        joined = rejoin = False
        if rc == _lib.GR_PENDING:
            try:
                torch.cuda.set_stream(cur)
                pipe.end(cur, side, (color, radii))
                joined = True
            finally:
                rc = L.gr_raster_forward_finish(nr)
            if rc in (_lib.GR_RETRY_BIN, _lib.GR_RETRY_FULL):
                torch.cuda.set_stream(side)
                rejoin = True
            if rc == _lib.GR_RETRY_FULL:
                rc = forward(flags)
        _lib.check(rc, allow=(_lib.GR_RETRY_BIN,))
        need = L.gr_raster_bin_bytes(sum(nr[:V]), W, H, V)
        if rc == _lib.GR_RETRY_BIN:
            binb = torch.empty(need + 256, dtype=torch.uint8, device=dev)
            _lib.check(L.gr_raster_render_ex(P, views, V, nr, _lib.ptr(geom), geom.numel(), _lib.ptr(binb), binb.numel(),
                                             _lib.ptr(color), flags, st))
        if len(_bin_hint) > 64:
            _bin_hint.clear()
        _bin_hint[key] = (need + need // 4 + 1024, int(nr[V]))
        if pipe is not None:
            torch.cuda.set_stream(cur)
            if not joined:
                pipe.end(cur, side, (color, radii))
            elif rejoin:
                cur.wait_stream(side)
    except BaseException:
        if pipe is not None and cur is not None:
            torch.cuda.set_stream(cur)
            pipe.abort(cur, side)
        raise
    finally:
        if home != dev.index:
            torch.cuda.set_device(home)
    return color, radii, nr[:V]


def rasterize_views(settings, means3D, opacities, shs=None,
                    colors_precomp=None, scales=None, rotations=None, cov3D_precomp=None, fast_exp=None, _one=False,
                    static_scene=False, *, means2D=None, render_depth=False):
    dev = means3D.device if means3D.is_cuda else _lib.require_gpu()
    n_pts = int(means3D.shape[0])

    def given(t):
        return t is not None and (t.numel() > 0 or n_pts == 0)

    has_sh, has_cp = given(shs), given(colors_precomp)
    has_sc, has_rot, has_cov = given(scales), given(rotations), given(cov3D_precomp)
    if has_sh == has_cp:
        raise Exception('Please provide excatly one of either SHs or precomputed colors!')
    has_sr = has_sc and has_rot
    if has_sr == has_cov or has_sc != has_rot:
        raise Exception('Please provide exactly one of either scale/rotation pair or precomputed 3D covariance!')
    vb = settings if isinstance(settings, ViewBatch) else ViewBatch(settings)
    cam_grad = vb.wants_grad()
    grad = cam_grad or _wants_grad(means3D, means2D, opacities, shs, colors_precomp, scales, rotations, cov3D_precomp)
    if means3D.dim() != 2 or means3D.shape[1] != 3:
        raise RuntimeError("means3D must have dimensions (num_points, 3)")
    if grad and means2D is not None:
        ok = (tuple(means2D.shape) == (vb.count, n_pts, 3) or
              (vb.count == 1 and tuple(means2D.shape) == (n_pts, 3)))
        if not ok:
            raise ValueError(f"means2D must have shape ({vb.count}, {n_pts}, 3)" +
                             (f" or ({n_pts}, 3)" if vb.count == 1 else "") + f", got {tuple(means2D.shape)}")
    inputs = (_dev_f32(means3D, dev, "means3D", grad),
              _dev_f32(shs, dev, "shs", grad) if has_sh else None,
              _dev_f32(colors_precomp, dev, "colors_precomp", grad) if has_cp else None,
              _dev_f32(opacities, dev, "opacities", grad),
              _dev_f32(scales, dev, "scales", grad) if has_sr else None,
              _dev_f32(rotations, dev, "rotations", grad) if has_sr else None,
              _dev_f32(cov3D_precomp, dev, "cov3D_precomp", grad) if has_cov else None)
    flags, one = _flags(fast_exp), _one and vb.count == 1
    if not (grad or render_depth):
        return _render_pipelined(vb, flags, one, inputs, static_scene)
    home = torch.cuda.current_device()
    if home != dev.index:
        torch.cuda.set_device(dev)
    try:
        if grad:
            num_rendered = []
            outs = _Rasterize.apply(vb, flags, render_depth, one, num_rendered, means2D, *inputs,
                                    *(vb.camera_inputs(dev) if cam_grad else (None, None, None)))
        else:
            outs, nr, _ = _render_serial(vb, flags, one, inputs, True, False)
            num_rendered = nr[:vb.count]
    finally:
        if home != dev.index:
            torch.cuda.set_device(home)
    return (outs[0], outs[1], num_rendered) + tuple(outs[2:])


def rasterize_gaussians(means3D, means2D, sh, colors_precomp, opacities, scales, rotations, cov3Ds_precomp,
                        raster_settings, fast_exp=None, static_scene=False, render_depth=False):
    vb = raster_settings if isinstance(raster_settings, ViewBatch) else [raster_settings]
    m2d = means2D if isinstance(means2D, torch.Tensor) and means2D.requires_grad else None
    if render_depth:
        color, radii, _, depth, alpha = rasterize_views(vb, means3D, opacities, sh, colors_precomp, scales, rotations,
                                                        cov3Ds_precomp, fast_exp=fast_exp, _one=True, means2D=m2d,
                                                        render_depth=True)
        return color, radii, depth, alpha
    color, radii, _ = rasterize_views(vb, means3D, opacities, sh, colors_precomp, scales, rotations, cov3Ds_precomp,
                                      fast_exp=fast_exp, _one=True, static_scene=static_scene, means2D=m2d)
    return color, radii


class GaussianRasterizer(torch.nn.Module):
    def __init__(self, raster_settings: GaussianRasterizationSettings, fast_exp=None, static_scene=False,
                 render_depth=False):
        super().__init__()
        self.render_depth = render_depth
        self.raster_settings = raster_settings
        self.fast_exp = fast_exp
        self.static_scene = static_scene
        self._view_batch = None

    @staticmethod
    def _stamp(rs):
        return _lib.tensor_stamp((rs.viewmatrix, rs.projmatrix, rs.campos, rs.bg))

    def _views(self):
        rs = self.raster_settings
        stamp = self._stamp(rs)
        if stamp is None:
            self._view_batch = None
            return ViewBatch([rs])
        if self._view_batch is None or self._view_batch[0] is not rs or self._view_batch[1] != stamp:
            self._view_batch = (rs, stamp, ViewBatch([rs]))
        return self._view_batch[2]

    def markVisible(self, positions):
        with torch.no_grad():
            dev = _lib.require_gpu()
            p = positions.detach().to(device=positions.device if positions.is_cuda else dev,
                                      dtype=torch.float32).contiguous()
            present = torch.zeros((p.shape[0],), dtype=torch.uint8, device=p.device)
            vm = (ctypes.c_float * 16)(*self.raster_settings.viewmatrix.detach().to("cpu", torch.float32)
                                       .reshape(-1).tolist())
            _lib.call(p.device, "gr_raster_mark_visible", p.shape[0], p, vm, present)
            return present.bool()

    def forward(self, means3D, means2D, opacities, shs=None, colors_precomp=None, scales=None, rotations=None,
                cov3D_precomp=None):
        rs = self.raster_settings
        if (shs is None and colors_precomp is None) or (shs is not None and colors_precomp is not None):
            raise Exception('Please provide excatly one of either SHs or precomputed colors!')
        if ((scales is None or rotations is None) and cov3D_precomp is None) or \
                ((scales is not None or rotations is not None) and cov3D_precomp is not None):
            raise Exception('Please provide exactly one of either scale/rotation pair or precomputed 3D covariance!')
        return rasterize_gaussians(means3D, means2D, shs, colors_precomp, opacities, scales, rotations,
                                   cov3D_precomp, self._views(), fast_exp=self.fast_exp, static_scene=self.static_scene,
                                   render_depth=self.render_depth)
```

Baseline: 14070 views/s.

## Add compact 32-byte per-view Gaussian records for render-only multi-view forward

For forward-only renders with more than four views, preprocess writes a compact two-float4 record per Gaussian and view (position, conic, colour), plus one shared per-Gaussian opacity array, in place of the four-float4 full record. The blend kernel rebuilds the culling cutoffs (sxx, syy, kc) from the conic on the fly. This roughly halves record write and gather traffic in preprocess and blend, at the cost of extra ALU work per fetched splat. The layout is tagged in the geometry buffer, and backward, keep-state and depth paths refuse compact buffers. Reading the layout tag can cost a host sync on the first lookup for each geometry buffer.

```diff
diff --git a/gaussreg_amd/_lib.py b/gaussreg_amd/_lib.py
--- a/gaussreg_amd/_lib.py
+++ b/gaussreg_amd/_lib.py
@@ -8,6 +8,7 @@
 TRAIN_HEADER_PATH = os.path.join(_HERE, "..", "include", "gaussreg_hip_train.h")
 MATCH_TRAIN_HEADER_PATH = os.path.join(_HERE, "..", "include", "gaussreg_hip_train_matching.h")
 BACKBONE_TRAIN_HEADER_PATH = os.path.join(_HERE, "..", "include", "gaussreg_hip_train_backbone.h")
+RASTER_HEADER_PATH = os.path.join(_HERE, "..", "include", "gaussreg_hip_raster.h")
 
 _lib = None
 
@@ -89,6 +90,8 @@
     MATCH_TRAIN_SIGNATURES, MATCH_TRAIN_DEFINES = parse_header(_f.read())
 with open(BACKBONE_TRAIN_HEADER_PATH) as _f:
     BACKBONE_TRAIN_SIGNATURES, BACKBONE_TRAIN_DEFINES = parse_header(_f.read())
+with open(RASTER_HEADER_PATH) as _f:
+    RASTER_SIGNATURES, RASTER_DEFINES = parse_header(_f.read())
 
 GR_PENDING = DEFINES["GR_PENDING"]
 GR_RETRY_FULL = DEFINES["GR_RETRY_FULL"]
@@ -112,7 +115,8 @@
                 "(there is no CPU fallback for the gaussreg_amd ops)")
         L = ctypes.CDLL(LIB_PATH)
         for name, (res, args) in (list(SIGNATURES.items()) + list(TRAIN_SIGNATURES.items())
-                                   + list(MATCH_TRAIN_SIGNATURES.items()) + list(BACKBONE_TRAIN_SIGNATURES.items())):
+                                   + list(MATCH_TRAIN_SIGNATURES.items()) + list(BACKBONE_TRAIN_SIGNATURES.items())
+                                   + list(RASTER_SIGNATURES.items())):
             fn = getattr(L, name)
             fn.restype = res
             fn.argtypes = args
diff --git a/gaussreg_amd/build.py b/gaussreg_amd/build.py
--- a/gaussreg_amd/build.py
+++ b/gaussreg_amd/build.py
@@ -30,7 +30,7 @@
     headers = [os.path.join(CSRC, f) for f in os.listdir(CSRC) if f.endswith((".hpp", ".h"))]
     headers += [os.path.join(HERE, "..", "include", h) for h in ("gaussreg_hip.h", "gaussreg_hip_train.h",
                                                                  "gaussreg_hip_train_matching.h",
-                                                                 "gaussreg_hip_train_backbone.h")]
+                                                                 "gaussreg_hip_train_backbone.h", "gaussreg_hip_raster.h")]
     jobs = []
     objs = []
     for src in sources():
diff --git a/gaussreg_amd/csrc/common.hpp b/gaussreg_amd/csrc/common.hpp
--- a/gaussreg_amd/csrc/common.hpp
+++ b/gaussreg_amd/csrc/common.hpp
@@ -139,6 +139,8 @@
 }
 #endif
 
+int raster_geom_layout(const void* geom, int64_t P, int num_views, int64_t tiles, hipStream_t stream, int* layout);
+
 struct DepthSortTotals {
   int32_t* chunk_total;
   int chunk, nchunk;
diff --git a/gaussreg_amd/csrc/preprocess_body.hpp b/gaussreg_amd/csrc/preprocess_body.hpp
--- a/gaussreg_amd/csrc/preprocess_body.hpp
+++ b/gaussreg_amd/csrc/preprocess_body.hpp
@@ -2,10 +2,13 @@
 #error "preprocess_body.hpp is the body of the two preprocess kernels of rasterizer.hip"
 #endif
 static_assert(std::is_same<decltype(WAVE_MM), const bool>::value, "the including kernel defines `constexpr bool WAVE_MM`");
+static_assert(std::is_same<std::remove_const_t<decltype(COMPACT)>, bool>::value,
+              "the including kernel defines `constexpr bool COMPACT` (or has it as a template parameter)");
   if (LATE && blockIdx.x == 0 && threadIdx.x < (int)(sizeof(DevView) / 4))
     reinterpret_cast<float*>(const_cast<DevView*>(views))[threadIdx.x] = reinterpret_cast<const float*>(&cam1)[threadIdx.x];
   __shared__ float4 s_sh[(SH16 && !LATE) ? WAVE * SH_ROW : 1];
-  __shared__ float4 s_rec[256 / WAVE][4 * REC_PLANE];
+  constexpr int RP = COMPACT ? 72 : REC_PLANE;
+  __shared__ float4 s_rec[256 / WAVE][(COMPACT ? 2 : 4) * RP];
   __shared__ int s_mm[WAVE_MM ? 1 : 2][2][256 / WAVE];
   int i = blockIdx.x * blockDim.x + threadIdx.x;
   float shr[SH16 ? 48 : 1];
@@ -57,6 +60,7 @@
     for (int k = 0; k < 3; ++k) cpre[k] = colors_precomp[3 * (int64_t)i + k];
   }
   float4* wrec = s_rec[threadIdx.x / WAVE];
+  if (COMPACT && valid) rec32_opacity(rec, (int64_t)V * P)[i] = opacity;
   float mod_prev = 0.f;
   bool have_cov = HAS_COV;
   for (int v = 0; v < V; ++v) {
@@ -118,12 +122,12 @@
           out_radius = (int)my_radius;
           out_xy = make_float2(px, py);
           out_co = make_float4(cv[2] * det_inv, -cv[1] * det_inv, cv[0] * det_inv, opacity);
-          const bool cullable = det > 0.0f && l2 >= 0.29f && l1 < 1.0e4f;
-          const float kc = cullable ? 1.001f / (0.5f / l1 - 2.0e-6f) : INFINITY;
+          const bool cullable = cutoffs_cullable(det, l1, l2);
+          const float kc = cutoff_kc_stored(l1, cullable);
           out_kc = kc;
           if (cullable) {
-            out_sxx = 2.0f * cv[0] * 1.004f;
-            out_syy = 2.0f * cv[2] * 1.004f;
+            out_sxx = cutoff_axis_stored(cv[0]);
+            out_syy = cutoff_axis_stored(cv[2]);
             const float pcm = __logf(255.0f * opacity) + 2.0e-3f;
             if (pcm > 0.0f) {
               const float cp = pcm + 2.0e-6f * (pcm * kc);
@@ -155,9 +159,13 @@
       dfield[o] = out_field;
       rect_raw[o] = out_rect;
     }
-    wrec[0 * REC_PLANE + lane] = make_float4(out_xy.x, out_xy.y, out_sxx, out_syy);
-    wrec[1 * REC_PLANE + lane] = out_co;
-    wrec[3 * REC_PLANE + lane] = make_float4(__int_as_float(out_radius), out_depth, 0.f, 0.f);
+    if (COMPACT) {
+      wrec[0 * RP + lane] = make_float4(out_xy.x, out_xy.y, out_co.x, out_co.y);
+    } else {
+      wrec[0 * RP + lane] = make_float4(out_xy.x, out_xy.y, out_sxx, out_syy);
+      wrec[1 * RP + lane] = out_co;
+      wrec[3 * RP + lane] = make_float4(__int_as_float(out_radius), out_depth, 0.f, 0.f);
+    }
     if (WAVE_MM) {
       const uint32_t fld = valid ? out_field : 0u;
       const int mn = wave_min_i32_dpp(fld != 0u ? (int)fld : 0x7fffffff), mx = wave_max_i32_dpp((int)fld);
@@ -186,21 +194,35 @@
         rgb[0] = cpre[0]; rgb[1] = cpre[1]; rgb[2] = cpre[2];
       }
     }
-    wrec[2 * REC_PLANE + lane] = make_float4(rgb[0], rgb[1], rgb[2], out_kc);
+    if (COMPACT) wrec[1 * RP + lane] = make_float4(out_co.z, rgb[0], rgb[1], rgb[2]);
+    else wrec[2 * RP + lane] = make_float4(rgb[0], rgb[1], rgb[2], out_kc);
     const unsigned long long vis = __ballot(valid && out_radius > 0);
     __builtin_amdgcn_fence(__ATOMIC_RELEASE, "wavefront");
     __builtin_amdgcn_wave_barrier();
     __builtin_amdgcn_fence(__ATOMIC_ACQUIRE, "wavefront");
+    if (COMPACT) {
+      float4* wout = rec + 2 * ((int64_t)v * P + wave_first);
+#pragma unroll
+      for (int k = 0; k < 2; ++k) {
+        const int rl = 32 * k + lane / 2;
+        const float4 piece = wrec[(lane & 1) * RP + rl];
+        if ((vis >> rl) & 1ull) {
+          typedef float pre_f4 __attribute__((ext_vector_type(4)));
+          __builtin_nontemporal_store(pre_f4{piece.x, piece.y, piece.z, piece.w}, reinterpret_cast<pre_f4*>(wout + 2 * rl + (lane & 1)));
+        }
+      }
+    } else {
     float4* wout = rec + 4 * ((int64_t)v * P + wave_first);
 #pragma unroll
     for (int k = 0; k < 4; ++k) {
       const int rl = 16 * k + lane / 4;
-      const float4 piece = wrec[(lane & 3) * REC_PLANE + rl];
+      const float4 piece = wrec[(lane & 3) * RP + rl];
       if ((vis >> rl) & 1ull) {
         typedef float pre_f4 __attribute__((ext_vector_type(4)));
         __builtin_nontemporal_store(pre_f4{piece.x, piece.y, piece.z, piece.w}, reinterpret_cast<pre_f4*>(wout + 4 * rl + (lane & 3)));
       }
     }
+    }
     __builtin_amdgcn_fence(__ATOMIC_RELEASE, "wavefront");
     __builtin_amdgcn_wave_barrier();
     __builtin_amdgcn_fence(__ATOMIC_ACQUIRE, "wavefront");
diff --git a/gaussreg_amd/csrc/raster_shared.hpp b/gaussreg_amd/csrc/raster_shared.hpp
--- a/gaussreg_amd/csrc/raster_shared.hpp
+++ b/gaussreg_amd/csrc/raster_shared.hpp
@@ -1,6 +1,7 @@
 #pragma once
 
 #include "common.hpp"
+#include "../../include/gaussreg_hip_raster.h"
 
 namespace gr {
 namespace {
@@ -145,6 +146,49 @@
     res += 0.5f;
     rgb[c] = fmaxf(res, 0.0f);
   }
+}
+
+constexpr int REC_LAYOUT_FULL = 0, REC_LAYOUT_COMPACT = 1;
+__host__ __device__ __forceinline__ float* rec32_opacity(const float4* rec, int64_t VP) {
+  return reinterpret_cast<float*>(const_cast<float4*>(rec) + 2 * VP);
+}
+
+struct CellCutoffs {
+  float sxx, syy, kc;
+};
+__device__ __forceinline__ bool cutoffs_cullable(float det, float l1, float l2) {
+  return det > 0.0f && l2 >= 0.29f && l1 < 1.0e4f;
+}
+__device__ __forceinline__ float cutoff_kc_stored(float l1, bool cullable) {
+  return cullable ? 1.001f / (0.5f / l1 - 2.0e-6f) : INFINITY;
+}
+__device__ __forceinline__ float cutoff_axis_stored(float cv_axis) { return 2.0f * cv_axis * 1.004f; }
+__device__ __forceinline__ CellCutoffs cutoffs_stored(const float* cv, float l1, bool cullable) {
+  CellCutoffs c;
+  c.kc = cutoff_kc_stored(l1, cullable);
+  c.sxx = cullable ? cutoff_axis_stored(cv[0]) : INFINITY;
+  c.syy = cullable ? cutoff_axis_stored(cv[2]) : INFINITY;
+  return c;
+}
+constexpr float CUTOFF_M_MAX = 18000.0f;
+constexpr float CUTOFF_WIDEN_MAX = (CUTOFF_M_MAX + 1.0f) / 1048576.0f;
+__device__ __forceinline__ CellCutoffs cutoffs_rebuilt(float x, float y, float z) {
+  const float xz = x * z, yy = y * y;
+  const float D = xz - yy, S = xz + yy;
+  const float invD = 1.0f / D;
+  const float E = 1.0f + 9.5367431640625e-7f * (S * invD + 1.0f);
+  const float mid_c = 0.5f * (x + z), hd = 0.5f * (x - z);
+  const float disc = fmaxf(0.1f * (D * D), hd * hd + yy) + 9.5367431640625e-7f * (mid_c * mid_c);
+  const float l1 = (mid_c + sqrtf(disc)) * invD;
+  const float midv = mid_c * invD;
+  const float l2 = fminf(midv * midv - 0.1f, invD) / l1;
+  const float G = E * E;
+  const bool ok = D > 0.0f && S <= CUTOFF_M_MAX * D && l2 >= 0.29f * G + 9.5367431640625e-7f * l1 && l1 * G < 1.0e4f;
+  CellCutoffs c;
+  c.kc = ok ? 1.001f / (0.5f / (l1 * E) - 2.0e-6f) * 1.000001f : INFINITY;
+  c.sxx = ok ? 2.0f * (z * invD) * 1.004f * E : INFINITY;
+  c.syy = ok ? 2.0f * (x * invD) * 1.004f * E : INFINITY;
+  return c;
 }
 
 struct Geom {
diff --git a/gaussreg_amd/csrc/rasterizer.hip b/gaussreg_amd/csrc/rasterizer.hip
--- a/gaussreg_amd/csrc/rasterizer.hip
+++ b/gaussreg_amd/csrc/rasterizer.hip
@@ -3,6 +3,7 @@
 #include <vector>
 
 #include <atomic>
+#include <mutex>
 
 #include "raster_shared.hpp"
 
@@ -34,12 +35,13 @@
     uint32_t* __restrict__ rect_raw, int32_t* __restrict__ far_flag, DevView cam1, int far_seq,
     int2* __restrict__ key_mm) {
   constexpr bool WAVE_MM = false;
+  constexpr bool COMPACT = false;
 #define GR_PREPROCESS_BODY_OK
 #include "preprocess_body.hpp"
 #undef GR_PREPROCESS_BODY_OK
 }
 
-template <bool HAS_SH, bool HAS_COV, bool SH16>
+template <bool HAS_SH, bool HAS_COV, bool SH16, bool COMPACT = false>
 __global__ __launch_bounds__(256) void preprocess_many_kernel(
     int P, int D, int M, int V, const DevView* __restrict__ views, const float* __restrict__ means3D,
     const float* __restrict__ shs, const float* __restrict__ colors_precomp,
@@ -670,11 +672,12 @@
   float* state;
 };
 
-template <bool FAST_EXP, bool KEEP = false, bool AUX = false>
-__global__ __launch_bounds__(BLOCK) __attribute__((amdgpu_waves_per_eu(8, 8))) void blend_kernel(
+template <bool FAST_EXP, bool KEEP, bool AUX, bool COMPACT>
+__device__ __forceinline__ void blend_body(
     int P, int W, int H, int nchunk, const DevView* __restrict__ views, const uint32_t* __restrict__ seg_off,
     const int32_t* __restrict__ point_list, const float4* __restrict__ rec, float* __restrict__ out_color,
     unsigned int list_cap, BlendAux<AUX> aux) {
+  static_assert(!(COMPACT && (KEEP || AUX)), "the compact records hold neither the depth nor what the backward reads");
   __shared__ float4 s_ga[BLOCK + 1], s_gb[BLOCK + 1];
   __shared__ f32x2 s_gc[BLOCK + 1];
   __shared__ float s_z[AUX ? BLOCK + 1 : 1];
@@ -750,10 +753,21 @@
       for (int st = WAVE / 2; st > 0; st >>= 1)
         if (s_wpre[lo + st - 1] <= e) lo += st;
       const int before = lo ? s_wpre[lo - 1] : 0;
-      const float4* r = rec + 4 * (goff + point_list[s_woff[lo] + (unsigned int)(e - before)]);
-      const float4 r0 = r[0];
-      const float4 co = r[1];
-      const float4 col = r[2];
+      const int gid = point_list[s_woff[lo] + (unsigned int)(e - before)];
+      const float4* r = rec + (COMPACT ? 2 : 4) * (goff + gid);
+      float4 r0, co, col;
+      if (COMPACT) {
+        const float4 q0 = r[0], q1 = r[1];
+        const float op = rec32_opacity(rec, (int64_t)gridDim.z * P)[gid];
+        const CellCutoffs cut = cutoffs_rebuilt(q0.z, q0.w, q1.x);
+        r0 = make_float4(q0.x, q0.y, cut.sxx, cut.syy);
+        co = make_float4(q0.z, q0.w, q1.x, op);
+        col = make_float4(q1.y, q1.z, q1.w, cut.kc);
+      } else {
+        r0 = r[0];
+        co = r[1];
+        col = r[2];
+      }
       const float pc = -__logf(255.0f * co.w) - 1.0e-3f;
       rc2 = -pc * col.w;
       const float cpr = -pc + 1.0e-3f + 2.0e-6f * rc2;
@@ -875,6 +889,22 @@
   }
 }
 
+template <bool FAST_EXP, bool KEEP = false, bool AUX = false>
+__global__ __launch_bounds__(BLOCK) __attribute__((amdgpu_waves_per_eu(8, 8))) void blend_kernel(
+    int P, int W, int H, int nchunk, const DevView* __restrict__ views, const uint32_t* __restrict__ seg_off,
+    const int32_t* __restrict__ point_list, const float4* __restrict__ rec, float* __restrict__ out_color,
+    unsigned int list_cap, BlendAux<AUX> aux) {
+  blend_body<FAST_EXP, KEEP, AUX, false>(P, W, H, nchunk, views, seg_off, point_list, rec, out_color, list_cap, aux);
+}
+
+template <bool FAST_EXP>
+__global__ __launch_bounds__(BLOCK) __attribute__((amdgpu_waves_per_eu(8, 8))) void blend_compact_kernel(
+    int P, int W, int H, int nchunk, const DevView* __restrict__ views, const uint32_t* __restrict__ seg_off,
+    const int32_t* __restrict__ point_list, const float4* __restrict__ rec, float* __restrict__ out_color,
+    unsigned int list_cap, BlendAux<false> aux) {
+  blend_body<FAST_EXP, false, false, true>(P, W, H, nchunk, views, seg_off, point_list, rec, out_color, list_cap, aux);
+}
+
 __global__ __launch_bounds__(256) void mark_visible_kernel(int P, const float* __restrict__ means3D,
                                                            float v2, float v6, float v10, float v14,
                                                            uint8_t* __restrict__ present) {
@@ -883,6 +913,25 @@
   const float z = fmaf(v2, means3D[3 * (int64_t)i],
                        fmaf(v6, means3D[3 * (int64_t)i + 1], fmaf(v10, means3D[3 * (int64_t)i + 2], v14)));
   present[i] = z > 0.2f ? 1 : 0;
+}
+
+__global__ __launch_bounds__(256) void cutoffs_probe_kernel(int64_t n, const float* __restrict__ cov2d,
+                                                            float* __restrict__ out_stored, float* __restrict__ out_rebuilt) {
+  const int64_t i = (int64_t)blockIdx.x * blockDim.x + threadIdx.x;
+  if (i >= n) return;
+  const float cv[3] = {cov2d[3 * i], cov2d[3 * i + 1], cov2d[3 * i + 2]};
+  CellCutoffs st{INFINITY, INFINITY, INFINITY}, rb{INFINITY, INFINITY, INFINITY};
+  const float det = cv[0] * cv[2] - cv[1] * cv[1];
+  if (det != 0.0f) {
+    const float det_inv = 1.f / det;
+    const float mid = 0.5f * (cv[0] + cv[2]);
+    const float sq = sqrtf(fmaxf(0.1f, mid * mid - det));
+    const float l1 = mid + sq, l2 = mid - sq;
+    st = cutoffs_stored(cv, l1, cutoffs_cullable(det, l1, l2));
+    rb = cutoffs_rebuilt(cv[2] * det_inv, -cv[1] * det_inv, cv[0] * det_inv);
+  }
+  out_stored[3 * i] = st.sxx, out_stored[3 * i + 1] = st.syy, out_stored[3 * i + 2] = st.kc;
+  out_rebuilt[3 * i] = rb.sxx, out_rebuilt[3 * i + 1] = rb.syy, out_rebuilt[3 * i + 2] = rb.kc;
 }
 
 int check_views(const gr_raster_view* h_views, int num_views) {
@@ -939,6 +988,47 @@
 
 namespace gr {
 namespace {
+std::atomic<int> g_compact_on{getenv("GR_RASTER_COMPACT_RECORDS") && getenv("GR_RASTER_COMPACT_RECORDS")[0] == '1' ? 1 : 0};
+struct LayoutNote {
+  const void* geom;
+  int layout;
+};
+std::mutex g_layout_mu;
+LayoutNote g_layout_notes[64];
+int g_layout_next = 0;
+void note_layout(const void* geom, int layout) {
+  std::lock_guard<std::mutex> lock(g_layout_mu);
+  for (LayoutNote& n : g_layout_notes)
+    if (n.geom == geom) {
+      n.layout = layout;
+      return;
+    }
+  g_layout_notes[g_layout_next] = LayoutNote{geom, layout};
+  g_layout_next = (g_layout_next + 1) % 64;
+}
+}
+
+int raster_geom_layout(const void* geom, int64_t P, int num_views, int64_t tiles, hipStream_t stream, int* layout) {
+  *layout = REC_LAYOUT_FULL;
+  if (num_views <= 4 || P == 0 || geom == nullptr) return GR_OK;
+  {
+    std::lock_guard<std::mutex> lock(g_layout_mu);
+    for (const LayoutNote& n : g_layout_notes)
+      if (n.geom == geom) {
+        *layout = n.layout;
+        return GR_OK;
+      }
+  }
+  const Geom g = carve_geom(const_cast<void*>(geom), P, num_views, tiles);
+  int32_t word = 0;
+  GR_HIP(hipMemcpyAsync(&word, g.totals + 2 * num_views + 1, sizeof(word), hipMemcpyDeviceToHost, stream));
+  GR_HIP(hipStreamSynchronize(stream));
+  *layout = word == REC_LAYOUT_COMPACT ? REC_LAYOUT_COMPACT : REC_LAYOUT_FULL;
+  note_layout(geom, *layout);
+  return GR_OK;
+}
+
+namespace {
 std::atomic<int> g_frames[64];
 
 bool verify_this_frame() {
@@ -1003,7 +1093,8 @@
   d.scale_mod = s.scale_modifier;
 }
 
-int upload_views(const gr_raster_view* h_views, int num_views, int32_t* d_flag, hipStream_t stream) {
+int upload_views(const gr_raster_view* h_views, int num_views, int32_t* d_flag, hipStream_t stream,
+                 int layout = REC_LAYOUT_FULL) {
   static_assert(sizeof(DevView) % 4 == 0, "DevView is copied word by word");
   if (num_views <= VIEW_PACK) {
     ViewPack pack;
@@ -1016,6 +1107,7 @@
   char* raw = static_cast<char*>(pinned_scratch(0, 16 + sizeof(DevView) * num_views));
   GR_REQUIRE(raw != nullptr, "pinned staging buffer for %d views could not be allocated", num_views);
   memset(raw, 0, 16);
+  reinterpret_cast<int32_t*>(raw)[1] = layout;
   DevView* stage = reinterpret_cast<DevView*>(raw + 16);
   for (int v = 0; v < num_views; ++v) fill_view(stage[v], h_views[v]);
   GR_HIP(hipMemcpyAsync(d_flag, raw, 16 + sizeof(DevView) * num_views, hipMemcpyHostToDevice, stream));
@@ -1070,7 +1162,7 @@
                            const float* scales, const float* rotations,
                            const float* cov3D_precomp, const gr_raster_view* h_views,
                            int num_views, int32_t* radii, void* geom, size_t geom_bytes,
-                           int64_t* h_num_rendered, hipStream_t stream, Deferred* defer_ev) {
+                           int64_t* h_num_rendered, hipStream_t stream, Deferred* defer_ev, bool want_compact = false) {
   int rc = check_views(h_views, num_views);
   if (rc != GR_OK) return rc;
   GR_REQUIRE(h_num_rendered != nullptr, "h_num_rendered is null");
@@ -1084,6 +1176,7 @@
     }
     rc = upload_views(h_views, num_views, g0.totals + 2 * num_views, stream);
     if (rc != GR_OK) return rc;
+    if (num_views > 4) note_layout(geom, REC_LAYOUT_FULL);
     GR_HIP(hipStreamSynchronize(stream));
     return GR_OK;
   }
@@ -1114,19 +1207,26 @@
   memset(&cam1, 0, sizeof(cam1));
   int far_seq = 1;
   if (sh16 && num_views == 1) fill_view(cam1, h_views[0]);
+  const bool msd_possible = depth_sort_msd_possible(P, num_views, KEY_DEPTH_BITS);
+  const bool msd = msd_possible && (defer_ev != nullptr ? defer_ev->bucket_sort : bucket_sort_allowed(true));
+  bool compact = want_compact && msd && num_views > 4 && gx <= 63 && gy <= 63 && g_compact_on.load() != 0;
   if (cam_in_args) {
     far_seq = defer_ev->seq;
   } else {
-    rc = upload_views(h_views, num_views, g.totals + 2 * num_views, stream);
+    rc = upload_views(h_views, num_views, g.totals + 2 * num_views, stream, compact ? REC_LAYOUT_COMPACT : REC_LAYOUT_FULL);
     if (rc != GR_OK) return rc;
   }
+  if (num_views > 4) note_layout(geom, compact ? REC_LAYOUT_COMPACT : REC_LAYOUT_FULL);
   if (defer_ev != nullptr) defer_ev->far_seq = far_seq;
-  const bool msd_possible = depth_sort_msd_possible(P, num_views, KEY_DEPTH_BITS);
-  const bool msd = msd_possible && (defer_ev != nullptr ? defer_ev->bucket_sort : bucket_sort_allowed(true));
   int2* const mm_out = msd ? g.key_mm : nullptr;
 #define GR_PRE(SH, COV, S16)                                                                       \
   if (S16 && num_views == 1)                                                                       \
     hipLaunchKernelGGL((preprocess_kernel<SH, COV, S16, S16>), grd, blk, 0, stream, (int)P, D, M, num_views, \
+                       g.views, means3D, shs, colors_precomp, opacities, scales, rotations,        \
+                       cov3D_precomp, W, H, radii, g.rec, g.dfield, g.rect_raw, g.totals + 2 * num_views, cam1, far_seq, \
+                       mm_out);                                                                    \
+  else if (msd && num_views > 4 && compact)                                                        \
+    hipLaunchKernelGGL((preprocess_many_kernel<SH, COV, S16, true>), grd, blk, 0, stream, (int)P, D, M, num_views, \
                        g.views, means3D, shs, colors_precomp, opacities, scales, rotations,        \
                        cov3D_precomp, W, H, radii, g.rec, g.dfield, g.rect_raw, g.totals + 2 * num_views, cam1, far_seq, \
                        mm_out);                                                                    \
@@ -1244,6 +1344,14 @@
     GR_REQUIRE(h_bad == 0, "depth sort produced an unsorted order (internal error)");
     return GR_OK;
   };
+  if (compact && (tot[2 * num_views] & 1)) {
+    compact = false;
+    rc = upload_views(h_views, num_views, g.totals + 2 * num_views, stream, REC_LAYOUT_FULL);
+    if (rc != GR_OK) return rc;
+    note_layout(geom, REC_LAYOUT_FULL);
+    run_preprocess();
+    GR_LAUNCH_CHECK();
+  }
   if (tot[2 * num_views] & 2) {
     bucket_sort_overflowed();
     GR_HIP(hipMemsetD32Async(reinterpret_cast<hipDeviceptr_t>(g.totals + 2 * num_views), tot[2 * num_views] & 1, 1, stream));
@@ -1287,6 +1395,34 @@
                                     int64_t* h_num_rendered, void* stream_) {
   return preprocess_impl(P, M, means3D, shs, colors_precomp, opacities, scales, rotations, cov3D_precomp, h_views, num_views,
                          radii, geom, geom_bytes, h_num_rendered, static_cast<hipStream_t>(stream_), nullptr);
+}
+
+extern "C" int gr_raster_preprocess_ex(int64_t P, int M, const float* means3D, const float* shs,
+                                       const float* colors_precomp, const float* opacities,
+                                       const float* scales, const float* rotations,
+                                       const float* cov3D_precomp, const gr_raster_view* h_views,
+                                       int num_views, int32_t* radii, void* geom, size_t geom_bytes,
+                                       int64_t* h_num_rendered, int flags, void* stream_) {
+  return preprocess_impl(P, M, means3D, shs, colors_precomp, opacities, scales, rotations, cov3D_precomp, h_views, num_views,
+                         radii, geom, geom_bytes, h_num_rendered, static_cast<hipStream_t>(stream_), nullptr,
+                         (flags & GR_RASTER_COMPACT) != 0);
+}
+
+extern "C" int gr_raster_cutoffs_probe(int64_t n, const float* cov2d, const float* opacity, float* out_stored,
+                                       float* out_rebuilt, void* stream_) {
+  (void)opacity;
+  GR_REQUIRE(n >= 0, "n out of range");
+  if (n == 0) return GR_OK;
+  GR_REQUIRE(cov2d && out_stored && out_rebuilt, "null argument");
+  hipLaunchKernelGGL(cutoffs_probe_kernel, dim3((unsigned)((n + 255) / 256)), dim3(256), 0, static_cast<hipStream_t>(stream_), n,
+                     cov2d, out_stored, out_rebuilt);
+  GR_LAUNCH_CHECK();
+  return GR_OK;
+}
+
+extern "C" int gr_raster_compact_records(int on) {
+  if (on == 0 || on == 1) return g_compact_on.exchange(on);
+  return g_compact_on.load();
 }
 
 static int preprocess_collect(int64_t P, int num_views, int64_t* h_num_rendered, bool* far_depth, Deferred& d, hipStream_t stream,
@@ -1350,6 +1486,15 @@
   const int tiles = gx * gy;
   Geom g = carve_geom(const_cast<void*>(geom), P, num_views, tiles);
   GR_REQUIRE(P == 0 || (geom && geom_bytes >= g.bytes), "geometry buffer missing or too small");
+  int layout = REC_LAYOUT_FULL;
+  rc = raster_geom_layout(geom, P, num_views, tiles, stream, &layout);
+  if (rc != GR_OK) return rc;
+  const bool compact = layout == REC_LAYOUT_COMPACT;
+  if (compact && (keep || out_depth != nullptr)) {
+    set_error("rasterizer: the geometry buffer holds the compact records of a render-only preprocess (GR_RASTER_COMPACT); "
+              "the kept state and the depth map need gr_raster_preprocess");
+    return GR_ERR_INVALID;
+  }
   Bin b = carve_bin(bin, R, vtiles);
   if (!bin || bin_bytes < b.bytes) {
     set_error("raster binning buffer too small: need %zu bytes, got %zu", b.bytes, bin_bytes);
@@ -1429,6 +1574,10 @@
 #define GR_BLEND(FE, KEEP)                                                                                            \
   hipLaunchKernelGGL((blend_kernel<FE, KEEP>), dim3(gx, gy, num_views), dim3(BLOCK), blend_pad, stream, (int)P, W, H,      \
                      blend_chunks, g.views, g.seg_off, point_list, g.rec, out_color, list_cap, BlendAux<false>{})
+#define GR_BLEND_COMPACT(FE)                                                                                          \
+  hipLaunchKernelGGL((blend_compact_kernel<FE>), dim3(gx, gy, num_views), dim3(BLOCK), blend_pad, stream,   \
+                     (int)P, W, H, blend_chunks, g.views, g.seg_off, point_list, g.rec, out_color, list_cap,            \
+                     BlendAux<false>{})
 #define GR_BLEND_AUX(FE, KEEP)                                                                                        \
   hipLaunchKernelGGL((blend_kernel<FE, KEEP, true>), dim3(gx, gy, num_views), dim3(BLOCK), 0, stream, (int)P, W, H,        \
                      blend_chunks, g.views, g.seg_off, point_list, g.rec, out_color, list_cap,                           \
@@ -1438,8 +1587,10 @@
     else if (fast) GR_BLEND_AUX(true, false); else GR_BLEND_AUX(false, false);
   }
   else if (keep) { if (fast) GR_BLEND(true, true); else GR_BLEND(false, true); }
+  else if (compact) { if (fast) GR_BLEND_COMPACT(true); else GR_BLEND_COMPACT(false); }
   else if (fast) GR_BLEND(true, false); else GR_BLEND(false, false);
 #undef GR_BLEND
+#undef GR_BLEND_COMPACT
 #undef GR_BLEND_AUX
   GR_LAUNCH_CHECK();
   frame_done();
@@ -1555,8 +1706,8 @@
     for (int v = 0; v < num_views; ++v) R += h_num_rendered[v];
     if (!far_depth) return R <= entries ? GR_OK : GR_RETRY_BIN;
   }
-  int rc = gr_raster_preprocess(P, M, means3D, shs, colors_precomp, opacities, scales, rotations, cov3D_precomp, h_views,
-                                num_views, radii, geom, geom_bytes, h_num_rendered, stream);
+  int rc = gr_raster_preprocess_ex(P, M, means3D, shs, colors_precomp, opacities, scales, rotations, cov3D_precomp, h_views,
+                                   num_views, radii, geom, geom_bytes, h_num_rendered, flags & GR_RASTER_COMPACT, stream);
   if (rc != GR_OK) return rc;
   int64_t R = 0;
   for (int v = 0; v < num_views; ++v) R += h_num_rendered[v];
diff --git a/gaussreg_amd/csrc/rasterizer_backward.hip b/gaussreg_amd/csrc/rasterizer_backward.hip
--- a/gaussreg_amd/csrc/rasterizer_backward.hip
+++ b/gaussreg_amd/csrc/rasterizer_backward.hip
@@ -475,6 +475,12 @@
   GR_REQUIRE(R < (1ll << 31) - 1, "too many rendered instances");
   const Geom g = carve_geom(const_cast<void*>(geom), P, num_views, tiles);
   GR_REQUIRE(geom != nullptr && geom_bytes >= g.bytes, "geometry buffer missing or too small");
+  {
+    int layout = 0;
+    const int rcl = raster_geom_layout(geom, P, num_views, tiles, stream, &layout);
+    if (rcl != GR_OK) return rcl;
+    GR_REQUIRE(layout == 0, "rasterizer backward: the geometry buffer holds the compact records of a render-only preprocess");
+  }
   const Bin bn = carve_bin(const_cast<void*>(bin), R, (int64_t)tiles * num_views);
   GR_REQUIRE(R == 0 || (bin != nullptr && bin_bytes >= bn.bytes), "binning buffer missing or too small");
   GR_REQUIRE(R == 0 || (final_T != nullptr && n_contrib != nullptr && (aux || dL_dcolor != nullptr)), "null per-pixel state");
diff --git a/gaussreg_amd/rasterizer.py b/gaussreg_amd/rasterizer.py
--- a/gaussreg_amd/rasterizer.py
+++ b/gaussreg_amd/rasterizer.py
@@ -24,6 +24,7 @@
 
 
 FAST_EXP, SPLIT, SHARE, BWD_COLOR_ONLY = (_lib.DEFINES["GR_RASTER_" + f] for f in ("FAST_EXP", "SPLIT", "SHARE", "BWD_COLOR_ONLY"))
+COMPACT = _lib.RASTER_DEFINES["GR_RASTER_COMPACT"]
 _ENV_FAST = None
 _bin_hint = {}
 
@@ -317,7 +318,8 @@
         def forward(fl):
             return L.gr_raster_forward(P, M, *ptrs, views, V, _lib.ptr(radii), _lib.ptr(geom), gbytes, _lib.ptr(binb),
                                        hint + 256 if binb is not None else 0, _lib.ptr(color), fl, nr, st)
-        rc = forward(flags | ((SPLIT | (SHARE if pipe.overlapping and V == 1 else 0)) if pipe is not None else 0))
+        rc = forward(flags | (COMPACT if V > 4 else 0) |
+                     ((SPLIT | (SHARE if pipe.overlapping and V == 1 else 0)) if pipe is not None else 0))
         joined = rejoin = False
         if rc == _lib.GR_PENDING:
             try:
diff --git a/include/gaussreg_hip_raster.h b/include/gaussreg_hip_raster.h
--- /dev/null
+++ b/include/gaussreg_hip_raster.h
@@ -0,0 +1,26 @@
+#ifndef GAUSSREG_HIP_RASTER_H_
+#define GAUSSREG_HIP_RASTER_H_
+
+#include <stddef.h>
+#include <stdint.h>
+
+#include "gaussreg_hip.h"
+
+#ifdef __cplusplus
+extern "C" {
+#endif
+
+#define GR_RASTER_COMPACT 16
+int gr_raster_preprocess_ex(int64_t P, int sh_coeffs, const float* means3D, const float* shs,
+                            const float* colors_precomp, const float* opacities, const float* scales,
+                            const float* rotations, const float* cov3D_precomp,
+                            const gr_raster_view* h_views, int num_views, int32_t* radii, void* geom,
+                            size_t geom_bytes, int64_t* h_num_rendered, int flags, void* stream);
+int gr_raster_compact_records(int on);
+int gr_raster_cutoffs_probe(int64_t n, const float* cov2d, const float* opacity, float* out_stored, float* out_rebuilt,
+                            void* stream);
+
+#ifdef __cplusplus
+}
+#endif
+#endif
```

Result: no change. 14060 views/s, median of 2 (-0.1%).
